# AdaptiveCity/deepdish

Hardware: AMD Instinct MI355X
Metric: end-to-end frames/sec (detect+encode+track) at 640x480 (higher is better)
Workload: dtype i8 (reference: uint8); encoder f16; 1 GPU; SSD-MobileNet-v1 uint8-quantised (300x300) + MARS-64x32x3 + deep_sort on synthetic 640x480 BGR frames, ~20 synthetic detections/frame (BASELINE.json configs[1]); streams_per_gpu=3072, worker_threads_per_gpu=2, parallelism=independent streams, 3072 per GPU in 2 worker groups, weights=seeded synthetic (seed 1234)

## Files before the change

deepdish_amd/csrc/mars_pair.hip:

```cpp
#include "mars_tail.h"

namespace {

typedef _Float16 h8 __attribute__((ext_vector_type(8)));
typedef float f4 __attribute__((ext_vector_type(4)));
typedef unsigned u4 __attribute__((ext_vector_type(4)));

__device__ __forceinline__ float elu(float v) {
    float e = __builtin_amdgcn_exp2f(v * 1.44269504088896340736f);
    e = __builtin_amdgcn_fmed3f(e, 0.f, 1.f);
    return __builtin_amdgcn_fmed3f(v, e - 1.f, 3.0e38f);
}

__device__ __forceinline__ void lds_fill16(const _Float16 *g, char *lds_wave_base) {
#if defined(__HIP_DEVICE_COMPILE__)
    __builtin_amdgcn_global_load_lds(g, lds_wave_base, 16, 0, 0);
#endif
}

__device__ __forceinline__ int frag_row(int a, int fr) { return (fr >> 2) * 8 + (a & 1) * 4 + (fr & 3); }

constexpr int PZ_B = 3072;
constexpr int PT64_B = 18 * 1024;
constexpr int PT32_B = 33 * 1024;
constexpr int PPLAIN_B = 16 * 1024;
constexpr int PRAW_B = 8 * 1024;
constexpr int pair_off_in(bool) { return PZ_B; }
constexpr int pair_off_h(bool first) { return PZ_B + 2 * (first ? PT32_B : PT64_B); }
constexpr int pair_off_res(bool first) { return pair_off_h(first) + 2 * PT64_B; }
constexpr int pair_off_raw(bool first) { return pair_off_res(first) + (first ? 2 : 3) * PPLAIN_B; }
constexpr int pair_off_const(bool first) { return pair_off_raw(first) + (first ? 2 * PRAW_B : 0); }
constexpr int pair_lds_bytes(bool first) { return pair_off_const(first) + 5 * 64 * 4; }

template <bool FIRST>
__global__ __launch_bounds__(512, 2) void mars_pair64_k(const MarsPairP P) {
    constexpr int OFF_IN = pair_off_in(FIRST), OFF_H = pair_off_h(FIRST), OFF_RES = pair_off_res(FIRST), OFF_RAW = pair_off_raw(FIRST),
                  OFF_C = pair_off_const(FIRST);
    constexpr int TIN_B = FIRST ? PT32_B : PT64_B, NRES = FIRST ? 2 : 3;
    extern __shared__ __attribute__((aligned(16))) char smem[];
    const int tid = threadIdx.x, lane = tid & 63;
    const int wave = __builtin_amdgcn_readfirstlane(tid >> 6);
    const int stage = wave >> 2, half = wave & 1, q = (wave >> 1) & 1;
    const int fr = lane & 15, fq = lane >> 4, j = fr >> 3, x = fr & 7;

    for (int i = tid * 16; i < OFF_C; i += 512 * 16) *reinterpret_cast<u4 *>(smem + i) = u4{0u, 0u, 0u, 0u};
    float *cst = reinterpret_cast<float *>(smem + OFF_C);
    if (tid < 64) {
        cst[tid] = P.bias_a[tid];
        cst[64 + tid] = P.bias_b[tid];
        cst[128 + tid] = P.aff2[tid];
        cst[192 + tid] = P.aff2[P.cout_pad + tid];
        cst[256 + tid] = (FIRST && P.bias_p) ? P.bias_p[tid] : 0.f;
    }
    __syncthreads();

    h8 wf[9][2][2];
    h8 wp[2];
    const bool a32 = FIRST && stage == 0;
    {
        const _Float16 *w = stage == 0 ? P.wa : P.wb;
        const int kpad = stage == 0 ? P.kpad_a : P.kpad_b;
#pragma unroll
        for (int t = 0; t < 9; ++t)
#pragma unroll
            for (int ks = 0; ks < 2; ++ks)
#pragma unroll
                for (int a = 0; a < 2; ++a) {
                    const size_t row = (size_t)(half * 32 + frag_row(a, fr)) * kpad;
                    wf[t][ks][a] = a32 ? *reinterpret_cast<const h8 *>(w + row + t * 32 + fq * 8)
                                       : *reinterpret_cast<const h8 *>(w + row + t * 64 + ks * 32 + fq * 8);
                }
#pragma unroll
        for (int a = 0; a < 2; ++a)
            wp[a] = FIRST ? *reinterpret_cast<const h8 *>(P.wp + (size_t)(half * 32 + frag_row(a, fr)) * P.kpad_p + fq * 8) : wf[0][0][a];
    }
#if defined(__HIP_DEVICE_COMPILE__)
#pragma unroll
    for (int t = 0; t < 9; ++t)
#pragma unroll
        for (int ks = 0; ks < 2; ++ks)
#pragma unroll
            for (int a = 0; a < 2; ++a) asm volatile("" ::"v"(wf[t][ks][a]));
    asm volatile("" ::"v"(wp[0]), "v"(wp[1]));
#endif

    const int n0 = blockIdx.x, nstep = gridDim.x;
    const int Kc = (P.n_img - n0 + nstep - 1) / nstep;

    const _Float16 *src[5];
    size_t stp[5];
    int n_dma;
    if constexpr (FIRST) {
        const int par = lane >> 5, pl = (lane >> 3) & 3, col = 2 * (lane & 7) + par;
#pragma unroll
        for (int h = 0; h < 4; ++h) {
            const int r = wave + 8 * h < 31 ? wave + 8 * h : 30;
            src[h] = col < 15 ? P.in + ((size_t)n0 * 31 + r) * 15 * P.cs_in + (size_t)col * P.cs_in + P.coff_in + pl * 8 : P.zero;
            stp[h] = col < 15 ? (size_t)nstep * 31 * 15 * P.cs_in : 0;
        }
        const int jr = lane >> 5, xx = lane & 7;
        src[4] = P.in2 + ((size_t)n0 * 31 + 2 * (2 * wave + jr)) * 15 * P.cs_in2 + (size_t)(2 * xx) * P.cs_in2 + P.coff_in2 + pl * 8;
        stp[4] = (size_t)nstep * 31 * 15 * P.cs_in2;
        n_dma = 5;
    } else {
        const int pl = lane >> 3, xx = lane & 7;
#pragma unroll
        for (int h = 0; h < 2; ++h) {
            src[h] = P.in + (((size_t)n0 * 16 + wave + 8 * h) * 8 + xx) * P.cs_in + P.coff_in + pl * 8;
            stp[h] = (size_t)nstep * 128 * P.cs_in;
            src[2 + h] = P.res + (((size_t)n0 * 16 + wave + 8 * h) * 8 + xx) * P.cs_res + P.coff_res + pl * 8;
            stp[2 + h] = (size_t)nstep * 128 * P.cs_res;
        }
        src[4] = P.zero; stp[4] = 0;
        n_dma = 4;
    }
    (void)n_dma;
    int dq = 0;
    auto issue = [&]() {
        char *T = smem + OFF_IN + (dq & 1) * TIN_B;
        if constexpr (FIRST) {
#pragma unroll
            for (int h = 0; h < 4; ++h) lds_fill16(src[h], T + ((wave + 8 * h < 31 ? wave + 8 * h : 30) + 1) * 1024);
            lds_fill16(src[4], smem + OFF_RAW + (dq & 1) * PRAW_B + wave * 1024);
        } else {
#pragma unroll
            for (int h = 0; h < 2; ++h) lds_fill16(src[h], T + (wave + 8 * h + 1) * 1024);
            const int rs = dq % 3;
#pragma unroll
            for (int h = 0; h < 2; ++h) lds_fill16(src[2 + h], smem + OFF_RES + rs * PPLAIN_B + (wave + 8 * h) * 1024);
        }
        ++dq;
        const bool more = dq < Kc;
#pragma unroll
        for (int h = 0; h < 5; ++h) src[h] += more ? stp[h] : 0;
    };

    const int co = half * 32 + fq * 8;
    const unsigned lo64 = (unsigned)((j * 64 + fq * 8 + x) * 16);
    const unsigned lo32 = (unsigned)((2 * j * 64 + fq * 8 + x) * 16);
    const f4 ba0 = *reinterpret_cast<const f4 *>(cst + (stage ? 64 : 0) + co), ba1 = *reinterpret_cast<const f4 *>(cst + (stage ? 64 : 0) + co + 4);

    issue();
    for (int c = 0; c <= Kc; ++c) {
#if defined(__HIP_DEVICE_COMPILE__)
        if (stage == 0 || c < 2) asm volatile("s_waitcnt vmcnt(0) lgkmcnt(0)" ::: "memory");
        else asm volatile("s_waitcnt vmcnt(8) lgkmcnt(0)" ::: "memory");
        __builtin_amdgcn_s_barrier();
        asm volatile("" ::: "memory");
#endif
        issue();
        const int cc = stage == 0 ? c : c - 1;
        if (cc < 0 || cc >= Kc) continue;
        const size_t n = (size_t)(n0 + cc * nstep);
#pragma unroll 1
        for (int f = 0; f < 4; ++f) {
            const int F = 4 * q + f;
            f4 acc[2] = {f4{0.f, 0.f, 0.f, 0.f}, f4{0.f, 0.f, 0.f, 0.f}};
            h8 X[4];
            if (a32) {
                const unsigned tb = (unsigned)(OFF_IN + (cc & 1) * PT32_B + 4 * F * 1024) + lo32;
                const unsigned bL = x == 0 ? ((tb + 512u - 16u) & 255u) : tb + 512u - 16u, bC = tb, bR = tb + 512u;
                const unsigned pb = (unsigned)(OFF_RAW + (cc & 1) * PRAW_B) + (unsigned)(((2 * F + j) * 32 + fq * 8 + x) * 16);
                f4 accp[2] = {f4{0.f, 0.f, 0.f, 0.f}, f4{0.f, 0.f, 0.f, 0.f}};
#if defined(__HIP_DEVICE_COMPILE__)
#define DD_RD(u_) do { if constexpr ((u_) < 9) { constexpr int dy_ = (u_) / 3, dx_ = (u_) - dy_ * 3;                                               \
                           asm volatile("ds_read_b128 %0, %1 offset:%2" : "=&v"(X[(u_) & 3]) : "v"(dx_ == 0 ? bL : dx_ == 1 ? bC : bR), "n"(dy_ * 1024) : "memory"); } \
                       else asm volatile("ds_read_b128 %0, %1" : "=&v"(X[(u_) & 3]) : "v"(pb) : "memory"); } while (0)
#define DD_UNIT(u_) do { if constexpr ((u_) + 3 < 10) DD_RD(((u_) + 3) % 10);                                                                      \
                         asm volatile("s_waitcnt lgkmcnt(%1)" : "+v"(X[(u_) & 3]) : "n"((u_) + 3 < 10 ? 3 : 9 - (u_)));                           \
                         if constexpr ((u_) < 9) { _Pragma("unroll") for (int a = 0; a < 2; ++a) acc[a] = __builtin_amdgcn_mfma_f32_16x16x32_f16(wf[(u_) % 9][0][a], X[(u_) & 3], acc[a], 0, 0, 0); } \
                         else { _Pragma("unroll") for (int a = 0; a < 2; ++a) accp[a] = __builtin_amdgcn_mfma_f32_16x16x32_f16(wp[a], X[(u_) & 3], accp[a], 0, 0, 0); } } while (0)
                DD_RD(0); DD_RD(1); DD_RD(2);
                DD_UNIT(0); DD_UNIT(1); DD_UNIT(2); DD_UNIT(3); DD_UNIT(4); DD_UNIT(5); DD_UNIT(6); DD_UNIT(7); DD_UNIT(8); DD_UNIT(9);
#undef DD_UNIT
#undef DD_RD
#endif
                const f4 c0 = *reinterpret_cast<const f4 *>(cst + 256 + co), c1 = *reinterpret_cast<const f4 *>(cst + 256 + co + 4);
                h8 sk;
#pragma unroll
                for (int i = 0; i < 4; ++i) { sk[i] = (_Float16)(accp[0][i] + c0[i]); sk[4 + i] = (_Float16)(accp[1][i] + c1[i]); }
                *reinterpret_cast<h8 *>(smem + OFF_RES + (cc & 1) * PPLAIN_B + ((2 * F + j) * 64 + (half * 4 + fq) * 8 + x) * 16) = sk;
            } else {
                const unsigned tb = (unsigned)((stage == 0 ? OFF_IN + (cc & 1) * PT64_B : OFF_H + (cc & 1) * PT64_B) + 2 * F * 1024) + lo64;
                const unsigned bL = x == 0 ? ((tb - 16u) & 255u) : tb - 16u, bC = tb, bR = x == 7 ? ((tb + 16u) & 255u) : tb + 16u;
#if defined(__HIP_DEVICE_COMPILE__)
#define DD_RD(u_) do { constexpr int t_ = (u_) >> 1, ks_ = (u_) & 1, dy_ = t_ / 3, dx_ = t_ - dy_ * 3;                                             \
                       asm volatile("ds_read_b128 %0, %1 offset:%2" : "=&v"(X[(u_) & 3]) : "v"(dx_ == 0 ? bL : dx_ == 1 ? bC : bR), "n"(dy_ * 1024 + ks_ * 512) : "memory"); } while (0)
#define DD_UNIT(u_) do { if constexpr ((u_) + 3 < 18) DD_RD(((u_) + 3) % 18);                                                                      \
                         asm volatile("s_waitcnt lgkmcnt(%1)" : "+v"(X[(u_) & 3]) : "n"((u_) + 3 < 18 ? 3 : 17 - (u_)));                          \
                         _Pragma("unroll") for (int a = 0; a < 2; ++a) acc[a] = __builtin_amdgcn_mfma_f32_16x16x32_f16(wf[(u_) >> 1][(u_) & 1][a], X[(u_) & 3], acc[a], 0, 0, 0); } while (0)
                DD_RD(0); DD_RD(1); DD_RD(2);
                DD_UNIT(0); DD_UNIT(1); DD_UNIT(2); DD_UNIT(3); DD_UNIT(4); DD_UNIT(5); DD_UNIT(6); DD_UNIT(7); DD_UNIT(8);
                DD_UNIT(9); DD_UNIT(10); DD_UNIT(11); DD_UNIT(12); DD_UNIT(13); DD_UNIT(14); DD_UNIT(15); DD_UNIT(16); DD_UNIT(17);
#undef DD_UNIT
#undef DD_RD
#endif
            }
            float v[8];
#pragma unroll
            for (int i = 0; i < 4; ++i) { v[i] = acc[0][i] + ba0[i]; v[4 + i] = acc[1][i] + ba1[i]; }
            if (stage == 0) {
                h8 o;
#pragma unroll
                for (int i = 0; i < 8; ++i) o[i] = (_Float16)elu(v[i]);
                *reinterpret_cast<h8 *>(smem + OFF_H + (cc & 1) * PT64_B + ((2 * F + j + 1) * 64 + (half * 4 + fq) * 8 + x) * 16) = o;
            } else {
                const int rs = FIRST ? (cc & 1) : cc % 3;
                const h8 rv = *reinterpret_cast<const h8 *>(smem + OFF_RES + rs * PPLAIN_B + ((2 * F + j) * 64 + (half * 4 + fq) * 8 + x) * 16);
#pragma unroll
                for (int i = 0; i < 8; ++i) v[i] += (float)rv[i];
                const size_t m = (n * 16 + 2 * F + j) * 8 + x;
                h8 o;
#pragma unroll
                for (int i = 0; i < 8; ++i) o[i] = (_Float16)v[i];
                *reinterpret_cast<h8 *>(P.out + m * P.cs_out + P.coff_out + co) = o;
                const f4 s0 = *reinterpret_cast<const f4 *>(cst + 128 + co), s1 = *reinterpret_cast<const f4 *>(cst + 128 + co + 4);
                const f4 t0 = *reinterpret_cast<const f4 *>(cst + 192 + co), t1 = *reinterpret_cast<const f4 *>(cst + 192 + co + 4);
                h8 o2;
#pragma unroll
                for (int i = 0; i < 4; ++i) { o2[i] = (_Float16)elu(s0[i] * v[i] + t0[i]); o2[4 + i] = (_Float16)elu(s1[i] * v[4 + i] + t1[i]); }
                *reinterpret_cast<h8 *>(P.out2 + m * P.cs_out2 + P.coff_out2 + co) = o2;
            }
        }
    }
#if defined(__HIP_DEVICE_COMPILE__)
    asm volatile("s_waitcnt vmcnt(0)" ::: "memory");
#endif
}

template <bool FIRST>
int launch_pair(hipStream_t s, int device, const MarsPairP &P) {
    constexpr int lds = pair_lds_bytes(FIRST);
    static_assert(lds <= 160 * 1024, "LDS budget");
    static DevOnce once;
    const int rc = once.run(device, [&]() -> int {
        DD_HIP(hipFuncSetAttribute(reinterpret_cast<const void *>(&mars_pair64_k<FIRST>), hipFuncAttributeMaxDynamicSharedMemorySize, lds));
        return DD_OK;
    });
    if (rc != DD_OK) return rc;
    const int n_cu = dd_cu_count(device);
    const int grid = P.n_img < n_cu ? P.n_img : n_cu;
    hipLaunchKernelGGL((mars_pair64_k<FIRST>), dim3(grid), dim3(512), lds, s, P);
    DD_LAUNCH_CHECK();
    return DD_OK;
}

}

int mars_pair64_launch(hipStream_t s, int device, const MarsPairP &P, bool first) {
    DD_REQUIRE(P.n_img > 0 && P.in && P.wa && P.wb && P.bias_a && P.bias_b && P.out && P.out2 && P.aff2 && P.zero && (first ? (P.in2 && P.wp) : P.res != nullptr), DD_E_ARG,
               "mars_pair64: bad argument");
    return first ? launch_pair<true>(s, device, P) : launch_pair<false>(s, device, P);
}
```

deepdish_amd/csrc/mars_tail.h:

```cpp
#pragma once
#include "common.h"

struct MarsWsP {
    const _Float16 *in;  int cs_in, coff_in;
    const _Float16 *in2; int cs_in2, coff_in2;
    const _Float16 *w;   int kpad;
    const _Float16 *w2;  int kpad2;
    const float *bias, *bias2;
    const _Float16 *res; int cs_res, coff_res;
    _Float16 *out;  int cs_out, coff_out;
    _Float16 *out2; int cs_out2, coff_out2;
    const float *aff2; int cout_pad;
    const _Float16 *zero;
    int n_img;
};

enum { MARS_WS_S1 = 0, MARS_WS_S1_RES = 1, MARS_WS_S2_PROJ = 2 };

int mars_ws128_launch(hipStream_t s, int device, const MarsWsP &P, int mode, int act, bool out2);

struct MarsPairP {
    const _Float16 *in;  int cs_in, coff_in;
    const _Float16 *in2; int cs_in2, coff_in2;
    const _Float16 *wa;  int kpad_a; const float *bias_a;
    const _Float16 *wp;  int kpad_p; const float *bias_p;
    const _Float16 *wb;  int kpad_b; const float *bias_b;
    const _Float16 *res; int cs_res, coff_res;
    _Float16 *out;  int cs_out, coff_out;
    _Float16 *out2; int cs_out2, coff_out2;
    const float *aff2; int cout_pad;
    const _Float16 *zero;
    int n_img;
};
int mars_pair64_launch(hipStream_t s, int device, const MarsPairP &P, bool first);
```

deepdish_amd/csrc/mars_tail.hip:

```cpp
#include "mars_tail.h"
#include <vector>

namespace {

typedef _Float16 h8 __attribute__((ext_vector_type(8)));
typedef float f4 __attribute__((ext_vector_type(4)));
typedef unsigned u4 __attribute__((ext_vector_type(4)));

enum { ACT_NONE = 0, ACT_ELU = 2 };

__device__ __forceinline__ float elu(float v) {
    float e = __builtin_amdgcn_exp2f(v * 1.44269504088896340736f);
    e = __builtin_amdgcn_fmed3f(e, 0.f, 1.f);
    return __builtin_amdgcn_fmed3f(v, e - 1.f, 3.0e38f);
}

__device__ __forceinline__ void lds_fill16(const _Float16 *g, char *lds_wave_base) {
#if defined(__HIP_DEVICE_COMPILE__)
    __builtin_amdgcn_global_load_lds(g, lds_wave_base, 16, 0, 0);
#endif
}

__device__ __forceinline__ int frag_row(int a, int fr) { return (fr >> 2) * 8 + (a & 1) * 4 + (fr & 3); }

#ifdef DD_MARS_STAMPS
__device__ unsigned long long dd_mars_stamps[256 * 8 * 8];
#define DD_STAMP(k) do { const unsigned long long t_ = __builtin_amdgcn_s_memtime(); st_acc[k] += t_ - st_last; st_last = t_; } while (0)
#else
#define DD_STAMP(k) do { } while (0)
#endif

constexpr int WS_LEAD = 2, WS_NB = WS_LEAD + 2, WS_NBR = WS_LEAD + 3;
constexpr int ws_tile_bytes(int mode) { return mode == MARS_WS_S2_PROJ ? 17 * 68 * 16 : 10 * 72 * 16; }
constexpr int ws_zero_bytes(int mode) { return mode == MARS_WS_S2_PROJ ? 0 : 7680; }
constexpr int WS_RES_BYTES = 8 * 72 * 16, WS_PRJ_BYTES = 4096;
constexpr int ws_xw_bytes(int mode) { return mode == MARS_WS_S2_PROJ ? 4096 : 2048; }
constexpr int ws_off_tiles(int mode) { return ws_zero_bytes(mode); }
constexpr int ws_off_aux(int mode) { return ws_off_tiles(mode) + WS_NB * ws_tile_bytes(mode); }
constexpr int ws_off_xchg(int mode) {
    return ws_off_aux(mode) + (mode == MARS_WS_S1_RES ? WS_NBR * WS_RES_BYTES : mode == MARS_WS_S2_PROJ ? WS_NB * WS_PRJ_BYTES : 0);
}
constexpr int ws_off_const(int mode) { return ws_off_xchg(mode) + 2 * 8 * ws_xw_bytes(mode); }
constexpr int ws_lds_bytes(int mode) { return ws_off_const(mode) + 3 * 128 * 4; }

template <int MODE, int ACT, bool OUT2>
__global__ __launch_bounds__(512, 2) void mars_ws128_k(const MarsWsP P) {
    constexpr bool S2 = MODE == MARS_WS_S2_PROJ, RES = MODE == MARS_WS_S1_RES;
    constexpr int LEAD = WS_LEAD, NB = WS_NB, NBR = WS_NBR;
    constexpr int TILE_B = ws_tile_bytes(MODE), XW_B = ws_xw_bytes(MODE);
    constexpr int OFF_T = ws_off_tiles(MODE), OFF_A = ws_off_aux(MODE), OFF_X = ws_off_xchg(MODE), OFF_C = ws_off_const(MODE);
    constexpr int KS = S2 ? 1 : 2, CIN = S2 ? 64 : 128;
    [[maybe_unused]] constexpr int N_DMA = S2 ? 3 : RES ? 2 : 1;
    [[maybe_unused]] constexpr int N_ST = S2 ? 2 : (RES && OUT2) ? 2 : 1;
    extern __shared__ __attribute__((aligned(16))) char smem[];
    const int tid = threadIdx.x, lane = tid & 63;
    const int wave = __builtin_amdgcn_readfirstlane(tid >> 6);
    const int cg = wave & 3, kh = wave >> 2;
    const int fr = lane & 15, fq = lane >> 4, yy = fr >> 2, x = fr & 3;

    for (int i = tid * 16; i < OFF_A; i += 512 * 16) *reinterpret_cast<u4 *>(smem + i) = u4{0u, 0u, 0u, 0u};
    float *cst = reinterpret_cast<float *>(smem + OFF_C);
    if (tid < 128) {
        cst[tid] = P.bias[tid];
        if constexpr (S2) cst[128 + tid] = P.bias2 ? P.bias2[tid] : 0.f;
        if constexpr (RES && OUT2) { cst[128 + tid] = P.aff2[tid]; cst[256 + tid] = P.aff2[P.cout_pad + tid]; }
    }
    __syncthreads();

    h8 wf[9][KS][2];
#pragma unroll
    for (int t = 0; t < 9; ++t)
#pragma unroll
        for (int ks = 0; ks < KS; ++ks)
#pragma unroll
            for (int a = 0; a < 2; ++a)
                wf[t][ks][a] = *reinterpret_cast<const h8 *>(P.w + (size_t)(cg * 32 + frag_row(a, fr)) * P.kpad + t * CIN + kh * (CIN / 2) + ks * 32 + fq * 8);
    h8 wp[2];
    if constexpr (S2) {
#pragma unroll
        for (int a = 0; a < 2; ++a) wp[a] = *reinterpret_cast<const h8 *>(P.w2 + (size_t)(cg * 32 + frag_row(a, fr)) * P.kpad2 + kh * 32 + fq * 8);
    }

#if defined(__HIP_DEVICE_COMPILE__)
#pragma unroll
    for (int t = 0; t < 9; ++t)
#pragma unroll
        for (int ks = 0; ks < KS; ++ks)
#pragma unroll
            for (int a = 0; a < 2; ++a) asm volatile("" ::"v"(wf[t][ks][a]));
    if constexpr (S2) asm volatile("" ::"v"(wp[0]), "v"(wp[1]));
#endif

    const int n0 = blockIdx.x, nstep = gridDim.x;
    const int Kc = (P.n_img - n0 + nstep - 1) / nstep;

    int dq = 0, dq_slot = 0, dq_rslot = 0;
    const _Float16 *src_a, *src_b, *src_c;
    size_t step_a, step_b, step_c;
    if constexpr (!S2) {
        src_a = P.in + (size_t)n0 * 32 * P.cs_in + ((wave * 4 + (lane & 3)) * P.cs_in + P.coff_in + (lane >> 2) * 8);
        src_b = RES ? P.res + (size_t)n0 * 32 * P.cs_res + ((wave * 4 + (lane & 3)) * P.cs_res + P.coff_res + (lane >> 2) * 8) : P.zero;
        src_c = P.zero;
        step_a = (size_t)nstep * 32 * P.cs_in; step_b = (size_t)nstep * 32 * P.cs_res; step_c = 0;
    } else {
        const int par = lane >> 5, pl = (lane >> 2) & 7, col = 2 * (lane & 3) + par;
        src_a = P.in + (size_t)n0 * 128 * P.cs_in + ((wave * 8 + col) * P.cs_in + P.coff_in + pl * 8);
        src_b = src_a + (size_t)64 * P.cs_in;
        const int ch = (wave & 3) * 64 + lane;
        src_c = P.in2 + (size_t)n0 * 128 * P.cs_in2 + ((2 * ((ch >> 2) & 7) * 8 + 2 * (ch & 3)) * P.cs_in2 + P.coff_in2 + (ch >> 5) * 8);
        step_a = step_b = (size_t)nstep * 128 * P.cs_in; step_c = (size_t)nstep * 128 * P.cs_in2;
    }
    auto issue = [&]() {
        char *T = smem + OFF_T + dq_slot * TILE_B;
        if constexpr (!S2) {
            lds_fill16(src_a, T + (wave + 1) * 72 * 16);
            if constexpr (RES) lds_fill16(src_b, smem + OFF_A + dq_rslot * WS_RES_BYTES + wave * 72 * 16);
        } else {
            lds_fill16(src_a, T + wave * 68 * 16);
            lds_fill16(src_b, T + (wave + 8) * 68 * 16);
            lds_fill16(src_c, smem + OFF_A + dq_slot * WS_PRJ_BYTES + (wave & 3) * 1024);
        }
        ++dq;
        const bool more = dq < Kc;
        src_a += more ? step_a : 0;
        if constexpr (RES || S2) src_b += more ? step_b : 0;
        if constexpr (S2) src_c += more ? step_c : 0;
        dq_slot = dq_slot + 1 == NB ? 0 : dq_slot + 1;
        dq_rslot = dq_rslot + 1 == NBR ? 0 : dq_rslot + 1;
    };

    const unsigned lo = S2 ? (unsigned)((2 * yy * 68 + (kh * 4 + fq) * 4 + x) * 16) : (unsigned)((yy * 72 + (kh * 8 + fq) * 4 + x) * 16);
    const unsigned lo_prj = (unsigned)(((kh * 4 + fq) * 32 + yy * 4 + x) * 16);
    const unsigned lo_res = (unsigned)(((4 * kh + yy) * 72 + (cg * 4 + fq) * 4 + x) * 16);
    const int co = cg * 32 + fq * 8;
    const f4 b0 = *reinterpret_cast<const f4 *>(cst + co), b1 = *reinterpret_cast<const f4 *>(cst + co + 4);

    f4 keep[S2 ? 4 : 2];
    int slot = 0, rslot_prev = 0, rslot = 0;

    auto epilogue = [&](int cprev) {
        const char *Xp = smem + OFF_X + ((cprev & 1) * 8 + (wave ^ 4)) * XW_B + lane * 16;
        const size_t n = (size_t)(n0 + cprev * nstep);
        const size_t m = (n * 8 + 4 * kh + yy) * 4 + x;
        float v[8];
        {
            const f4 o0 = *reinterpret_cast<const f4 *>(Xp), o1 = *reinterpret_cast<const f4 *>(Xp + 1024);
#pragma unroll
            for (int i = 0; i < 4; ++i) { v[i] = keep[0][i] + o0[i] + b0[i]; v[4 + i] = keep[1][i] + o1[i] + b1[i]; }
        }
        if constexpr (ACT == ACT_ELU) {
#pragma unroll
            for (int i = 0; i < 8; ++i) v[i] = elu(v[i]);
        }
        if constexpr (RES) {
            const h8 rv = *reinterpret_cast<const h8 *>(smem + OFF_A + rslot_prev * WS_RES_BYTES + lo_res);
#pragma unroll
            for (int i = 0; i < 8; ++i) v[i] += (float)rv[i];
        }
        h8 o;
#pragma unroll
        for (int i = 0; i < 8; ++i) o[i] = (_Float16)v[i];
        *reinterpret_cast<h8 *>(P.out + m * P.cs_out + P.coff_out + co) = o;
        if constexpr (RES && OUT2) {
            const f4 s0 = *reinterpret_cast<const f4 *>(cst + 128 + co), s1 = *reinterpret_cast<const f4 *>(cst + 128 + co + 4);
            const f4 t0 = *reinterpret_cast<const f4 *>(cst + 256 + co), t1 = *reinterpret_cast<const f4 *>(cst + 256 + co + 4);
            h8 o2;
#pragma unroll
            for (int i = 0; i < 4; ++i) { o2[i] = (_Float16)elu(s0[i] * v[i] + t0[i]); o2[4 + i] = (_Float16)elu(s1[i] * v[4 + i] + t1[i]); }
            *reinterpret_cast<h8 *>(P.out2 + m * P.cs_out2 + P.coff_out2 + co) = o2;
        }
        if constexpr (S2) {
            const f4 o0 = *reinterpret_cast<const f4 *>(Xp + 2048), o1 = *reinterpret_cast<const f4 *>(Xp + 3072);
            const f4 c0 = *reinterpret_cast<const f4 *>(cst + 128 + co), c1 = *reinterpret_cast<const f4 *>(cst + 128 + co + 4);
            h8 o2;
#pragma unroll
            for (int i = 0; i < 4; ++i) { o2[i] = (_Float16)(keep[2][i] + o0[i] + c0[i]); o2[4 + i] = (_Float16)(keep[3][i] + o1[i] + c1[i]); }
            *reinterpret_cast<h8 *>(P.out2 + m * P.cs_out2 + P.coff_out2 + co) = o2;
        }
    };

#ifdef DD_MARS_STAMPS
    unsigned long long st_acc[8] = {0, 0, 0, 0, 0, 0, 0, 0}, st_last = __builtin_amdgcn_s_memtime();
    const unsigned long long st_begin = st_last;
#endif
    static_assert(LEAD == 2, "the counted waits below are written for two crops of look-ahead");
    for (int ci = 0; ci < LEAD; ++ci) issue();
    DD_STAMP(0);
    for (int c = 0; c <= Kc; ++c) {
#if defined(__HIP_DEVICE_COMPILE__)
        if (kh == 0 || c == 0) {
            if (c <= 1) asm volatile("s_waitcnt vmcnt(%0) lgkmcnt(0)" ::"i"(N_DMA) : "memory");
            else if (c == 2) asm volatile("s_waitcnt vmcnt(%0) lgkmcnt(0)" ::"i"(N_DMA + N_ST) : "memory");
            else asm volatile("s_waitcnt vmcnt(%0) lgkmcnt(0)" ::"i"(N_DMA + 2 * N_ST) : "memory");
        } else asm volatile("s_waitcnt lgkmcnt(0)" ::: "memory");
        DD_STAMP(2);
        __builtin_amdgcn_s_barrier();
        asm volatile("" ::: "memory");
#endif
        DD_STAMP(3);
        auto compute = [&](f4 (&kp)[S2 ? 4 : 2]) {
            const unsigned tb = (unsigned)(OFF_T + slot * TILE_B) + lo;
            f4 acc[2][2] = {{f4{0.f, 0.f, 0.f, 0.f}, f4{0.f, 0.f, 0.f, 0.f}}, {f4{0.f, 0.f, 0.f, 0.f}, f4{0.f, 0.f, 0.f, 0.f}}};
            if constexpr (!S2) {
                const unsigned bs[3] = {x == 0 ? ((tb - 16u) & 255u) : tb - 16u, tb, x == 3 ? ((tb + 16u) & 255u) : tb + 16u};
                h8 X[4][2];
#if defined(__HIP_DEVICE_COMPILE__)
#define DD_RD(u_) do { constexpr int t_ = (u_) >> 1, p_ = (u_) & 1, dy_ = t_ / 3, dx_ = t_ - dy_ * 3;                                      \
                       asm volatile("ds_read_b128 %0, %2 offset:%3\n\tds_read_b128 %1, %2 offset:%4"                                       \
                                    : "=&v"(X[(u_) & 3][0]), "=&v"(X[(u_) & 3][1]) : "v"(bs[dx_]), "n"(((4 * p_ + dy_) * 72) * 16), "n"(((4 * p_ + dy_) * 72 + 16) * 16) : "memory"); } while (0)
#define DD_UNIT(u_) do { if constexpr ((u_) + 3 < 18) DD_RD(((u_) + 3) % 18);                                                            \
                         asm volatile("s_waitcnt lgkmcnt(%2)" : "+v"(X[(u_) & 3][0]), "+v"(X[(u_) & 3][1]) : "n"((u_) + 3 < 18 ? 6 : 2 * (17 - (u_))));          \
                         _Pragma("unroll") for (int ks = 0; ks < 2; ++ks) _Pragma("unroll") for (int a = 0; a < 2; ++a)                  \
                             acc[(u_) & 1][a] = __builtin_amdgcn_mfma_f32_16x16x32_f16(wf[(u_) >> 1][ks][a], X[(u_) & 3][ks], acc[(u_) & 1][a], 0, 0, 0); } while (0)
                DD_RD(0); DD_RD(1); DD_RD(2);
                DD_UNIT(0); DD_UNIT(1); DD_UNIT(2); DD_UNIT(3); DD_UNIT(4); DD_UNIT(5); DD_UNIT(6); DD_UNIT(7); DD_UNIT(8);
                DD_UNIT(9); DD_UNIT(10); DD_UNIT(11); DD_UNIT(12); DD_UNIT(13); DD_UNIT(14); DD_UNIT(15); DD_UNIT(16); DD_UNIT(17);
#undef DD_UNIT
#undef DD_RD
#endif
            } else {
                f4 accp[2][2] = {{f4{0.f, 0.f, 0.f, 0.f}, f4{0.f, 0.f, 0.f, 0.f}}, {f4{0.f, 0.f, 0.f, 0.f}, f4{0.f, 0.f, 0.f, 0.f}}};
                h8 X[4];
                const unsigned pb = (unsigned)(OFF_A + slot * WS_PRJ_BYTES) + lo_prj;
                const h8 hz = {(_Float16)0.f, (_Float16)0.f, (_Float16)0.f, (_Float16)0.f, (_Float16)0.f, (_Float16)0.f, (_Float16)0.f, (_Float16)0.f};
#if defined(__HIP_DEVICE_COMPILE__)
#define DD_RD(u_) do { if constexpr ((u_) < 18) { constexpr int t_ = (u_) >> 1, p_ = (u_) & 1, dy_ = t_ / 3, dx_ = t_ - dy_ * 3;                    \
                           asm volatile("ds_read_b128 %0, %1 offset:%2" : "=&v"(X[(u_) & 3]) : "v"(tb), "n"(((8 * p_ + dy_) * 68 + (dx_ == 1 ? 32 : 0) + (dx_ == 2 ? 1 : 0)) * 16) : "memory"); } \
                       else asm volatile("ds_read_b128 %0, %1 offset:%2" : "=&v"(X[(u_) & 3]) : "v"(pb), "n"(((u_) - 18) * 256) : "memory"); } while (0)
#define DD_UNIT(u_) do { if constexpr ((u_) + 3 < 20) DD_RD(((u_) + 3) % 20);                                                            \
                         asm volatile("s_waitcnt lgkmcnt(%1)" : "+v"(X[(u_) & 3]) : "n"((u_) + 3 < 20 ? 3 : 19 - (u_)));               \
                         if constexpr ((u_) < 18) { const h8 xv_ = (((u_) >> 1) % 3 == 2 && x == 3) ? hz : X[(u_) & 3];                    \
                             _Pragma("unroll") for (int a = 0; a < 2; ++a) acc[(u_) & 1][a] = __builtin_amdgcn_mfma_f32_16x16x32_f16(wf[(u_) >> 1][0][a], xv_, acc[(u_) & 1][a], 0, 0, 0); } \
                         else { _Pragma("unroll") for (int a = 0; a < 2; ++a) accp[(u_) - 18][a] = __builtin_amdgcn_mfma_f32_16x16x32_f16(wp[a], X[(u_) & 3], accp[(u_) - 18][a], 0, 0, 0); } } while (0)
                DD_RD(0); DD_RD(1); DD_RD(2);
                DD_UNIT(0); DD_UNIT(1); DD_UNIT(2); DD_UNIT(3); DD_UNIT(4); DD_UNIT(5); DD_UNIT(6); DD_UNIT(7); DD_UNIT(8); DD_UNIT(9);
                DD_UNIT(10); DD_UNIT(11); DD_UNIT(12); DD_UNIT(13); DD_UNIT(14); DD_UNIT(15); DD_UNIT(16); DD_UNIT(17); DD_UNIT(18); DD_UNIT(19);
#undef DD_UNIT
#undef DD_RD
#endif
                char *Xm = smem + OFF_X + ((c & 1) * 8 + wave) * XW_B + lane * 16;
                *reinterpret_cast<f4 *>(Xm + 2048) = kh ? accp[0][0] : accp[1][0];
                *reinterpret_cast<f4 *>(Xm + 3072) = kh ? accp[0][1] : accp[1][1];
                kp[2] = kh ? accp[1][0] : accp[0][0];
                kp[3] = kh ? accp[1][1] : accp[0][1];
            }
            char *Xm = smem + OFF_X + ((c & 1) * 8 + wave) * XW_B + lane * 16;
            *reinterpret_cast<f4 *>(Xm) = kh ? acc[0][0] : acc[1][0];
            *reinterpret_cast<f4 *>(Xm + 1024) = kh ? acc[0][1] : acc[1][1];
            kp[0] = kh ? acc[1][0] : acc[0][0];
            kp[1] = kh ? acc[1][1] : acc[0][1];
        };
        if (kh == 0) {
            f4 kn[S2 ? 4 : 2];
            if (c < Kc) compute(kn);
            DD_STAMP(5);
#if defined(__HIP_DEVICE_COMPILE__)
            asm volatile("s_waitcnt lgkmcnt(0)" ::: "memory");
            __builtin_amdgcn_s_barrier();
            asm volatile("" ::: "memory");
#endif
            DD_STAMP(3);
            issue();
            DD_STAMP(1);
            if (c > 0) epilogue(c - 1);
            DD_STAMP(4);
#pragma unroll
            for (int i = 0; i < (S2 ? 4 : 2); ++i) keep[i] = kn[i];
        } else {
            issue();
            DD_STAMP(1);
            if (c > 0) epilogue(c - 1);
            DD_STAMP(4);
#if defined(__HIP_DEVICE_COMPILE__)
            if (c == 0) asm volatile("s_waitcnt vmcnt(%0) lgkmcnt(0)" ::"i"(N_DMA) : "memory");
            else if (c == 1) asm volatile("s_waitcnt vmcnt(%0) lgkmcnt(0)" ::"i"(N_DMA + N_ST) : "memory");
            else asm volatile("s_waitcnt vmcnt(%0) lgkmcnt(0)" ::"i"(N_DMA + 2 * N_ST) : "memory");
            __builtin_amdgcn_s_barrier();
            asm volatile("" ::: "memory");
#endif
            DD_STAMP(3);
            if (c < Kc) compute(keep);
            DD_STAMP(5);
        }
        slot = slot + 1 == NB ? 0 : slot + 1;
        rslot_prev = rslot;
        rslot = rslot + 1 == NBR ? 0 : rslot + 1;
    }
#if defined(__HIP_DEVICE_COMPILE__)
    asm volatile("s_waitcnt vmcnt(0)" ::: "memory");
#endif
#ifdef DD_MARS_STAMPS
    if (lane == 0) {
        unsigned long long *d = dd_mars_stamps + ((size_t)blockIdx.x * 8 + wave) * 8;
        for (int k = 0; k < 6; ++k) d[k] = st_acc[k];
        d[6] = __builtin_amdgcn_s_memtime() - st_begin;
        d[7] = (unsigned long long)Kc;
    }
#endif
}

template <int MODE, int ACT, bool OUT2>
int launch_one(hipStream_t s, int device, const MarsWsP &P) {
    constexpr int lds = ws_lds_bytes(MODE);
    static_assert(lds <= 160 * 1024, "LDS budget");
    static DevOnce once;
    const int rc = once.run(device, [&]() -> int {
        DD_HIP(hipFuncSetAttribute(reinterpret_cast<const void *>(&mars_ws128_k<MODE, ACT, OUT2>), hipFuncAttributeMaxDynamicSharedMemorySize, lds));
        return DD_OK;
    });
    if (rc != DD_OK) return rc;
    const int n_cu = dd_cu_count(device);
    const int grid = P.n_img < n_cu ? P.n_img : n_cu;
    hipLaunchKernelGGL((mars_ws128_k<MODE, ACT, OUT2>), dim3(grid), dim3(512), lds, s, P);
    DD_LAUNCH_CHECK();
#ifdef DD_MARS_STAMPS
    {
        static std::vector<unsigned long long> h(256 * 8 * 8);
        DD_HIP(hipStreamSynchronize(s));
        DD_HIP(hipMemcpyFromSymbol(h.data(), HIP_SYMBOL(dd_mars_stamps), h.size() * 8));
        for (int half = 0; half < 2; ++half) {
            double a[7] = {0, 0, 0, 0, 0, 0, 0};
            int nw = 0;
            for (int b = 0; b < grid; ++b)
                for (int w = half * 4; w < half * 4 + 4; ++w, ++nw) {
                    const unsigned long long *d = h.data() + ((size_t)b * 8 + w) * 8;
                    for (int k = 0; k < 7; ++k) a[k] += (double)d[k] / (double)(k == 0 || k == 6 ? 1 : d[7] + 1);
                }
            fprintf(stderr, "mars_ws128_k<%d,%d,%d> K half %d: prologue DMAs %.0f | per step: issue %.0f, wait %.0f, barrier %.0f, epilogue %.0f, compute %.0f | loop total %.0f cycles, %d steps\n",
                    MODE, ACT, (int)OUT2, half, a[0] / nw, a[1] / nw, a[2] / nw, a[3] / nw, a[4] / nw, a[5] / nw, a[6] / nw, (int)h[7] + 1);
        }
    }
#endif
    return DD_OK;
}

}

int mars_ws128_launch(hipStream_t s, int device, const MarsWsP &P, int mode, int act, bool out2) {
    DD_REQUIRE(P.n_img > 0 && P.in && P.w && P.bias && P.out && P.zero, DD_E_ARG, "mars_ws128: bad argument");
    DD_REQUIRE((long long)P.n_img * 128 * (P.cs_in > P.cs_out ? P.cs_in : P.cs_out) < (1ll << 40), DD_E_CAPACITY, "mars_ws128: batch of %d", P.n_img);
    if (mode == MARS_WS_S2_PROJ) {
        DD_REQUIRE(P.in2 && P.w2 && P.out2 && act == ACT_ELU, DD_E_ARG, "mars_ws128: stride-2 form needs the projection operands and ELU");
        return launch_one<MARS_WS_S2_PROJ, ACT_ELU, false>(s, device, P);
    }
    if (mode == MARS_WS_S1) {
        DD_REQUIRE(!P.res && !P.out2, DD_E_ARG, "mars_ws128: plain form with a residual or a second output");
        return act == ACT_ELU ? launch_one<MARS_WS_S1, ACT_ELU, false>(s, device, P) : launch_one<MARS_WS_S1, ACT_NONE, false>(s, device, P);
    }
    DD_REQUIRE(mode == MARS_WS_S1_RES && P.res && act == ACT_NONE && (!out2 || (P.out2 && P.aff2)), DD_E_ARG, "mars_ws128: residual form");
    return out2 ? launch_one<MARS_WS_S1_RES, ACT_NONE, true>(s, device, P) : launch_one<MARS_WS_S1_RES, ACT_NONE, false>(s, device, P);
}
```

deepdish_amd/csrc/net_priv.h:

```cpp
#pragma once
#include <map>
#include <utility>
#include <vector>
#include "common.h"

struct TensorDesc { int buf, h, w, c, cs, coff, dtype, pad; };

struct dd_net {
    dd_ctx *ctx = nullptr;
    int max_batch = 0;
    std::vector<int32_t> prog;
    std::vector<TensorDesc> tensors;
    std::vector<int64_t> buf_elems;
    std::vector<void *> bufs;
    std::vector<int> buf_dtype;
    int n_ops = 0, ops_off = 0;
    void *arena = nullptr;
    int64_t arena_bytes = 0;
    char *d_weights = nullptr;
    int64_t weight_bytes = 0;
    int in_h = 0, in_w = 0, out_tensor = -1;
    bool profile = false;
    int last_batch = 0;
    DevBuf slab;
    bool ssd_dec = false, yolo_dec = false;
    int dec_anchors = 0; float dec_thr = 0.f;
    float *d_anchors = nullptr, *dec_boxes = nullptr, *dec_score = nullptr, *dec_keys = nullptr; int *dec_cls = nullptr;
    bool slab_moved = false;
    _Float16 *d_zero = nullptr;
    bool use_glds = true;
    bool use_rw = true;
    int tile_mode = 0;
    std::vector<hipEvent_t> events;
    std::vector<int32_t> op_launch;
    struct GraphEntry { int calls = 0; hipGraph_t graph = nullptr; hipGraphExec_t exec = nullptr; };
    bool use_graph = false;
    std::map<std::pair<const void *, int>, GraphEntry> graphs;
};

int netq_run_op(dd_net *net, int op_index, const int32_t *o, const uint8_t *input, int nimg, hipStream_t s, int *handled);
int netq_run_front(dd_net *net, const int32_t *o0, const int32_t *o1, const int32_t *o2, const uint8_t *input, int nimg, hipStream_t s, int *ran);
int netq_run_mid(dd_net *net, const int32_t *o3, const int32_t *o4, int nimg, hipStream_t s, int *ran);
int netq_prepare(dd_net *net);
```

deepdish_amd/csrc/nets.hip:

```cpp
#include <algorithm>
#include <cmath>
#include <cstdlib>
#include <map>
#include <string>
#include "common.h"
#include "ssd_dev.h"
#include "net_priv.h"
#include "mars_tail.h"

namespace {

typedef _Float16 h8 __attribute__((ext_vector_type(8)));
typedef _Float16 h4 __attribute__((ext_vector_type(4)));
typedef float f4 __attribute__((ext_vector_type(4)));

enum { OP_INPUT = 1, OP_CONV = 2, OP_DWCONV = 3, OP_MAXPOOL = 4, OP_UPSAMPLE = 5, OP_FC = 6, OP_L2NORM = 7, OP_STEM = 8, OP_DWPW = 9 };
enum { ACT_NONE = 0, ACT_RELU6 = 1, ACT_ELU = 2, ACT_SILU = 3, ACT_RELU = 4, ACT_SIGMOID = 5 };
enum { EPI_F16 = 0, EPI_F32 = 1, EPI_SSD_HEAD = 2, EPI_YOLO = 3 };
enum { OPK_DEFAULT = 0, OPK_FOLDED = 1, OPK_POOL_ROWS = 2, OPK_POOL_ROWS_STEM = 3, OPK_RES_UNIT = 4, OPK_SSD_FRONT = 5, OPK_C64_ROWS = 6, OPK_S2_ROWS = 7, OPK_CONV_WS = 8, OPK_WS_DW = 9, OPK_DWPW_ROWS = 10, OPK_SSD_HEAD_DEC = 11, OPK_RES_PAIR = 12, OPK_YOLO_HEAD_DEC = 13, OPK_MARS_WS = 14, OPK_FOLDED_PREV = 15, OPK_MARS_PAIR = 16, OPK_C64_STRIPS = 18, OPK_Q_FRONT = 19, OPK_Q_MID = 20, OPK_STEM_WIDE = 23 };
enum { DT_F16 = 0, DT_F32 = 1, DT_U8 = 2 };

constexpr int OP_WORDS = 48;
constexpr int TENSOR_WORDS = 8;

// ... 40 lines not shown
    const _Float16 *in; int H, W, cs_in, coff_in, cin;
    const _Float16 *w; const float *bias; int kpad;
    int kh, kw, stride, pad_t, pad_l;
    int ho, wo, cout, m;
    int act;
    void *out; int cs_out, coff_out, epi;
    const _Float16 *res; int cs_res, coff_res;
    _Float16 *out2; int cs_out2, coff_out2; const float *aff2; int cout_pad;
    int post_aff;
    int splitk; float *slab;
    const _Float16 *zero;
    int p[6]; float f[8];
    int th, tw, tiles_x, tiles_y;
    const uint8_t *src8; float in_mean, in_scale;
    const _Float16 *dw_w; const float *dw_bias; int dw_act; int total_quads;
    const float *anchors; float *dec_boxes, *dec_score, *dec_keys; int *dec_cls; float dec_thr;
};


__device__ __forceinline__ void conv_epilogue(const ConvP &P, int m, int co, float v[4], int hw) {
    const f4 bv = *reinterpret_cast<const f4 *>(P.bias + co);
#pragma unroll
    for (int r = 0; r < 4; ++r) v[r] += bv[r];
    if (P.epi == EPI_YOLO) {
        const int n = m / hw, p = m - n * hw;
        const int py = p / P.wo, px = p - py * P.wo;
#pragma unroll
        for (int r = 0; r < 4; ++r) {
            const int ch = co + r;
            if (ch >= P.cout) continue;
            const int no = P.p[0];
            const int an = ch / no, o = ch - an * no;
            const float s = fast_sigmoid(v[r]);
            float val = s;
            if (o < 4) val = yolo_box_col(o, s, (float)px, (float)py, P.f[6], P.f[2 * an], P.f[2 * an + 1], P.f[7], (float)P.p[4]);
            const size_t row = (size_t)n * P.p[1] + P.p[2] + (size_t)an * hw + p;
            static_cast<float *>(P.out)[row * no + o] = val;
        }
        return;
    }
#pragma unroll
    for (int r = 0; r < 4; ++r) v[r] = apply_act(v[r], P.act);
    if (P.epi == EPI_SSD_HEAD) {
        const int n = m / hw, p = m - n * hw;
        const int A = P.p[5];
        float *dst = static_cast<float *>(P.out) + ((size_t)n * P.p[1] + P.p[2] + (size_t)p * A) * P.p[3];
#pragma unroll
        for (int r = 0; r < 4; ++r)
            if (co + r < P.cout) dst[co + r] = v[r];
        return;
    }
    if (P.res) {
        const h4 rv = *reinterpret_cast<const h4 *>(P.res + (size_t)m * P.cs_res + P.coff_res + co);
#pragma unroll
        for (int r = 0; r < 4; ++r) v[r] += (float)rv[r];
    }
    if (P.epi == EPI_F32) {
        if (P.post_aff) {
            const f4 sc = *reinterpret_cast<const f4 *>(P.aff2 + co);
            const f4 sh = *reinterpret_cast<const f4 *>(P.aff2 + P.cout_pad + co);
#pragma unroll
            for (int r = 0; r < 4; ++r) v[r] = sc[r] * v[r] + sh[r];
        }
#pragma unroll
        for (int r = 0; r < 4; ++r)
            if (co + r >= P.cout) v[r] = 0.f;
        *reinterpret_cast<f4 *>(static_cast<float *>(P.out) + (size_t)m * P.cs_out + P.coff_out + co) = f4{v[0], v[1], v[2], v[3]};
        return;
    }
#pragma unroll
    for (int r = 0; r < 4; ++r)
        if (co + r >= P.cout) v[r] = 0.f;
    {
        h4 o;
#pragma unroll
        for (int r = 0; r < 4; ++r) o[r] = (_Float16)v[r];
        *reinterpret_cast<h4 *>(static_cast<_Float16 *>(P.out) + (size_t)m * P.cs_out + P.coff_out + co) = o;
    }
    if (P.out2) {
        const f4 sc = *reinterpret_cast<const f4 *>(P.aff2 + co);
        const f4 sh = *reinterpret_cast<const f4 *>(P.aff2 + P.cout_pad + co);
        h4 o;
#pragma unroll
        for (int r = 0; r < 4; ++r) {
            const float t = co + r < P.cout ? apply_act(sc[r] * v[r] + sh[r], ACT_ELU) : 0.f;
            o[r] = (_Float16)t;
        }
        *reinterpret_cast<h4 *>(P.out2 + (size_t)m * P.cs_out2 + P.coff_out2 + co) = o;
    }
}

typedef unsigned u4v_t __attribute__((ext_vector_type(4)));
template <int HI>
__device__ __forceinline__ float fma_mix_f16(unsigned x, unsigned w, float acc) {
#if defined(__HIP_DEVICE_COMPILE__)
    if (HI) asm("v_fma_mix_f32 %0, %1, %2, %0 op_sel:[1,1,0] op_sel_hi:[1,1,0]" : "+v"(acc) : "v"(x), "v"(w));
    else asm("v_fma_mix_f32 %0, %1, %2, %0 op_sel:[0,0,0] op_sel_hi:[1,1,0]" : "+v"(acc) : "v"(x), "v"(w));
#endif
    return acc;
}
__device__ __forceinline__ void dw_tap(float (&acc)[8], const h8 &x, const h8 &w) {
    const u4v_t xv = __builtin_bit_cast(u4v_t, x), wv = __builtin_bit_cast(u4v_t, w);
#pragma unroll
    for (int i = 0; i < 8; ++i)
        acc[i] = (i & 1) ? fma_mix_f16<1>(xv[i >> 1], wv[i >> 1], acc[i]) : fma_mix_f16<0>(xv[i >> 1], wv[i >> 1], acc[i]);
}

struct Epi8 { f4 b0, b1, s0, s1, t0, t1; };

__device__ __forceinline__ Epi8 epi8_load(const ConvP &P, int co) {
    Epi8 E;
    E.b0 = *reinterpret_cast<const f4 *>(P.bias + co);
    E.b1 = *reinterpret_cast<const f4 *>(P.bias + co + 4);
    E.s0 = E.s1 = E.t0 = E.t1 = f4{0.f, 0.f, 0.f, 0.f};
    if (P.out2) {
        E.s0 = *reinterpret_cast<const f4 *>(P.aff2 + co);
        E.s1 = *reinterpret_cast<const f4 *>(P.aff2 + co + 4);
        E.t0 = *reinterpret_cast<const f4 *>(P.aff2 + P.cout_pad + co);
        E.t1 = *reinterpret_cast<const f4 *>(P.aff2 + P.cout_pad + co + 4);
    }
    return E;
}

#ifndef DD_EPI_NT
#define DD_EPI_NT true
#endif
template <int ACT = -1, bool BIAS = true, int EF = -1, bool NT = DD_EPI_NT, bool TAIL = true>
__device__ __forceinline__ void conv_epilogue_f16x8(const ConvP &P, const Epi8 &E, int m, int co, float v[8], const h8 *res_pre = nullptr) {
    const int act = ACT < 0 ? P.act : ACT;
    const bool has_res = EF < 0 ? P.res != nullptr : EF >= 1, has_out2 = EF < 0 ? P.out2 != nullptr : EF == 1;
#pragma unroll
    for (int r = 0; r < 4; ++r) {
        v[r] = apply_act(BIAS ? v[r] + E.b0[r] : v[r], act);
        v[4 + r] = apply_act(BIAS ? v[4 + r] + E.b1[r] : v[4 + r], act);
    }
    if (has_res) {
        const h8 rv = res_pre ? *res_pre : *reinterpret_cast<const h8 *>(P.res + (size_t)m * P.cs_res + P.coff_res + co);
#pragma unroll
        for (int r = 0; r < 8; ++r) v[r] += (float)rv[r];
    }
    const bool tail = TAIL && co + 8 > P.cout;
    h8 o;
#pragma unroll
    for (int r = 0; r < 8; ++r) o[r] = (_Float16)v[r];
    if (tail) {
#pragma unroll
        for (int r = 0; r < 8; ++r)
            if (co + r >= P.cout) o[r] = (_Float16)0.f;
    }
    h8 *dst = reinterpret_cast<h8 *>(static_cast<_Float16 *>(P.out) + (size_t)m * P.cs_out + P.coff_out + co);
    if constexpr (NT) __builtin_nontemporal_store(o, dst);
    else *dst = o;
    if (has_out2) {
        h8 o2;
#pragma unroll
        for (int r = 0; r < 8; ++r) {
            const float sc = r < 4 ? E.s0[r] : E.s1[r - 4], sh = r < 4 ? E.t0[r] : E.t1[r - 4];
            o2[r] = (_Float16)apply_act(sc * v[r] + sh, ACT_ELU);
        }
        if (tail) {
#pragma unroll
            for (int r = 0; r < 8; ++r)
                if (co + r >= P.cout) o2[r] = (_Float16)0.f;
        }
        *reinterpret_cast<h8 *>(P.out2 + (size_t)m * P.cs_out2 + P.coff_out2 + co) = o2;
    }
}

template <int ACT = -1>
__device__ __forceinline__ void conv_epilogue_f16x8(const ConvP &P, int m, int co, float v[8]) {
    const Epi8 E = epi8_load(P, co);
    conv_epilogue_f16x8<ACT>(P, E, m, co, v);
}

template <int ACT, int BM, int BN, int T>
__device__ __forceinline__ void conv_finish_rows(const ConvP &P, const float *ot, int m0, int n0) {
    constexpr int OROW = BN + 4, G = BN / 8;
    static_assert(T % G == 0, "a thread keeps its channel group over the row loop");
    const int g = threadIdx.x % G, co = n0 + g * 8;
    if (co >= P.cout_pad) return;
    const Epi8 E = epi8_load(P, co);
    for (int pl = threadIdx.x / G; pl < BM; pl += T / G) {
        const int m = m0 + pl;
        if (m >= P.m) break;
        const f4 lo = *reinterpret_cast<const f4 *>(ot + pl * OROW + g * 8);
        const f4 hi = *reinterpret_cast<const f4 *>(ot + pl * OROW + g * 8 + 4);
        float v[8] = {lo[0], lo[1], lo[2], lo[3], hi[0], hi[1], hi[2], hi[3]};
        conv_epilogue_f16x8<ACT>(P, E, m, co, v);
    }
}

template <int WM, int WN, int MI, int NI>
__device__ __forceinline__ void conv_finish(const ConvP &P, f4 (&acc)[NI][MI], _Float16 *lds, int m0, int n0, int hw) {
    constexpr int T = WM * WN * 64;
    constexpr int BM = WM * MI * 16, BN = WN * NI * 16;
    const int tid = threadIdx.x, lane = tid & 63, wave = tid >> 6;
    const int wm = wave / WN, wn = wave % WN;
    const int fr = lane & 15, fq = lane >> 4;
    if (P.epi == EPI_F16 && P.splitk == 1) {
        constexpr int OROW = BN + 4;
        float *ot = reinterpret_cast<float *>(lds);
#pragma unroll
        for (int b = 0; b < MI; ++b)
#pragma unroll
            for (int a = 0; a < NI; ++a)
                *reinterpret_cast<f4 *>(ot + ((wm * MI + b) * 16 + fr) * OROW + (wn * NI + a) * 16 + fq * 4) = acc[a][b];
        __syncthreads();
        switch (P.act) {
            case ACT_NONE: conv_finish_rows<ACT_NONE, BM, BN, T>(P, ot, m0, n0); break;
            case ACT_RELU6: conv_finish_rows<ACT_RELU6, BM, BN, T>(P, ot, m0, n0); break;
            case ACT_ELU: conv_finish_rows<ACT_ELU, BM, BN, T>(P, ot, m0, n0); break;
            case ACT_SILU: conv_finish_rows<ACT_SILU, BM, BN, T>(P, ot, m0, n0); break;
            default: conv_finish_rows<-1, BM, BN, T>(P, ot, m0, n0);
        }
        return;
    }
    if (P.epi == EPI_SSD_HEAD && P.splitk == 1) {
        constexpr int OROW = BN + 4;
        float *ot = reinterpret_cast<float *>(lds);
#pragma unroll
        for (int b = 0; b < MI; ++b)
#pragma unroll
            for (int a = 0; a < NI; ++a)
                *reinterpret_cast<f4 *>(ot + ((wm * MI + b) * 16 + fr) * OROW + (wn * NI + a) * 16 + fq * 4) = acc[a][b];
        __syncthreads();
        const int A = P.p[5];
        typedef float f4u __attribute__((ext_vector_type(4), aligned(4)));
        constexpr int LPP = BN / 4, PPW = 64 / LPP;
        const int lc = (lane % LPP) * 4, lp = lane / LPP;
        const int ch = n0 + lc;
        const int nlive = min(4, max(0, P.cout - ch));
        f4 bias = f4{0.f, 0.f, 0.f, 0.f};
        for (int q = 0; q < nlive; ++q) bias[q] = P.bias[ch + q];
        for (int pl = wave * PPW + lp; pl < BM; pl += WM * WN * PPW) {
            const int m = m0 + pl;
            if (m >= P.m || nlive == 0) continue;
            const int n = m / hw, p = m - n * hw;
            float *__restrict__ dst = static_cast<float *>(P.out) + ((size_t)n * P.p[1] + P.p[2] + (size_t)p * A) * P.p[3] + ch;
            const f4 v = *reinterpret_cast<const f4 *>(ot + pl * OROW + lc) + bias;
            if (nlive == 4) *reinterpret_cast<f4u *>(dst) = v;
            else for (int q = 0; q < nlive; ++q) dst[q] = v[q];
// ... 1176 lines not shown
        for (int r = 0; r <= H / 2; ++r) {
            fill_pre(2 * r + 3); fill_pre(2 * r + 4);
            if constexpr (RAW_SEP) { fill_raw(2 * r + 1); fill_raw(2 * r + 2); }
            auto conv2 = [&](const _Float16 *ringp, int slot0, int mask, const h8 (&w)[9][2], f4 (&acc)[2][2]) {
                h8 X[2][3];
                auto rd = [&](int i, h8 (&x)[3]) {
                    const _Float16 *rs = ringp + ((slot0 + i) & mask) * RU_SLOT + offC;
                    x[0] = *reinterpret_cast<const h8 *>(rs - 8);
                    x[1] = *reinterpret_cast<const h8 *>(rs);
                    x[2] = *reinterpret_cast<const h8 *>(rs + 8);
                };
                rd(0, X[0]);
#pragma unroll
                for (int i = 0; i < 4; ++i) {
                    h8 (&x)[3] = X[i & 1];
#if defined(__HIP_DEVICE_COMPILE__)
                    asm volatile("" : "+v"(x[0]), "+v"(x[1]), "+v"(x[2]));
                    __builtin_amdgcn_sched_barrier(0);
#endif
                    if (i + 1 < 4) rd(i + 1, X[(i + 1) & 1]);
#if defined(__HIP_DEVICE_COMPILE__)
                    __builtin_amdgcn_sched_barrier(0);
#endif
#pragma unroll
                    for (int dx = 0; dx < 3; ++dx)
#pragma unroll
                        for (int cr = 0; cr < 2; ++cr) {
                            const int dy = i - cr;
                            if (dy < 0 || dy > 2) continue;
#pragma unroll
                            for (int a = 0; a < 2; ++a)
                                acc[cr][a] = __builtin_amdgcn_mfma_f32_16x16x32_f16(w[dy * 3 + dx][a], x[dx], acc[cr][a], 0, 0, 0);
                        }
#if defined(__HIP_DEVICE_COMPILE__)
                    __builtin_amdgcn_sched_barrier(0);
#endif
                }
            };
            {
                f4 acc[2][2] = {{bA0, bA1}, {bA0, bA1}};
                conv2(pre, 2 * r, RU_PRE_SLOTS - 1, wA, acc);
#pragma unroll
                for (int cr = 0; cr < 2; ++cr) {
                    const int y = 2 * r + cr;
                    const bool live = y < H && fr < W;
                    h8 o;
#pragma unroll
                    for (int q = 0; q < 4; ++q) {
                        o[q] = (_Float16)apply_act(acc[cr][0][q], actA);
                        o[4 + q] = (_Float16)apply_act(acc[cr][1][q], actA);
                    }
                    u4v_t ou = __builtin_bit_cast(u4v_t, o);
                    ou &= live ? 0xFFFFFFFFu : 0u;
                    *reinterpret_cast<u4v_t *>(h1 + (y & (RU_H1_SLOTS - 1)) * RU_SLOT + offC) = ou;
                }
            }
            {
                f4 acc[2][2] = {{EB.b0, EB.b1}, {EB.b0, EB.b1}};
                conv2(h1, 2 * r - 2, RU_H1_SLOTS - 1, wB, acc);
                h8 rv0 = RAW_SEP ? *reinterpret_cast<const h8 *>(rawr + ((2 * r - 1) & (RU_RAW_SLOTS - 1)) * RU_SLOT + offC)
                                 : *reinterpret_cast<const h8 *>(pre + ((2 * r) & (RU_PRE_SLOTS - 1)) * RU_SLOT + offC);
#if defined(__HIP_DEVICE_COMPILE__)
                asm volatile("s_waitcnt vmcnt(0)" ::: "memory");
#endif
#pragma unroll
                for (int cr = 0; cr < 2; ++cr) {
                    const int y = 2 * r - 1 + cr;
                    if (cr == 1) rv0 = RAW_SEP ? *reinterpret_cast<const h8 *>(rawr + (y & (RU_RAW_SLOTS - 1)) * RU_SLOT + offC)
                                               : *reinterpret_cast<const h8 *>(pre + ((y + 1) & (RU_PRE_SLOTS - 1)) * RU_SLOT + offC);
                    if ((unsigned)y >= (unsigned)H || fr >= W) continue;
                    float o[8];
#pragma unroll
                    for (int q = 0; q < 4; ++q) { o[q] = acc[cr][0][q]; o[4 + q] = acc[cr][1][q]; }
                    conv_epilogue_f16x8<ACT_NONE, false, 1, true, false>(PB, EB, (n * H + y) * W + fr, fq * 8, o, &rv0);
                }
            }
        }
    }
}

constexpr int RP_X_SLOTS = 8;
constexpr int rp_pair_halves() { return 6 * 8 + (RU_PRE_SLOTS + 2 * RU_H1_SLOTS + 2 * RP_X_SLOTS) * RU_SLOT; }

template <int ACT_A>
__global__ __launch_bounds__(512, 2) void res_pair_rows_k(const ConvP P1A, const ConvP P1B, const ConvP P2A, const ConvP P2B, const int n_img) {
    extern __shared__ __attribute__((aligned(16))) _Float16 lds[];
    const int tid = threadIdx.x, lane = tid & 63;
    const int wave = __builtin_amdgcn_readfirstlane(tid >> 6);
    const int pair = wave & 3, role = wave >> 2;
    const int fr = lane & 15, fq = lane >> 4;
    _Float16 *pbase = lds + (size_t)pair * rp_pair_halves();
    _Float16 *pre = pbase + 8;
    _Float16 *h1a = pre + RU_PRE_SLOTS * RU_SLOT + 8;
    _Float16 *xo = h1a + RU_H1_SLOTS * RU_SLOT + 8;
    _Float16 *xo2 = xo + RP_X_SLOTS * RU_SLOT + 8;
    _Float16 *h1b = xo2 + RP_X_SLOTS * RU_SLOT + 8;
    const h8 zero8 = {(_Float16)0.f, (_Float16)0.f, (_Float16)0.f, (_Float16)0.f, (_Float16)0.f, (_Float16)0.f, (_Float16)0.f, (_Float16)0.f};
    for (int i = (role * 64 + lane) * 8; i < rp_pair_halves(); i += 128 * 8) *reinterpret_cast<h8 *>(pbase + i) = zero8;

    const _Float16 *wa_p = role ? P2A.w : P1A.w, *wb_p = role ? P2B.w : P1B.w;
    const int kpa = role ? P2A.kpad : P1A.kpad, kpb = role ? P2B.kpad : P1B.kpad;
    h8 wA[9][2], wB[9][2];
#pragma unroll
    for (int t = 0; t < 9; ++t)
#pragma unroll
        for (int a = 0; a < 2; ++a) {
            wA[t][a] = *reinterpret_cast<const h8 *>(wa_p + (size_t)rw_weight_row(a, fr) * kpa + t * 32 + fq * 8);
            wB[t][a] = *reinterpret_cast<const h8 *>(wb_p + (size_t)rw_weight_row(a, fr) * kpb + t * 32 + fq * 8);
        }
    const float *ba_p = role ? P2A.bias : P1A.bias, *bb_p = role ? P2B.bias : P1B.bias, *af_p = role ? P2B.aff2 : P1B.aff2;
    const int cpad = role ? P2B.cout_pad : P1B.cout_pad;
    const f4 bA0 = *reinterpret_cast<const f4 *>(ba_p + fq * 8), bA1 = *reinterpret_cast<const f4 *>(ba_p + fq * 8 + 4);
    Epi8 EB;
    EB.b0 = *reinterpret_cast<const f4 *>(bb_p + fq * 8); EB.b1 = *reinterpret_cast<const f4 *>(bb_p + fq * 8 + 4);
    EB.s0 = *reinterpret_cast<const f4 *>(af_p + fq * 8); EB.s1 = *reinterpret_cast<const f4 *>(af_p + fq * 8 + 4);
    EB.t0 = *reinterpret_cast<const f4 *>(af_p + cpad + fq * 8); EB.t1 = *reinterpret_cast<const f4 *>(af_p + cpad + fq * 8 + 4);
    const int H = P1A.H, W = P1A.W;
    const int offC = (fq * 16 + fr) * 8;
    const int actA = ACT_A < 0 ? P1A.act : ACT_A;
    _Float16 *inr = role ? xo2 : pre, *h1r = role ? h1b : h1a, *resr = role ? xo : pre;

    const int n0 = blockIdx.x * 4 + pair, nstep = gridDim.x * 4;
    const int K = n0 < n_img ? (n_img - n0 + nstep - 1) / nstep : 0;
    const int base4 = blockIdx.x * 4;
    const int Kmax = base4 < n_img ? (n_img - base4 + nstep - 1) / nstep : 0;
    const int GA = 16 * K, Gall = 16 * Kmax + 2;
    auto fill_pre = [&](int s) {
        const int kk = (s + 1) >> 5, y = ((s + 1) & 31) - 1;
        const bool ok = kk < K && y >= 0 && fr < W;
        const _Float16 *src = P1A.in + ((size_t)(n0 + (ok ? kk : 0) * nstep) * H * W + (size_t)(ok ? y : 0) * W + fr) * P1A.cs_in + P1A.coff_in + fq * 8;
        lds_fill16(ok ? src : P1A.zero, pre + ((s + 1) & (RU_PRE_SLOTS - 1)) * RU_SLOT);
    };
#if defined(__HIP_DEVICE_COMPILE__)
    asm volatile("s_waitcnt lgkmcnt(0)" ::: "memory");
    __builtin_amdgcn_s_barrier();
    asm volatile("" ::: "memory");
#endif
    if (role == 0 && K > 0) { fill_pre(-1); fill_pre(0); fill_pre(1); fill_pre(2); fill_pre(3); fill_pre(4); }
#if defined(__HIP_DEVICE_COMPILE__)
    asm volatile("s_waitcnt vmcnt(0)" ::: "memory");
#endif
    auto conv2 = [&](const _Float16 *ringp, int slot0, int mask, const h8 (&w)[9][2], f4 (&acc)[2][2]) {
        h8 X[2][3];
        auto rd = [&](int i, h8 (&x)[3]) {
            const _Float16 *rs = ringp + ((slot0 + i) & mask) * RU_SLOT + offC;
            x[0] = *reinterpret_cast<const h8 *>(rs - 8);
            x[1] = *reinterpret_cast<const h8 *>(rs);
            x[2] = *reinterpret_cast<const h8 *>(rs + 8);
        };
        rd(0, X[0]);
#pragma unroll
        for (int i = 0; i < 4; ++i) {
            h8 (&x)[3] = X[i & 1];
#if defined(__HIP_DEVICE_COMPILE__)
            asm volatile("" : "+v"(x[0]), "+v"(x[1]), "+v"(x[2]));
            __builtin_amdgcn_sched_barrier(0);
#endif
            if (i + 1 < 4) rd(i + 1, X[(i + 1) & 1]);
#if defined(__HIP_DEVICE_COMPILE__)
            __builtin_amdgcn_sched_barrier(0);
#endif
#pragma unroll
            for (int dx = 0; dx < 3; ++dx)
#pragma unroll
                for (int cr = 0; cr < 2; ++cr) {
                    const int dy = i - cr;
                    if (dy < 0 || dy > 2) continue;
#pragma unroll
                    for (int a = 0; a < 2; ++a)
                        acc[cr][a] = __builtin_amdgcn_mfma_f32_16x16x32_f16(w[dy * 3 + dx][a], x[dx], acc[cr][a], 0, 0, 0);
                }
#if defined(__HIP_DEVICE_COMPILE__)
            __builtin_amdgcn_sched_barrier(0);
#endif
        }
    };
    f4 accC[2][2];
    int grC = -1;
    auto b_store = [&]() {
#pragma unroll
        for (int cr = 0; cr < 2; ++cr) {
            const int s = 2 * grC - 1 + cr;
            const int kk = (s + 1) >> 5, y = ((s + 1) & 31) - 1;
            if (y < 0 || fr >= W) continue;
            float o[8];
#pragma unroll
            for (int q = 0; q < 4; ++q) { o[q] = accC[cr][0][q]; o[4 + q] = accC[cr][1][q]; }
            const h8 rv = *reinterpret_cast<const h8 *>(resr + ((s + 1) & (RU_PRE_SLOTS - 1)) * RU_SLOT + offC);
            conv_epilogue_f16x8<ACT_NONE, false, 1, true, false>(P2B, EB, ((n0 + kk * nstep) * H + y) * W + fr, fq * 8, o, &rv);
        }
    };
    for (int g = 0; g < Gall; ++g) {
        const int gr = role ? g - 2 : g;
        const bool active = role ? (gr >= 0 && gr < GA) : (K > 0 && gr <= GA);
        if (grC >= 0) { b_store(); grC = -1; }
        if (active) {
            if (role == 0) { fill_pre(2 * gr + 5); fill_pre(2 * gr + 6); }
            {
                f4 acc[2][2] = {{bA0, bA1}, {bA0, bA1}};
                conv2(inr, 2 * gr, RU_PRE_SLOTS - 1, wA, acc);
#pragma unroll
                for (int cr = 0; cr < 2; ++cr) {
                    const int s = 2 * gr + cr;
                    const bool live = ((s + 1) & 31) != 0 && fr < W;
                    h8 o;
#pragma unroll
                    for (int q = 0; q < 4; ++q) {
                        o[q] = (_Float16)apply_act(acc[cr][0][q], actA);
                        o[4 + q] = (_Float16)apply_act(acc[cr][1][q], actA);
                    }
                    u4v_t ou = __builtin_bit_cast(u4v_t, o);
                    ou &= live ? 0xFFFFFFFFu : 0u;
                    *reinterpret_cast<u4v_t *>(h1r + (s & (RU_H1_SLOTS - 1)) * RU_SLOT + offC) = ou;
                }
            }
            {
                f4 acc[2][2] = {{EB.b0, EB.b1}, {EB.b0, EB.b1}};
                conv2(h1r, 2 * gr - 2, RU_H1_SLOTS - 1, wB, acc);
                h8 rv[2];
#pragma unroll
                for (int cr = 0; cr < 2; ++cr) rv[cr] = *reinterpret_cast<const h8 *>(resr + ((2 * gr + cr) & (RU_PRE_SLOTS - 1)) * RU_SLOT + offC);
                if (role == 0) {
#pragma unroll
                    for (int cr = 0; cr < 2; ++cr) {
                        const int s = 2 * gr - 1 + cr;
                        const bool live = ((s + 1) & 31) != 0 && fr < W;
                        float v[8];
#pragma unroll
                        for (int q = 0; q < 4; ++q) { v[q] = acc[cr][0][q]; v[4 + q] = acc[cr][1][q]; }
#pragma unroll
                        for (int q = 0; q < 8; ++q) v[q] += (float)rv[cr][q];
                        h8 o, o2;
#pragma unroll
                        for (int q = 0; q < 8; ++q) o[q] = (_Float16)v[q];
#pragma unroll
                        for (int q = 0; q < 8; ++q) {
                            const float sc = q < 4 ? EB.s0[q] : EB.s1[q - 4], sh = q < 4 ? EB.t0[q] : EB.t1[q - 4];
                            o2[q] = (_Float16)apply_act(sc * v[q] + sh, ACT_ELU);
                        }
                        u4v_t ou = __builtin_bit_cast(u4v_t, o), ou2 = __builtin_bit_cast(u4v_t, o2);
                        ou &= live ? 0xFFFFFFFFu : 0u;
                        ou2 &= live ? 0xFFFFFFFFu : 0u;
                        *reinterpret_cast<u4v_t *>(xo + ((s + 1) & (RP_X_SLOTS - 1)) * RU_SLOT + offC) = ou;
                        *reinterpret_cast<u4v_t *>(xo2 + ((s + 1) & (RP_X_SLOTS - 1)) * RU_SLOT + offC) = ou2;
                    }
#if defined(__HIP_DEVICE_COMPILE__)
                    asm volatile("s_waitcnt vmcnt(2)" ::: "memory");
#endif
                } else {
#pragma unroll
                    for (int cr = 0; cr < 2; ++cr) { accC[cr][0] = acc[cr][0]; accC[cr][1] = acc[cr][1]; }
                    grC = gr;
                }
            }
        }
#if defined(__HIP_DEVICE_COMPILE__)
        asm volatile("s_waitcnt lgkmcnt(0)" ::: "memory");
        __builtin_amdgcn_s_barrier();
        asm volatile("" ::: "memory");
#endif
    }
    if (grC >= 0) b_store();
#if defined(__HIP_DEVICE_COMPILE__)
    asm volatile("s_waitcnt vmcnt(0)" ::: "memory");
#endif
}

constexpr int C64_PITCH = 704, C64_SLOTS = 11, C64_RES_SLOTS = 4, C64_LEAD = 3;
constexpr int c64_wave_halves() { return C64_SLOTS * C64_PITCH + C64_RES_SLOTS * 512; }

template <int ACT, int EF, bool STRIP = false>
__global__ __launch_bounds__(256, 2) void conv3x3_c64_rows_k(const ConvP P, const int n_img) {
    extern __shared__ __attribute__((aligned(16))) _Float16 lds[];
    const int tid = threadIdx.x, lane = tid & 63;
    const int wave = __builtin_amdgcn_readfirstlane(tid >> 6);
    const int fr = lane & 15, fq = lane >> 4;
    const int j = fr >> 3, x = fr & 7;
    _Float16 *ring = lds + (size_t)wave * c64_wave_halves(), *resr = ring + C64_SLOTS * C64_PITCH;
    const int H = P.H, S = H + 1, RPI = H / 2;
    constexpr int NRES = EF ? 1 : 0;
    (void)NRES;
    const int NSX = STRIP ? P.W >> 3 : 1;

    const int half = wave & 1;
    h8 wf[9][2][2];
#pragma unroll
    for (int t = 0; t < 9; ++t)
#pragma unroll
        for (int ks = 0; ks < 2; ++ks)
#pragma unroll
            for (int a = 0; a < 2; ++a)
                wf[t][ks][a] = *reinterpret_cast<const h8 *>(P.w + (size_t)(half * 32 + rw_weight_row(a, fr)) * P.kpad + t * 64 + ks * 32 + fq * 8);
    const Epi8 E = epi8_load(P, half * 32 + fq * 8);
    const int lane_off = (fq * 10 + x) * 8;
    const int n0 = blockIdx.x * 2 + (wave >> 1), nstep = gridDim.x * 2;
    const int K = n0 < n_img ? (n_img - n0 + nstep - 1) / nstep : 0;
    const int T = K * S + 1, Q = K * RPI;

    int dma_off[2];
    bool dma_px[2], dma_l[2], dma_r[2];
#pragma unroll
    for (int c2 = 0; c2 < 2; ++c2) {
        const int c = 16 * c2 + lane, pl = c / 10, sl = c - pl * 10;
        dma_px[c2] = sl >= 1 && sl <= 8;
        dma_l[c2] = sl == 0; dma_r[c2] = sl == 9;
        dma_off[c2] = (sl - 1) * P.cs_in + pl * 8;
    }
    int dq = 0, dq_slot = 0, dq_k = 0, dq_y = -1;
    int dq_f = n0 / NSX, dq_sx = n0 - dq_f * NSX;
    auto issue_row = [&]() {
        const bool rok = dq < T && dq_y >= 0;
        const _Float16 *row = STRIP ? P.in + (((size_t)dq_f * H + (rok ? dq_y : 0)) * P.W + dq_sx * 8) * P.cs_in + P.coff_in
                                    : P.in + ((size_t)(n0 + dq_k * nstep) * H + (rok ? dq_y : 0)) * 8 * P.cs_in + P.coff_in;
        _Float16 *dst = ring + dq_slot * C64_PITCH;
#pragma unroll
        for (int c2 = 0; c2 < 2; ++c2) {
            const bool ok = rok && (dma_px[c2] || (STRIP && ((dma_l[c2] && dq_sx > 0) || (dma_r[c2] && dq_sx + 1 < NSX))));
            lds_fill16(ok ? row + dma_off[c2] : P.zero, dst + 128 * c2);
        }
        ++dq;
        dq_slot = dq_slot + 1 == C64_SLOTS ? 0 : dq_slot + 1;
// ... 1676 lines not shown
            const int split = force_split > 0 ? force_split : nimg >= 1536 ? 1 : nimg >= 768 ? 2 : 4;
            const int n_units = nimg * split;
            const int grid = std::min(dd_ceil_div(n_units, 4), 2 * 256);
            if (stem) hipLaunchKernelGGL((conv3x3_pool_rows_k<ACT_ELU, true>), dim3((unsigned)grid), dim3(256), ring_bytes, s, P, n_units, split | (dbg << 8));
            else hipLaunchKernelGGL((conv3x3_pool_rows_k<ACT_ELU, false>), dim3((unsigned)grid), dim3(256), ring_bytes, s, P, n_units, split | (dbg << 8));
            DD_LAUNCH_CHECK();
            return DD_OK;
        }
    } else {
        spatial_tile(P.ho, P.wo, 1, RW_MAX_PATCH, P);
    }
    const int npix = (P.th + 2) * (P.tw + 2);
    DD_REQUIRE(npix <= RW_MAX_PATCH, DD_E_ARG, "conv3x3_rw: patch of %d pixels", npix);
    DD_REQUIRE(pool || !P.src8 || (P.tw == 32 && P.act == ACT_SILU && !P.res && !P.out2), DD_E_ARG, "conv3x3_rw: an input op was folded into a launch that cannot take it");
    const size_t lds_bytes = (size_t)4 * ((npix * 16 + 255) & ~255) + (pool ? (size_t)P.th * P.tw * 32 * sizeof(_Float16) : 0);
    const int total = nimg * P.tiles_x * P.tiles_y;
    const int grid = std::min(total, 2 * 256);
    if (pool) {
        static DevOnce once;
        const int rc = once.run(device, [&]() -> int {
            DD_HIP(hipFuncSetAttribute(reinterpret_cast<const void *>(&conv3x3_rw_k<2, 32, ACT_ELU, true>),
                                       hipFuncAttributeMaxDynamicSharedMemorySize, (int)lds_bytes));
            return DD_OK;
        });
        if (rc != DD_OK) return rc;
    }
    if (pool) {
        hipLaunchKernelGGL((conv3x3_rw_k<2, 32, ACT_ELU, true>), dim3((unsigned)grid), dim3(256), lds_bytes, s, P, total);
        DD_LAUNCH_CHECK();
        return DD_OK;
    }
#define DD_RW(TW_, ACT_, EF_) hipLaunchKernelGGL((conv3x3_rw_k<2, TW_, ACT_, false, EF_>), dim3((unsigned)grid), dim3(256), lds_bytes, s, P, total)
    const int ef = (!P.res && !P.out2) ? 0 : (P.res && P.out2) ? 1 : -1;
    if (P.tw == 32 && P.act == ACT_ELU && ef == 0) DD_RW(32, ACT_ELU, 0);
    else if (P.tw == 32 && P.act == ACT_SILU && P.src8 && ef == 0)
        hipLaunchKernelGGL((conv3x3_rw_k<2, 32, ACT_SILU, false, 0, true>), dim3((unsigned)grid), dim3(256), lds_bytes, s, P, total);
    else if (P.tw == 32 && P.act == ACT_SILU) DD_RW(32, ACT_SILU, -1);
    else if (P.tw == 15 && P.act == ACT_ELU && ef == 0) DD_RW(15, ACT_ELU, 0);
    else if (P.tw == 15 && P.act == ACT_NONE && ef == 1) DD_RW(15, ACT_NONE, 1);
    else DD_RW(0, -1, -1);
#undef DD_RW
    DD_LAUNCH_CHECK();
    return DD_OK;
}

bool res_unit_fusable(const ConvP &A, const ConvP &B, int nimg) {
    static const bool off = getenv("DD_RES_UNIT_UNFUSED") && atoi(getenv("DD_RES_UNIT_UNFUSED")) != 0;
    static const int min_img = getenv("DD_RES_UNIT_MIN") ? atoi(getenv("DD_RES_UNIT_MIN")) : 512;
    auto plain = [](const ConvP &P) {
        return P.kh == 3 && P.kw == 3 && P.stride == 1 && P.pad_t == 1 && P.pad_l == 1 && P.cin == 32 && P.cout == 32 && P.cout_pad == 32 &&
               P.epi == EPI_F16 && P.W == 15 && P.wo == 15 && P.H == P.ho && P.splitk <= 1;
    };
    return !off && nimg >= min_img && plain(A) && plain(B) && A.act == ACT_ELU && !A.res && !A.out2 && !A.coff_out &&
           B.act == ACT_NONE && B.res && B.out2 && B.in == static_cast<const _Float16 *>(A.out) && !B.coff_in && B.cs_in == A.cs_out && B.H == A.H;
}

int launch_res_unit(hipStream_t s, const ConvP &A, const ConvP &B, int nimg, int device) {
    const bool raw_sep = !(B.res == A.in && B.cs_res == A.cs_in && B.coff_res == A.coff_in);
    const size_t lds_bytes = (size_t)4 * ru_wave_halves(raw_sep) * sizeof(_Float16);
    static DevOnce once;
    const int rc = once.run(device, [&]() -> int {
        DD_HIP(hipFuncSetAttribute(reinterpret_cast<const void *>(&res_unit_rows_k<ACT_ELU, true>),
                                   hipFuncAttributeMaxDynamicSharedMemorySize, (int)(4 * ru_wave_halves(true) * sizeof(_Float16))));
        return DD_OK;
    });
    if (rc != DD_OK) return rc;
    const int grid = std::min(dd_ceil_div(nimg, 4), 2 * 256);
    if (raw_sep) hipLaunchKernelGGL((res_unit_rows_k<ACT_ELU, true>), dim3((unsigned)grid), dim3(256), lds_bytes, s, A, B, nimg);
    else hipLaunchKernelGGL((res_unit_rows_k<ACT_ELU, false>), dim3((unsigned)grid), dim3(256), lds_bytes, s, A, B, nimg);
    DD_LAUNCH_CHECK();
    return DD_OK;
}

bool res_pair_fusable(const ConvP &A1, const ConvP &B1, const ConvP &A2, const ConvP &B2, int nimg) {
    static const bool off = getenv("DD_RES_PAIR_OFF") && atoi(getenv("DD_RES_PAIR_OFF")) != 0;
    static const int min_img = getenv("DD_RES_PAIR_MIN") ? atoi(getenv("DD_RES_PAIR_MIN")) : 1024;
    return !off && nimg >= min_img && A1.H == 31 && A1.W == 15 &&
           B1.res == A1.in && B1.cs_res == A1.cs_in && B1.coff_res == A1.coff_in &&
           A2.in == static_cast<const _Float16 *>(B1.out2) && A2.cs_in == B1.cs_out2 && !A2.coff_in && !B1.coff_out2 &&
           B2.res == static_cast<const _Float16 *>(B1.out) && B2.cs_res == B1.cs_out && B2.coff_res == B1.coff_out &&
           A2.H == A1.H && A2.W == A1.W && A1.act == ACT_ELU && A2.act == ACT_ELU;
}

int launch_res_pair(hipStream_t s, const ConvP &A1, const ConvP &B1, const ConvP &A2, const ConvP &B2, int nimg, int device) {
    constexpr size_t lds_bytes = (size_t)4 * rp_pair_halves() * sizeof(_Float16);
    static DevOnce once;
    const int rc = once.run(device, [&]() -> int {
        DD_HIP(hipFuncSetAttribute(reinterpret_cast<const void *>(&res_pair_rows_k<ACT_ELU>), hipFuncAttributeMaxDynamicSharedMemorySize, (int)lds_bytes));
        return DD_OK;
    });
    if (rc != DD_OK) return rc;
    const int grid = std::min(dd_ceil_div(nimg, 4), 256);
    hipLaunchKernelGGL((res_pair_rows_k<ACT_ELU>), dim3((unsigned)grid), dim3(512), lds_bytes, s, A1, B1, A2, B2, nimg);
    DD_LAUNCH_CHECK();
    return DD_OK;
}

bool s2_rows_eligible(const ConvP &P, int nimg, int max_batch) {
    static const bool off = getenv("DD_S2_ROWS_OFF") && atoi(getenv("DD_S2_ROWS_OFF")) != 0;
    static const int min_img = getenv("DD_S2_ROWS_MIN") ? atoi(getenv("DD_S2_ROWS_MIN")) : 512;
    return !off && nimg >= min_img && P.kh == 3 && P.kw == 3 && P.stride == 2 && P.pad_t == 1 && P.pad_l == 1 && P.cin == 32 && P.cout == 64 &&
           P.cout_pad == 64 && P.kpad >= 288 && P.epi == EPI_F16 && P.W == 15 && P.H == 31 && P.ho == 16 && P.wo == 8 && P.splitk <= 1 &&
           P.act == ACT_ELU && !P.res && !P.out2 && (long long)dd_ceil_div(max_batch * P.ho * P.wo, 64) >= 256;
}

int launch_conv3x3_s2_rows(hipStream_t s, const ConvP &P, int nimg, int device) {
    constexpr size_t lds_bytes = (size_t)4 * S2_SLOTS * S2_PITCH * sizeof(_Float16);
    static DevOnce once;
    const int rc = once.run(device, [&]() -> int {
        DD_HIP(hipFuncSetAttribute(reinterpret_cast<const void *>(&conv3x3_s2_rows_k<ACT_ELU>), hipFuncAttributeMaxDynamicSharedMemorySize, (int)lds_bytes));
        return DD_OK;
    });
    if (rc != DD_OK) return rc;
    const int grid = std::min(dd_ceil_div(nimg, 4), 2 * 256);
    hipLaunchKernelGGL((conv3x3_s2_rows_k<ACT_ELU>), dim3((unsigned)grid), dim3(256), lds_bytes, s, P, nimg);
    DD_LAUNCH_CHECK();
    return DD_OK;
}

bool c64_strips_eligible(const ConvP &P, int nimg, int max_batch) {
    static const bool off = getenv("DD_C64_STRIPS_OFF") && atoi(getenv("DD_C64_STRIPS_OFF")) != 0;
    static const int min_items = getenv("DD_C64_STRIPS_MIN") ? atoi(getenv("DD_C64_STRIPS_MIN")) : 1024;
    return !off && P.kh == 3 && P.kw == 3 && P.stride == 1 && P.pad_t == 1 && P.pad_l == 1 && P.cin == 64 && P.cout == 64 &&
           P.cout_pad == 64 && P.kpad == 576 && P.epi == EPI_F16 && P.W > 8 && P.W % 8 == 0 && P.wo == P.W && P.H == P.ho && P.H % 2 == 0 &&
           P.splitk <= 1 && P.act == ACT_SILU && !P.out2 && (!P.res || (P.cs_res % 8 == 0 && P.coff_res % 8 == 0)) &&
           P.cs_in % 8 == 0 && P.coff_in % 8 == 0 && (long long)nimg * (P.W >> 3) >= min_items &&
           (long long)dd_ceil_div(max_batch * P.ho * P.wo, 64) >= 256;
}

int launch_conv3x3_c64_strips(hipStream_t s, const ConvP &P, int nimg, int device) {
    constexpr size_t lds_bytes = (size_t)4 * c64_wave_halves() * sizeof(_Float16);
    static DevOnce once;
    const int rc = once.run(device, [&]() -> int {
        DD_HIP(hipFuncSetAttribute(reinterpret_cast<const void *>(&conv3x3_c64_rows_k<ACT_SILU, 0, true>), hipFuncAttributeMaxDynamicSharedMemorySize, (int)lds_bytes));
        DD_HIP(hipFuncSetAttribute(reinterpret_cast<const void *>(&conv3x3_c64_rows_k<ACT_SILU, 2, true>), hipFuncAttributeMaxDynamicSharedMemorySize, (int)lds_bytes));
        return DD_OK;
    });
    if (rc != DD_OK) return rc;
    const long long items = (long long)nimg * (P.W >> 3);
    DD_REQUIRE(items * P.H * 8 < (1LL << 31), DD_E_CAPACITY, "conv3x3_c64 strips: %lld items exceed 32-bit pixel indexing", items);
    const int grid = (int)std::min<long long>((items + 1) / 2, 2 * 256);
    if (P.res) hipLaunchKernelGGL((conv3x3_c64_rows_k<ACT_SILU, 2, true>), dim3((unsigned)grid), dim3(256), lds_bytes, s, P, (int)items);
    else hipLaunchKernelGGL((conv3x3_c64_rows_k<ACT_SILU, 0, true>), dim3((unsigned)grid), dim3(256), lds_bytes, s, P, (int)items);
    DD_LAUNCH_CHECK();
    return DD_OK;
}

bool c64_rows_eligible(const ConvP &P, int nimg, int max_batch) {
    static const bool off = getenv("DD_C64_ROWS_OFF") && atoi(getenv("DD_C64_ROWS_OFF")) != 0;
    static const int min_img = getenv("DD_C64_ROWS_MIN") ? atoi(getenv("DD_C64_ROWS_MIN")) : 512;
    return !off && nimg >= min_img && P.kh == 3 && P.kw == 3 && P.stride == 1 && P.pad_t == 1 && P.pad_l == 1 && P.cin == 64 && P.cout == 64 &&
           P.cout_pad == 64 && P.kpad == 576 && P.epi == EPI_F16 && P.W == 8 && P.wo == 8 && P.H == P.ho && P.H % 2 == 0 && P.splitk <= 1 &&
           ((P.act == ACT_ELU && !P.res && !P.out2) || (P.act == ACT_NONE && P.res && P.out2 && P.cs_res % 8 == 0 && P.coff_res % 8 == 0)) &&
           (long long)dd_ceil_div(max_batch * P.ho * P.wo, 64) >= 256;
}

int launch_conv3x3_c64_rows(hipStream_t s, const ConvP &P, int nimg, int device) {
    constexpr size_t lds_bytes = (size_t)4 * c64_wave_halves() * sizeof(_Float16);
    static DevOnce once;
    const int rc = once.run(device, [&]() -> int {
        DD_HIP(hipFuncSetAttribute(reinterpret_cast<const void *>(&conv3x3_c64_rows_k<ACT_ELU, 0>), hipFuncAttributeMaxDynamicSharedMemorySize, (int)lds_bytes));
        DD_HIP(hipFuncSetAttribute(reinterpret_cast<const void *>(&conv3x3_c64_rows_k<ACT_NONE, 1>), hipFuncAttributeMaxDynamicSharedMemorySize, (int)lds_bytes));
        return DD_OK;
    });
    if (rc != DD_OK) return rc;
    const int grid = std::min(dd_ceil_div(nimg, 2), 2 * 256);
    if (P.res) hipLaunchKernelGGL((conv3x3_c64_rows_k<ACT_NONE, 1>), dim3((unsigned)grid), dim3(256), lds_bytes, s, P, nimg);
    else hipLaunchKernelGGL((conv3x3_c64_rows_k<ACT_ELU, 0>), dim3((unsigned)grid), dim3(256), lds_bytes, s, P, nimg);
    DD_LAUNCH_CHECK();
    return DD_OK;
}

bool ssd_front_fusable(const ConvP &S, const ConvP &P, int nimg) {
    static const bool off = getenv("DD_SSD_FRONT_UNFUSED") && atoi(getenv("DD_SSD_FRONT_UNFUSED")) != 0;
    static const int min_img = getenv("DD_SSD_FRONT_MIN") ? atoi(getenv("DD_SSD_FRONT_MIN")) : 16;
    return !off && nimg >= min_img && S.stride == 2 && S.cout == 32 && S.cout_pad == 32 && S.act == ACT_RELU6 && (S.W * 3) % 4 == 0 &&
// ... 173 lines not shown
    DD_LAUNCH_CHECK();
    return DD_OK;
}

bool ws_dw_fusable(const ConvP &P, const DwP &Q, int nimg) {
    static const bool off = getenv("DD_WS_DW_OFF") && atoi(getenv("DD_WS_DW_OFF")) != 0;
    if (off || !ws_eligible(P) || P.act != ACT_RELU6 || Q.act != ACT_RELU6 || Q.stride != 1 || Q.pad_t != 1 || Q.pad_l != 1) return false;
    if (Q.in != static_cast<const _Float16 *>(P.out) || Q.coff_in || Q.cs_in != P.cs_out || P.coff_out || Q.H != P.ho || Q.W != P.wo ||
        Q.ho != Q.H || Q.wo != Q.W || Q.c != P.cout || P.cout != P.cout_pad || (Q.W != 19 && Q.W != 10) || (long long)nimg * Q.H * Q.W >= (1 << 23))
        return false;
    const int n_slices = P.cout_pad / 128, n_workers = (512 / 8 / n_slices) * 8;
    if (n_slices < 1 || (512 / 8) % n_slices) return false;
    const int per = dd_ceil_div(nimg, n_workers);
    return (double)nimg / ((double)per * n_workers) >= 0.85;
}

template <int KS, int WMAP>
int launch_conv_ws_dw(hipStream_t s, ConvP &P, const DwP &Q, int nimg, int device) {
    constexpr int NW = 4, D = 4;
    const int n_slices = P.cout_pad / (32 * NW);
    P.splitk = 1;
    constexpr size_t lds_bytes = ((size_t)D * WS_BM * 64 + NW * 4 * WSD_SLOTS * 8 + 8 + 9 * 128) * sizeof(_Float16);
    static DevOnce once;
    const int rc = once.run(device, [&]() -> int {
        DD_HIP(hipFuncSetAttribute(reinterpret_cast<const void *>(&conv_ws_dw_k<KS, WMAP, ACT_RELU6, ACT_RELU6>), hipFuncAttributeMaxDynamicSharedMemorySize, (int)lds_bytes));
        return DD_OK;
    });
    if (rc != DD_OK) return rc;
    static const int dbg_mode = getenv("DD_WS_MODE") ? atoi(getenv("DD_WS_MODE")) : 0;
    P.p[5] = dbg_mode;
    hipLaunchKernelGGL((conv_ws_dw_k<KS, WMAP, ACT_RELU6, ACT_RELU6>), dim3(512), dim3(NW * 64), lds_bytes, s, P, Q, n_slices, nimg);
    DD_LAUNCH_CHECK();
    return DD_OK;
}


template <int STRIDE>
int launch_dwpw_big(hipStream_t s, ConvP &P, int device, int nimg) {
    const size_t in_bytes = (size_t)nimg * P.H * P.W * P.cs_in * sizeof(_Float16);
    DD_REQUIRE(in_bytes < (1ull << 31), DD_E_CAPACITY, "dwpw_big: input of %zu bytes exceeds the 2 GiB buffer-resource window", in_bytes);
    P.p[0] = (int)in_bytes;
    P.total_quads = nimg * P.ho * ((P.wo + 1) / 2);
    const size_t lds_bytes = (size_t)(2 * DWB_BM + 2 * DWB_BN) * 64 * sizeof(_Float16) + (size_t)P.cin * (18 + 4) + DWB_BM * sizeof(int);
    const bool relu6 = P.act == ACT_RELU6 && P.dw_act == ACT_RELU6;
    static DevOnce once;
    const int rc = once.run(device, [&]() -> int {
        DD_HIP(hipFuncSetAttribute(reinterpret_cast<const void *>(&dwpw_big_k<STRIDE, ACT_RELU6, ACT_RELU6>),
                                   hipFuncAttributeMaxDynamicSharedMemorySize, 160 * 1024));
        DD_HIP(hipFuncSetAttribute(reinterpret_cast<const void *>(&dwpw_big_k<STRIDE, -1, -1>),
                                   hipFuncAttributeMaxDynamicSharedMemorySize, 160 * 1024));
        return DD_OK;
    });
    if (rc != DD_OK) return rc;
    const dim3 grid((unsigned)(dd_ceil_div(P.total_quads, DWB_BM / 2) * (P.cout_pad / DWB_BN)));
    if (relu6) hipLaunchKernelGGL((dwpw_big_k<STRIDE, ACT_RELU6, ACT_RELU6>), grid, dim3(512), lds_bytes, s, P);
    else hipLaunchKernelGGL((dwpw_big_k<STRIDE, -1, -1>), grid, dim3(512), lds_bytes, s, P);
    DD_LAUNCH_CHECK();
    return DD_OK;
}


bool mars_ws_on() {
    static const bool on = !(getenv("DD_MARS_WS") && atoi(getenv("DD_MARS_WS")) == 0);
    return on;
}
bool mars_ws_s1_eligible(const ConvP &P) {
    return mars_ws_on() && P.kh == 3 && P.kw == 3 && P.stride == 1 && P.pad_t == 1 && P.pad_l == 1 && P.H == 8 && P.W == 4 && P.ho == 8 && P.wo == 4 &&
           P.cin == 128 && P.cout == 128 && P.cout_pad == 128 && P.kpad >= 1152 && P.epi == EPI_F16 && P.cs_in % 8 == 0 && P.coff_in % 8 == 0 &&
           P.cs_out % 8 == 0 && P.coff_out % 8 == 0 &&
           ((P.act == ACT_ELU && !P.res && !P.out2) || (P.act == ACT_NONE && P.res && P.cs_res % 8 == 0 && P.coff_res % 8 == 0 && (!P.out2 || (P.cs_out2 % 8 == 0 && P.coff_out2 % 8 == 0))));
}
bool mars_ws_s2_eligible(const ConvP &P) {
    return mars_ws_on() && P.kh == 3 && P.kw == 3 && P.stride == 2 && P.pad_t == 0 && P.pad_l == 0 && P.H == 16 && P.W == 8 && P.ho == 8 && P.wo == 4 &&
           P.cin == 64 && P.cout == 128 && P.cout_pad == 128 && P.kpad >= 576 && P.epi == EPI_F16 && P.act == ACT_ELU && !P.res && !P.out2 &&
           P.cs_in % 8 == 0 && P.coff_in % 8 == 0 && P.cs_out % 8 == 0 && P.coff_out % 8 == 0;
}
bool mars_proj_follows(const dd_net *net, int i, const ConvP &P) {
    const int32_t *q = net->prog.data() + net->ops_off + (size_t)(i + 1) * OP_WORDS;
    if (q[0] != OP_CONV || q[5] != 1 || q[6] != 1 || q[7] != 2 || q[8] != 0 || q[9] != 0 || q[10] != 64 || q[11] != 128 || q[12] != 128 ||
        q[14] != ACT_NONE || q[15] != EPI_F16 || q[3] >= 0 || q[4] >= 0 || q[13] < 64 || q[1] < 0 || q[2] < 0) return false;
    const TensorDesc &qs = net->tensors[q[1]], &qd = net->tensors[q[2]];
    return qs.h == 16 && qs.w == 8 && qd.h == 8 && qd.w == 4 && qs.cs % 8 == 0 && qs.coff % 8 == 0 && qd.cs % 8 == 0 && qd.coff % 8 == 0 && qd.dtype == DT_F16;
}
int mars_pair_match(const dd_net *net, int i, int nimg, MarsPairP &Q, bool &first) {
    void *const *bufs = net->bufs.data();
    static const bool off = getenv("DD_MARS_PAIR") && atoi(getenv("DD_MARS_PAIR")) == 0;
    static const int min_crops = getenv("DD_MARS_PAIR_MIN") ? atoi(getenv("DD_MARS_PAIR_MIN")) : 256;
    if (off || nimg < min_crops) return 0;
    auto op = [&](int k) { return net->prog.data() + net->ops_off + (size_t)k * OP_WORDS; };
    auto W = [&](const int32_t *o, int word) { return net->d_weights + (size_t)(uint32_t)o[word]; };
    auto conv3 = [&](const int32_t *o, int stride, int cin, int act) {
        return o[0] == OP_CONV && o[5] == 3 && o[6] == 3 && o[7] == stride && o[10] == cin && o[11] == 64 && o[12] == 64 && o[14] == act && o[15] == EPI_F16 &&
               o[8] == 1 && o[9] == 1 && o[13] >= 9 * cin && o[1] >= 0 && o[2] >= 0 && !o[29];
    };
    auto t16x8 = [&](int t, int c) { const TensorDesc &d = net->tensors[t]; return d.h == 16 && d.w == 8 && d.c == c && d.cs % 8 == 0 && d.coff % 8 == 0 && d.dtype == DT_F16; };
    auto t31x15 = [&](int t) { const TensorDesc &d = net->tensors[t]; return d.h == 31 && d.w == 15 && d.c == 32 && d.cs % 8 == 0 && d.coff % 8 == 0 && d.dtype == DT_F16; };
    memset(&Q, 0, sizeof(Q));
    const int32_t *a = op(i);
    int nb;
    if (i + 2 < net->n_ops && a[30] == 3 && conv3(a, 2, 32, ACT_ELU) && a[3] < 0 && a[4] < 0 && t31x15(a[1]) && t16x8(a[2], 64)) {
        const int32_t *p = op(i + 1);
        if (!(p[30] == 4 && p[0] == OP_CONV && p[5] == 1 && p[6] == 1 && p[7] == 2 && p[8] == 0 && p[9] == 0 && p[10] == 32 && p[11] == 64 && p[12] == 64 &&
              p[14] == ACT_NONE && p[15] == EPI_F16 && p[3] < 0 && p[4] < 0 && p[13] >= 32 && p[1] >= 0 && p[2] >= 0 && t31x15(p[1]) && t16x8(p[2], 64))) return 0;
        first = true; nb = i + 2;
        const TensorDesc &ti = net->tensors[a[1]], &tr = net->tensors[p[1]];
        Q.in = reinterpret_cast<const _Float16 *>(bufs[ti.buf]); Q.cs_in = ti.cs; Q.coff_in = ti.coff;
        Q.in2 = reinterpret_cast<const _Float16 *>(bufs[tr.buf]); Q.cs_in2 = tr.cs; Q.coff_in2 = tr.coff;
        Q.wp = reinterpret_cast<const _Float16 *>(W(p, 16)); Q.kpad_p = p[13]; Q.bias_p = reinterpret_cast<const float *>(W(p, 17));
        const int32_t *b = op(nb);
        if (b[3] != p[2]) return 0;
    } else if (i + 1 < net->n_ops && a[30] == 4 && conv3(a, 1, 64, ACT_ELU) && a[3] < 0 && a[4] < 0 && t16x8(a[1], 64) && t16x8(a[2], 64)) {
        first = false; nb = i + 1;
        const TensorDesc &ti = net->tensors[a[1]];
        Q.in = reinterpret_cast<const _Float16 *>(bufs[ti.buf]); Q.cs_in = ti.cs; Q.coff_in = ti.coff;
        const int32_t *b = op(nb);
        if (b[3] < 0 || !t16x8(b[3], 64)) return 0;
        const TensorDesc &tr = net->tensors[b[3]];
        Q.res = reinterpret_cast<const _Float16 *>(bufs[tr.buf]); Q.cs_res = tr.cs; Q.coff_res = tr.coff;
    } else return 0;
    const int32_t *b = op(nb);
    if (!(conv3(b, 1, 64, ACT_NONE) && b[1] == a[2] && b[3] >= 0 && b[4] >= 0 && b[19] && t16x8(b[2], 64) && t16x8(b[4], 64))) return 0;
    Q.wa = reinterpret_cast<const _Float16 *>(W(a, 16)); Q.kpad_a = a[13]; Q.bias_a = reinterpret_cast<const float *>(W(a, 17));
    Q.wb = reinterpret_cast<const _Float16 *>(W(b, 16)); Q.kpad_b = b[13]; Q.bias_b = reinterpret_cast<const float *>(W(b, 17));
    const TensorDesc &to = net->tensors[b[2]], &t2 = net->tensors[b[4]];
    Q.out = reinterpret_cast<_Float16 *>(bufs[to.buf]); Q.cs_out = to.cs; Q.coff_out = to.coff;
    Q.out2 = reinterpret_cast<_Float16 *>(bufs[t2.buf]); Q.cs_out2 = t2.cs; Q.coff_out2 = t2.coff;
    Q.aff2 = reinterpret_cast<const float *>(W(b, 18)); Q.cout_pad = b[12];
    Q.zero = net->d_zero; Q.n_img = nimg;
    return nb - i + 1;
}

MarsWsP mars_ws_params(const ConvP &P, int nimg) {
    MarsWsP Q;
    memset(&Q, 0, sizeof(Q));
    Q.in = P.in; Q.cs_in = P.cs_in; Q.coff_in = P.coff_in;
    Q.w = P.w; Q.kpad = P.kpad; Q.bias = P.bias;
    Q.res = P.res; Q.cs_res = P.cs_res; Q.coff_res = P.coff_res;
    Q.out = static_cast<_Float16 *>(P.out); Q.cs_out = P.cs_out; Q.coff_out = P.coff_out;
    Q.out2 = P.out2; Q.cs_out2 = P.cs_out2; Q.coff_out2 = P.coff_out2; Q.aff2 = P.aff2; Q.cout_pad = P.cout_pad;
    Q.zero = P.zero; Q.n_img = nimg;
    return Q;
}

}

extern "C" {

static int net_create(dd_ctx *ctx, const int32_t *program_host, int n_words, const void *weights_host,
                      int64_t n_weight_bytes, int max_batch, dd_net **out, bool share);
int dd_net_destroy(dd_net *n);

int dd_net_create(dd_ctx *ctx, const int32_t *program_host, int n_words, const void *weights_host,
                  int64_t n_weight_bytes, int max_batch, dd_net **out) {
    return net_create(ctx, program_host, n_words, weights_host, n_weight_bytes, max_batch, out, false);
}

int dd_net_create_shared(dd_ctx *ctx, const int32_t *program_host, int n_words, const void *weights_host,
                         int64_t n_weight_bytes, int max_batch, dd_net **out) {
    return net_create(ctx, program_host, n_words, weights_host, n_weight_bytes, max_batch, out, true);
}

static int net_create(dd_ctx *ctx, const int32_t *program_host, int n_words, const void *weights_host,
                      int64_t n_weight_bytes, int max_batch, dd_net **out, bool share) {
    DD_REQUIRE(ctx && program_host && weights_host && out && max_batch > 0 && n_words >= 8, DD_E_ARG,
               "dd_net_create: bad argument");
    DD_REQUIRE(program_host[0] == 0x314E4444, DD_E_ARG, "dd_net_create: bad program magic");
    const int nt = program_host[1], nb = program_host[2], no = program_host[3];
    DD_REQUIRE(n_words == 8 + nt * TENSOR_WORDS + nb * 2 + no * OP_WORDS, DD_E_ARG, "dd_net_create: program size mismatch");
    dd_net *n = new dd_net();
    struct Guard { dd_net *n; ~Guard() { if (n) (void)dd_net_destroy(n); } } guard{n};
    n->ctx = ctx;
    n->max_batch = max_batch;
    n->prog.assign(program_host, program_host + n_words);
    n->in_h = program_host[4];
    n->in_w = program_host[5];
    n->out_tensor = program_host[6];
    const int32_t *p = program_host + 8;
    for (int i = 0; i < nt; ++i, p += TENSOR_WORDS) n->tensors.push_back(TensorDesc{p[0], p[1], p[2], p[3], p[4], p[5], p[6], p[7]});
    DD_HIP(hipSetDevice(ctx->device));
    if (share) {
        const int32_t *ops = p + (size_t)nb * 2;
        std::vector<int> first(nb, -1), last(nb, -1);
        for (int t = 0; t < nt; ++t) DD_REQUIRE(n->tensors[t].buf >= 0 && n->tensors[t].buf < nb, DD_E_ARG, "dd_net_create_shared: tensor %d names buffer %d of %d", t, n->tensors[t].buf, nb);
        for (int i = 0; i < no; ++i)
            DD_REQUIRE((ops + (size_t)i * OP_WORDS)[0] < 16, DD_E_ARG, "dd_net_create_shared: uint8 programs keep one buffer per tensor (their borders are set once)");
        std::vector<int> gs(no), ge(no);
        for (int i = 0; i < no;) {
            int j = i;
            while (j + 1 < no && (ops + (size_t)j * OP_WORDS)[30] != 0) ++j;
            for (int k = i; k <= j; ++k) { gs[k] = i; ge[k] = j; }
            i = j + 1;
        }
        auto touch2 = [&](int t, int i) {
            if (t < 0 || t >= nt) return;
            const int b = n->tensors[t].buf;
            first[b] = first[b] < 0 ? gs[i] : std::min(first[b], gs[i]);
            last[b] = std::max(last[b], ge[i]);
        };
        for (int i = 0; i < no; ++i) {
            const int32_t *o = ops + (size_t)i * OP_WORDS;
            touch2(o[1], i); touch2(o[2], i); touch2(o[3], i); touch2(o[4], i);
        }
        if (n->out_tensor >= 0) last[n->tensors[n->out_tensor].buf] = no;
        std::vector<size_t> bytes(nb), off(nb, 0);
        size_t arena = 0;
        std::vector<int> order(nb);
        for (int b = 0; b < nb; ++b) { order[b] = b; bytes[b] = ((size_t)p[2 * b] * max_batch * dtype_size(p[2 * b + 1] & 0xff) + 256 + 255) & ~(size_t)255; }
        std::stable_sort(order.begin(), order.end(), [&](int a, int b) { return first[a] < first[b]; });
        std::vector<int> placed;
        for (int b : order) {
            if (first[b] < 0) { first[b] = 0; last[b] = no; }
            size_t at = 0;
            for (bool moved = true; moved;) {
                moved = false;
                for (int q : placed)
                    if (!(last[q] < first[b] || last[b] < first[q]) && at < off[q] + bytes[q] && off[q] < at + bytes[b]) { at = off[q] + bytes[q]; moved = true; }
            }
            off[b] = at;
            arena = std::max(arena, at + bytes[b]);
            placed.push_back(b);
        }
        DD_HIP(hipMalloc(&n->arena, arena));
        DD_HIP(hipMemset(n->arena, 0, arena));
        n->arena_bytes = (int64_t)arena;
// ... 42 lines not shown
    if (n->arena) (void)hipFree(n->arena);
    else for (void *b : n->bufs) (void)hipFree(b);
    for (hipEvent_t e : n->events) (void)hipEventDestroy(e);
    net_drop_graphs(n);
    n->slab.release();
    (void)hipFree(n->d_zero);
    (void)hipFree(n->d_weights);
    for (void *q : {(void *)n->d_anchors, (void *)n->dec_boxes, (void *)n->dec_score, (void *)n->dec_keys, (void *)n->dec_cls}) (void)hipFree(q);
    delete n;
    return DD_OK;
}

int dd_net_activation_bytes(dd_net *n, int64_t *out_host) {
    DD_REQUIRE(n && out_host, DD_E_ARG, "dd_net_activation_bytes: NULL argument");
    if (n->arena) { *out_host = n->arena_bytes; return DD_OK; }
    int64_t tot = 0;
    for (size_t i = 0; i < n->bufs.size(); ++i) tot += n->buf_elems[i] * n->max_batch * (int64_t)dtype_size(n->buf_dtype[i]) + 256;
    *out_host = tot;
    return DD_OK;
}

int dd_net_last_batch(dd_net *n, int *out_host) {
    DD_REQUIRE(n && out_host, DD_E_ARG, "dd_net_last_batch: NULL argument");
    *out_host = n->last_batch;
    return DD_OK;
}

int dd_net_input_size(dd_net *n, int *h_host, int *w_host) {
    DD_REQUIRE(n && h_host && w_host, DD_E_ARG, "dd_net_input_size: NULL argument");
    *h_host = n->in_h; *w_host = n->in_w;
    return DD_OK;
}

int dd_net_max_batch(dd_net *n, int *out_host) {
    DD_REQUIRE(n && out_host, DD_E_ARG, "dd_net_max_batch: NULL argument");
    *out_host = n->max_batch;
    return DD_OK;
}

int dd_net_output(dd_net *n, int tensor, void **dev_ptr, int *h, int *w, int *c, int *cs, int *dtype) {
    DD_REQUIRE(n, DD_E_ARG, "dd_net_output: NULL net");
    const int t = tensor < 0 ? n->out_tensor : tensor;
    DD_REQUIRE(t >= 0 && t < (int)n->tensors.size(), DD_E_ARG, "dd_net_output: tensor %d out of range", t);
    const TensorDesc &d = n->tensors[t];
    if (dev_ptr) *dev_ptr = static_cast<char *>(n->bufs[d.buf]) + (size_t)d.coff * dtype_size(d.dtype);
    if (h) *h = d.h;
    if (w) *w = d.w;
    if (c) *c = d.c;
    if (cs) *cs = d.cs;
    if (dtype) *dtype = d.dtype;
    return DD_OK;
}

int dd_net_profile(dd_net *n, int enable) {
    DD_REQUIRE(n, DD_E_ARG, "dd_net_profile: NULL net");
    DD_DEVICE(n->ctx);
    if (enable && n->events.empty()) {
        n->events.resize(n->n_ops + 2);
        for (auto &e : n->events) DD_HIP(hipEventCreate(&e));
    }
    n->profile = enable != 0;
    return DD_OK;
}

int dd_net_profile_read(dd_net *n, float *ms_host, int cap, int *n_ops_host) {
    DD_REQUIRE(n && ms_host && n_ops_host, DD_E_ARG, "dd_net_profile_read: NULL argument");
    DD_DEVICE(n->ctx);
    DD_REQUIRE(n->profile && !n->events.empty(), DD_E_STATE, "dd_net_profile_read: profiling is off");
    DD_REQUIRE(cap >= n->n_ops, DD_E_ARG, "dd_net_profile_read: cap %d < %d ops", cap, n->n_ops);
    DD_HIP(hipEventSynchronize(n->events[n->n_ops + 1]));
    float empty = 0.f;
    DD_HIP(hipEventElapsedTime(&empty, n->events[n->n_ops], n->events[n->n_ops + 1]));
    for (int i = 0; i < n->n_ops; ++i) {
        DD_HIP(hipEventElapsedTime(&ms_host[i], n->events[i], n->events[i + 1]));
        ms_host[i] = ms_host[i] > empty ? ms_host[i] - empty : 0.f;
    }
    *n_ops_host = n->n_ops;
    return DD_OK;
}

int dd_net_op_launches(dd_net *n, int32_t *codes_host, int cap, int *n_ops_host) {
    DD_REQUIRE(n && codes_host && n_ops_host, DD_E_ARG, "dd_net_op_launches: NULL argument");
    DD_REQUIRE(cap >= n->n_ops, DD_E_ARG, "dd_net_op_launches: cap %d < %d ops", cap, n->n_ops);
    for (int i = 0; i < n->n_ops; ++i) codes_host[i] = i < (int)n->op_launch.size() ? n->op_launch[i] : OPK_DEFAULT;
    *n_ops_host = n->n_ops;
    return DD_OK;
}

int dd_net_read(dd_net *n, int tensor, int n_img, void *dst, int dst_on_device, void *stream) {
    DD_REQUIRE(n && dst && n_img >= 0 && n_img <= n->max_batch, DD_E_ARG, "dd_net_read: bad argument");
    DD_DEVICE(n->ctx);
    const int t = tensor < 0 ? n->out_tensor : tensor;
    DD_REQUIRE(t >= 0 && t < (int)n->tensors.size(), DD_E_ARG, "dd_net_read: tensor %d out of range", t);
    const TensorDesc &d = n->tensors[t];
    DD_REQUIRE(!n->arena || t == n->out_tensor, DD_E_STATE, "dd_net_read: tensor %d of an engine whose buffers share memory by lifetime "
               "(dd_net_create_shared): only the output tensor outlives the forward", t);
    DD_REQUIRE(d.coff == 0, DD_E_ARG, "dd_net_read: tensor %d is a channel slice", t);
    for (int i = 0; i < n->n_ops && i < (int)n->op_launch.size(); ++i) {
        const int32_t *o = n->prog.data() + n->ops_off + (size_t)i * OP_WORDS;
        DD_REQUIRE(!(o[2] == t && n->op_launch[i] == OPK_SSD_HEAD_DEC), DD_E_STATE,
                   "dd_net_read: tensor %d (the SSD head matrix) was not written: the head layers decoded in their epilogue "
                   "(dd_net_ssd_decode); read dd_net_ssd_decoded instead", t);
        DD_REQUIRE(!(o[2] == t && n->op_launch[i] == OPK_YOLO_HEAD_DEC), DD_E_STATE,
                   "dd_net_read: tensor %d (the Detect matrix) was not written: the head layers reduced their rows in their epilogue "
                   "(dd_net_yolo_decode); read dd_net_yolo_decoded instead", t);
        DD_REQUIRE(!((o[2] == t || o[4] == t) && n->op_launch[i] == OPK_FOLDED), DD_E_STATE,
                   "dd_net_read: tensor %d was not written by the last forward (op %d ran inside the next op's launch at this batch "
                   "size and its output stayed on chip); run a smaller batch or a program compiled without the fusion flags", t, i);
    }
    hipStream_t s = dd_pick_stream(n->ctx, stream);
    const size_t bytes = d.pad ? (size_t)n_img * (d.h + 2) * (d.w + 2) * d.cs
                               : (size_t)n_img * d.h * d.w * d.cs * dtype_size(d.dtype);
    if (!bytes) return DD_OK;
    DD_HIP(hipMemcpyAsync(dst, n->bufs[d.buf], bytes, dst_on_device ? hipMemcpyDeviceToDevice : hipMemcpyDeviceToHost, s));
    if (!dst_on_device) DD_HIP(hipStreamSynchronize(s));
    return DD_OK;
}

static int net_run_ops(dd_net *net, const uint8_t *input, int nimg, hipStream_t s);

int dd_net_use_graph(dd_net *net, int enable) {
    DD_REQUIRE(net, DD_E_ARG, "dd_net_use_graph: NULL net");
    DD_DEVICE(net->ctx);
    net->use_graph = enable != 0;
    if (!net->use_graph) net_drop_graphs(net);
    return DD_OK;
}

int dd_net_ssd_decode(dd_net *net, const float *anchors_host, int n_anchors, float score_thr, int enable) {
    DD_REQUIRE(net, DD_E_ARG, "dd_net_ssd_decode: NULL net");
    DD_DEVICE(net->ctx);
    net_drop_graphs(net);
    if (!enable) { net->ssd_dec = false; return DD_OK; }
    DD_REQUIRE(anchors_host && n_anchors > 0, DD_E_ARG, "dd_net_ssd_decode: anchors missing");
    int heads = 0;
    for (int i = 0; i < net->n_ops; ++i) {
        const int32_t *o = net->prog.data() + net->ops_off + (size_t)i * OP_WORDS;
        if (o[0] == OP_CONV && o[15] == EPI_SSD_HEAD) {
            DD_REQUIRE(o[18] && o[21] == n_anchors && 4 + o[20] <= 96, DD_E_ARG,
                       "dd_net_ssd_decode: head op %d has no per-anchor weight copy, or %d anchors / %d classes do not fit", i, o[21], o[20]);
            ++heads;
        }
        if (o[0] == 20) {
            DD_REQUIRE(o[21] == n_anchors, DD_E_ARG, "dd_net_ssd_decode: the program decodes %d anchors, %d given", o[21], n_anchors);
            ++heads;
        }
    }
    DD_REQUIRE(heads > 0, DD_E_ARG, "dd_net_ssd_decode: the program has no SSD head");
    if (net->dec_anchors != n_anchors) {
        for (void *q : {(void *)net->d_anchors, (void *)net->dec_boxes, (void *)net->dec_score, (void *)net->dec_keys, (void *)net->dec_cls}) (void)hipFree(q);
        net->d_anchors = net->dec_boxes = net->dec_score = net->dec_keys = nullptr; net->dec_cls = nullptr; net->dec_anchors = 0;
        const size_t per = (size_t)net->max_batch * n_anchors;
        DD_HIP(hipMalloc(&net->d_anchors, (size_t)n_anchors * 4 * sizeof(float)));
        DD_HIP(hipMalloc(&net->dec_boxes, per * 4 * sizeof(float)));
        DD_HIP(hipMalloc(&net->dec_score, per * sizeof(float)));
        DD_HIP(hipMalloc(&net->dec_keys, per * sizeof(float)));
        DD_HIP(hipMalloc(&net->dec_cls, per * sizeof(int)));
        net->dec_anchors = n_anchors;
    }
    DD_HIP(hipMemcpy(net->d_anchors, anchors_host, (size_t)n_anchors * 4 * sizeof(float), hipMemcpyHostToDevice));
    net->dec_thr = score_thr;
    net->ssd_dec = true;
    return DD_OK;
}

int dd_net_yolo_decode(dd_net *net, int enable) {
    DD_REQUIRE(net, DD_E_ARG, "dd_net_yolo_decode: NULL net");
    DD_DEVICE(net->ctx);
    net_drop_graphs(net);
    if (!enable) { net->yolo_dec = false; return DD_OK; }
    DD_REQUIRE(!net->ssd_dec, DD_E_STATE, "dd_net_yolo_decode: the SSD decode is on for this network");
    int heads = 0, rows = 0;
    for (int i = 0; i < net->n_ops; ++i) {
        const int32_t *o = net->prog.data() + net->ops_off + (size_t)i * OP_WORDS;
        if (o[0] == OP_CONV && o[15] == EPI_YOLO) {
            DD_REQUIRE(o[18] && !o[19] && o[20] >= 6 && o[20] <= 96, DD_E_ARG,
                       "dd_net_yolo_decode: head op %d has no per-anchor weight copy, or %d columns per row do not fit", i, o[20]);
            DD_REQUIRE(rows == 0 || rows == o[21], DD_E_ARG, "dd_net_yolo_decode: heads disagree on the rows per image");
            rows = o[21];
            ++heads;
        }
    }
    DD_REQUIRE(heads > 0 && rows > 0, DD_E_ARG, "dd_net_yolo_decode: the program has no YOLOv5 Detect head");
    if (net->dec_anchors != rows || !net->dec_boxes) {
        for (void *q : {(void *)net->d_anchors, (void *)net->dec_boxes, (void *)net->dec_score, (void *)net->dec_keys, (void *)net->dec_cls}) (void)hipFree(q);
        net->d_anchors = net->dec_boxes = net->dec_score = net->dec_keys = nullptr; net->dec_cls = nullptr; net->dec_anchors = 0;
        const size_t per = (size_t)net->max_batch * rows;
        DD_HIP(hipMalloc(&net->dec_boxes, per * 4 * sizeof(float)));
// ... 26 lines not shown
}


int dd_net_ssd_decoded(dd_net *net, float **boxes, float **scores, int **classes, float **keys) {
    DD_REQUIRE(net && net->ssd_dec, DD_E_STATE, "dd_net_ssd_decoded: dd_net_ssd_decode is off");
    if (boxes) *boxes = net->dec_boxes;
    if (scores) *scores = net->dec_score;
    if (classes) *classes = net->dec_cls;
    if (keys) *keys = net->dec_keys;
    return DD_OK;
}

int dd_net_ssd_heads_u8(dd_net *net, const uint8_t **box_q, const uint8_t **cls_q, int *cls_stride, const uint8_t **lut, float *quant4_host,
                        int *n_anchors, int *n_classes) {
    DD_REQUIRE(net && box_q && cls_q && cls_stride && lut && quant4_host && n_anchors && n_classes, DD_E_ARG, "dd_net_ssd_heads_u8: NULL argument");
    DD_REQUIRE(!net->arena, DD_E_STATE, "dd_net_ssd_heads_u8: the engine's buffers share memory by lifetime (dd_net_create_shared): the head "
               "tensors do not outlive the forward");
    for (int i = 0; i < net->n_ops; ++i) {
        const int32_t *o = net->prog.data() + net->ops_off + (size_t)i * OP_WORDS;
        if (o[0] != 20) continue;
        DD_REQUIRE(o[1] >= 0 && o[1] < (int)net->tensors.size() && o[3] >= 0 && o[3] < (int)net->tensors.size(), DD_E_ARG, "dd_net_ssd_heads_u8: head tensors out of range");
        const TensorDesc &tb = net->tensors[o[1]], &tc = net->tensors[o[3]];
        DD_REQUIRE(tb.cs == 4 && tb.h == o[21] && tc.h == o[21] && tb.w == 1 && tc.w == 1 && o[20] <= tc.cs && !tb.pad && !tc.pad && !tb.coff && !tc.coff, DD_E_ARG,
                   "dd_net_ssd_heads_u8: head tensors of %d anchors are not [anchors][4] / [anchors][>= %d] bytes", o[21], o[20]);
        *box_q = static_cast<const uint8_t *>(net->bufs[tb.buf]); *cls_q = static_cast<const uint8_t *>(net->bufs[tc.buf]);
        *cls_stride = tc.cs; *n_anchors = o[21]; *n_classes = o[20];
        *lut = reinterpret_cast<const uint8_t *>(net->d_weights + (size_t)(uint32_t)o[16]);
        const float *of = reinterpret_cast<const float *>(o);
        for (int q = 0; q < 4; ++q) quant4_host[q] = of[32 + q];
        return DD_OK;
    }
    DD_REQUIRE(false, DD_E_ARG, "dd_net_ssd_heads_u8: the program has no uint8 SSD head");
}

int dd_net_ssd_decoded_read(dd_net *net, int n, float *boxes_host, float *scores_host, int *classes_host, float *keys_host) {
    DD_REQUIRE(net && net->ssd_dec && n >= 0 && n <= net->max_batch, DD_E_STATE, "dd_net_ssd_decoded_read: decode is off or n out of range");
    DD_DEVICE(net->ctx);
    hipStream_t s = net->ctx->stream;
    DD_HIP(hipStreamSynchronize(s));
    const size_t per = (size_t)n * net->dec_anchors;
    if (!per) return DD_OK;
    if (boxes_host) DD_HIP(hipMemcpy(boxes_host, net->dec_boxes, per * 4 * sizeof(float), hipMemcpyDeviceToHost));
    if (scores_host) DD_HIP(hipMemcpy(scores_host, net->dec_score, per * sizeof(float), hipMemcpyDeviceToHost));
    if (classes_host) DD_HIP(hipMemcpy(classes_host, net->dec_cls, per * sizeof(int), hipMemcpyDeviceToHost));
    if (keys_host) DD_HIP(hipMemcpy(keys_host, net->dec_keys, per * sizeof(float), hipMemcpyDeviceToHost));
    return DD_OK;
}

int dd_net_forward(dd_net *net, const uint8_t *input, int nimg, void *stream) {
    DD_REQUIRE(net && input && nimg >= 0, DD_E_ARG, "dd_net_forward: bad argument");
    DD_DEVICE(net->ctx);
    DD_REQUIRE(nimg <= net->max_batch, DD_E_CAPACITY, "dd_net_forward: batch %d > max_batch %d", nimg, net->max_batch);
    if (nimg == 0) return DD_OK;
    net->last_batch = nimg;
    hipStream_t s = dd_pick_stream(net->ctx, stream);
    auto eager = [&]() -> int {
        const int rc = net_run_ops(net, input, nimg, s);
        if (net->slab_moved) { net->slab_moved = false; net_drop_graphs(net); }
        return rc;
    };
    if (!net->use_graph || net->profile) return eager();
    if (net->graphs.size() > 256) net_drop_graphs(net);
    dd_net::GraphEntry &g = net->graphs[std::make_pair(static_cast<const void *>(input), nimg)];
    if (g.exec) { DD_HIP(hipGraphLaunch(g.exec, s)); return DD_OK; }
    if (g.calls++ == 0) return eager();
    DD_HIP(hipStreamBeginCapture(s, hipStreamCaptureModeThreadLocal));
    const int rc = net_run_ops(net, input, nimg, s);
    hipGraph_t graph = nullptr;
    const hipError_t e = hipStreamEndCapture(s, &graph);
    if (rc != DD_OK) { if (graph) (void)hipGraphDestroy(graph); return rc; }
    DD_HIP(e);
    g.graph = graph;
    DD_HIP(hipGraphInstantiate(&g.exec, graph, nullptr, nullptr, 0));
    DD_HIP(hipGraphLaunch(g.exec, s));
    return DD_OK;
}

static int net_run_ops(dd_net *net, const uint8_t *input, int nimg, hipStream_t s) {
    auto base = [&](int t) -> char * {
        const TensorDesc &d = net->tensors[t];
        return static_cast<char *>(net->bufs[d.buf]);
    };
    net->op_launch.assign((size_t)net->n_ops, OPK_DEFAULT);
    ConvP stem_p;
    bool stem_pending = false;
    bool wide_pending = false, wide_ready = false;
    bool input_pending = false;
    float input_mean = 0.f, input_scale = 1.f;
    int input_op = -1;
    ConvP unit_a;
    bool unit_pending = false;
    ConvP pw_p;
    bool pw_pending = false;
    bool proj_done = false;
    MarsPairP pair64;
    bool pair64_first = false;
    int pair_left = 0;
    ConvP pair_a, pair_b;
    bool pair_pending = false;
    int pair_op = -1;
    auto flush_pair = [&]() -> int {
        pair_pending = false;
        net->op_launch[pair_op] = OPK_RES_UNIT;
        return launch_res_unit(s, pair_a, pair_b, nimg, net->ctx->device);
    };
    auto run_ws = [&](ConvP &P) { return P.cin == 256 ? launch_conv_ws<4>(s, P, net->ctx->device) : launch_conv_ws<8>(s, P, net->ctx->device); };
    int first_op = 0;
    bool mid_on = false;
    {
        static const int chunk_env = getenv("DD_Q_FRONT_CHUNK") ? atoi(getenv("DD_Q_FRONT_CHUNK")) : 0;
        auto opw = [&](int k) { return net->prog.data() + net->ops_off + (size_t)k * OP_WORDS; };
        const char *front_env = getenv("DD_Q_FRONT"), *front_min_env = getenv("DD_Q_FRONT_MIN");
        const int front_min = front_min_env ? atoi(front_min_env) : 24;
        {
            const char *mid_env = getenv("DD_Q_MID");
            mid_on = !(mid_env && atoi(mid_env) == 0) && nimg >= front_min;
        }
        if (!(front_env && atoi(front_env) == 0) && chunk_env <= 0 && nimg >= front_min && net->n_ops > 3 && opw(0)[0] == 16 && opw(1)[0] == 19 && opw(2)[0] == 19) {
            if (net->profile) for (int k = 0; k < 3; ++k) DD_HIP(hipEventRecord(net->events[k], s));
            int ran = 0;
            const int rc = netq_run_front(net, opw(0), opw(1), opw(2), input, nimg, s, &ran);
            if (rc != DD_OK) return rc;
            if (ran) { first_op = 3; net->op_launch[0] = OPK_FOLDED; net->op_launch[1] = OPK_FOLDED; net->op_launch[2] = OPK_Q_FRONT; }
        }
        if (first_op == 0 && chunk_env > 0 && nimg > chunk_env && net->n_ops > 3 && opw(0)[0] == 16 && opw(1)[0] == 19 && opw(2)[0] == 19 && opw(1)[1] == opw(0)[2] && opw(2)[1] == opw(1)[2]) {
            const TensorDesc &t2 = net->tensors[opw(2)[2]];
            const size_t img_out = (size_t)(t2.h + 2) * (t2.w + 2) * t2.cs;
            void *&out_buf = net->bufs[t2.buf];
            void *const out_base = out_buf;
            if (net->profile) for (int k = 0; k < 3; ++k) DD_HIP(hipEventRecord(net->events[k], s));
            for (int c0 = 0; c0 < nimg; c0 += chunk_env) {
                const int nc = std::min(chunk_env, nimg - c0);
                out_buf = static_cast<char *>(out_base) + (size_t)c0 * img_out;
                for (int k = 0; k < 3; ++k) {
                    int handled = 0;
                    const int rc = netq_run_op(net, k, opw(k), input + (size_t)c0 * net->in_h * net->in_w * 3, nc, s, &handled);
                    if (rc != DD_OK || !handled) { out_buf = out_base; return rc != DD_OK ? rc : DD_E_ARG; }
                }
            }
            out_buf = out_base;
            first_op = 3;
        }
    }
    for (int i = first_op; i < net->n_ops; ++i) {
        if (net->profile) DD_HIP(hipEventRecord(net->events[i], s));
        const int32_t *o = net->prog.data() + net->ops_off + (size_t)i * OP_WORDS;
        const float *of = reinterpret_cast<const float *>(o);
        const int kind = o[0], src = o[1], dst = o[2], res = o[3], dst2 = o[4];
        const TensorDesc *ts = src >= 0 ? &net->tensors[src] : nullptr;
        const TensorDesc *td = dst >= 0 ? &net->tensors[dst] : nullptr;
        DD_REQUIRE(!input_pending || (kind == OP_CONV && i == input_op + 1), DD_E_STATE, "dd_net_forward: input op %d was folded into an op that did not take it", input_op);
        if (mid_on && kind == 19 && i + 1 < net->n_ops && net->prog[net->ops_off + (size_t)(i + 1) * OP_WORDS] == 19) {
            const int32_t *o4 = net->prog.data() + net->ops_off + (size_t)(i + 1) * OP_WORDS;
            if (net->profile) DD_HIP(hipEventRecord(net->events[i + 1], s));
            int ran = 0;
            const int rc = netq_run_mid(net, o, o4, nimg, s, &ran);
            if (rc != DD_OK) return rc;
            if (ran) { net->op_launch[i] = OPK_FOLDED; net->op_launch[i + 1] = OPK_Q_MID; ++i; continue; }
        }
        DD_REQUIRE((!wide_pending || kind == OP_CONV) && (!wide_ready || kind == OP_MAXPOOL), DD_E_STATE, "dd_net_forward: op %d does not take the first layer folded into it", i);
        if (pair_pending && kind != OP_CONV) { const int rc = flush_pair(); if (rc != DD_OK) return rc; }
        if (pw_pending && kind != OP_DWCONV) {
            pw_pending = false; net->op_launch[i - 1] = OPK_CONV_WS;
            const int rc = run_ws(pw_p);
            if (rc != DD_OK) return rc;
        }
        if (unit_pending && kind != OP_CONV) {
            unit_pending = false; net->op_launch[i - 1] = OPK_DEFAULT;
            const int rc = launch_conv3x3_rw(s, unit_a, nimg, false, net->ctx->device);
            if (rc != DD_OK) return rc;
        }
        if (stem_pending && !(kind == OP_CONV && o[29]) && kind != OP_DWPW) {
            stem_pending = false; net->op_launch[i - 1] = OPK_DEFAULT;
            const int rc = launch_stem(s, stem_p, nimg);
            if (rc != DD_OK) return rc;
        }
        switch (kind) {
            case OP_INPUT: {
                const int s2d = o[5];
                const int m = nimg * td->h * td->w;
                if (s2d && o[30] && !o[6] && td->cs == 32 && !td->coff && i + 1 < net->n_ops && net->use_rw) {
                    const int32_t *q = net->prog.data() + net->ops_off + (size_t)(i + 1) * OP_WORDS;
                    static const bool off = getenv("DD_FOCUS_UNFUSED") && atoi(getenv("DD_FOCUS_UNFUSED")) != 0;
                    if (!off && q[0] == OP_CONV && q[1] == dst && q[5] == 3 && q[6] == 3 && q[7] == 1 && q[8] == 1 && q[9] == 1 && q[10] == 32 &&
                        q[12] == 32 && q[14] == ACT_SILU && q[15] == EPI_F16 && q[3] < 0 && q[4] < 0 && !q[29] && td->w % 32 == 0) {
                        input_pending = true; input_mean = of[32]; input_scale = of[33]; input_op = i;
                        net->op_launch[i] = OPK_FOLDED;
                        break;
                    }
                }
                if (s2d && td->cs >= 16 && td->cs % 8 == 0) {
                    const int cpp = td->cs / 8;
                    DD_REQUIRE((long long)m * cpp < (1ll << 31), DD_E_CAPACITY, "dd_net_forward: %d x %d input chunks", m, cpp);
                    hipLaunchKernelGGL(input_s2d_chunks_k, dim3(dd_ceil_div(m * cpp, 256)), dim3(256), 0, s, input, net->in_h, net->in_w, o[6],
                                       of[32], of[33], m * cpp, cpp, reinterpret_cast<_Float16 *>(base(dst)) + td->coff, td->cs);
                } else
                hipLaunchKernelGGL(input_k, dim3(dd_ceil_div(m, 256)), dim3(256), 0, s, input, net->in_h, net->in_w, o[6],
                                   of[32], of[33], s2d, m, reinterpret_cast<_Float16 *>(base(dst)) + td->coff, td->cs);
                DD_LAUNCH_CHECK();
                break;
            }
            case OP_CONV: {
#define DD_NO_PENDING() DD_REQUIRE(!unit_pending && !pair_pending && !stem_pending && !pw_pending && !input_pending, DD_E_STATE, \
                                   "dd_net_forward: op %d is folded into a neighbouring launch while an earlier op's launch is still held back", i)
                if (proj_done) { DD_NO_PENDING(); proj_done = false; net->op_launch[i] = OPK_FOLDED_PREV; break; }
                if (pair_left > 0) {
                    DD_NO_PENDING();
                    if (--pair_left > 0) { net->op_launch[i] = OPK_FOLDED; break; }
                    const int rc = mars_pair64_launch(s, net->ctx->device, pair64, pair64_first);
                    if (rc != DD_OK) return rc;
                    net->op_launch[i] = OPK_MARS_PAIR;
                    break;
                }
                if (o[30] == 3 || o[30] == 4) {
                    const int n_ops = mars_pair_match(net, i, nimg, pair64, pair64_first);
                    if (n_ops) { DD_NO_PENDING(); pair_left = n_ops - 1; net->op_launch[i] = OPK_FOLDED; break; }
                }
#undef DD_NO_PENDING
                ConvP P;
                memset(&P, 0, sizeof(P));
                P.in = reinterpret_cast<const _Float16 *>(base(src)); P.H = ts->h; P.W = ts->w; P.cs_in = ts->cs;
                P.coff_in = ts->coff; P.cin = o[10];
                P.kh = o[5]; P.kw = o[6]; P.stride = o[7]; P.pad_t = o[8]; P.pad_l = o[9];
                P.cout = o[11]; P.cout_pad = o[12]; P.kpad = o[13]; P.act = o[14]; P.epi = o[15];
                P.w = reinterpret_cast<const _Float16 *>(net->d_weights + (size_t)(uint32_t)o[16]);
                P.bias = reinterpret_cast<const float *>(net->d_weights + (size_t)(uint32_t)o[17]);
                P.ho = o[26]; P.wo = o[27]; P.m = nimg * P.ho * P.wo;
                P.out = base(dst); P.cs_out = td->cs; P.coff_out = td->coff;
                if (res >= 0) {
                    const TensorDesc &tr = net->tensors[res];
                    P.res = reinterpret_cast<const _Float16 *>(base(res)); P.cs_res = tr.cs; P.coff_res = tr.coff;
                }
                if (dst2 >= 0) {
                    const TensorDesc &t2 = net->tensors[dst2];
                    P.out2 = reinterpret_cast<_Float16 *>(base(dst2)); P.cs_out2 = t2.cs; P.coff_out2 = t2.coff;
                    P.aff2 = reinterpret_cast<const float *>(net->d_weights + (size_t)(uint32_t)o[18]);
                }
                if (dst2 < 0 && o[19]) {
                    P.aff2 = reinterpret_cast<const float *>(net->d_weights + (size_t)(uint32_t)o[18]);
                    P.post_aff = 1;
                }
                for (int q = 0; q < 6; ++q) P.p[q] = o[20 + q];
                for (int q = 0; q < 8; ++q) P.f[q] = of[32 + q];
                int rc;
                DD_REQUIRE(!o[29] || (net->use_rw && P.kh == 3 && P.stride == 1 && P.cin == 32 && P.cout_pad == 32), DD_E_ARG,
                           "dd_net_forward: fused pooling is only built for the 3x3 32->32 kernel");
                if (unit_pending) {
                    unit_pending = false;
                    if (res_unit_fusable(unit_a, P, nimg)) {
                        P.zero = net->d_zero;
                        if (pair_pending) {
                            if (res_pair_fusable(pair_a, pair_b, unit_a, P, nimg)) {
                                pair_pending = false;
                                rc = launch_res_pair(s, pair_a, pair_b, unit_a, P, nimg, net->ctx->device);
                                if (rc != DD_OK) return rc;
                                net->op_launch[i] = OPK_RES_PAIR;
                                break;
                            }
                            if ((rc = flush_pair()) != DD_OK) return rc;
                        }
                        if (o[30] == 2 && i + 2 < net->n_ops) {
                            pair_a = unit_a; pair_b = P; pair_pending = true; pair_op = i;
                            net->op_launch[i] = OPK_FOLDED;
                            break;
                        }
                        rc = launch_res_unit(s, unit_a, P, nimg, net->ctx->device);
                        if (rc != DD_OK) return rc;
                        net->op_launch[i] = OPK_RES_UNIT;
                        break;
                    }
                    if (pair_pending && (rc = flush_pair()) != DD_OK) return rc;
                    net->op_launch[i - 1] = OPK_DEFAULT;
                    rc = launch_conv3x3_rw(s, unit_a, nimg, false, net->ctx->device);
                    if (rc != DD_OK) return rc;
                }
                if (pair_pending) {
                    const bool next_a = net->use_rw && P.kh == 3 && P.kw == 3 && P.stride == 1 && P.cin == 32 && P.cout_pad == 32 && P.epi == EPI_F16 &&
                                        P.pad_t == 1 && P.pad_l == 1 && o[30] && !o[29] && i + 1 < net->n_ops && nimg >= 160 && !P.res && !P.out2 &&
                                        P.in == static_cast<const _Float16 *>(pair_b.out2);
                    if (!next_a && (rc = flush_pair()) != DD_OK) return rc;
                }
                if (P.epi == EPI_YOLO && net->yolo_dec && o[18] && !o[19]) {
                    DD_REQUIRE(P.p[1] == net->dec_anchors, DD_E_ARG, "dd_net_forward: head of %d rows, decode set up for %d", P.p[1], net->dec_anchors);
                    P.w = reinterpret_cast<const _Float16 *>(net->d_weights + (size_t)(uint32_t)o[18]);
                    P.bias = reinterpret_cast<const float *>(net->d_weights + (size_t)(uint32_t)o[31]);
                    P.zero = net->d_zero;
                    P.dec_boxes = net->dec_boxes; P.dec_score = net->dec_score; P.dec_cls = net->dec_cls;
                    rc = launch_yolo_head_dec(s, P);
                    if (rc != DD_OK) return rc;
                    net->op_launch[i] = OPK_YOLO_HEAD_DEC;
                    break;
                }
                if (P.epi == EPI_SSD_HEAD && net->ssd_dec && o[18] && !o[19]) {
                    DD_REQUIRE(P.p[1] == net->dec_anchors, DD_E_ARG, "dd_net_forward: head of %d anchors, decode set up for %d", P.p[1], net->dec_anchors);
                    P.w = reinterpret_cast<const _Float16 *>(net->d_weights + (size_t)(uint32_t)o[18]);
                    P.bias = reinterpret_cast<const float *>(net->d_weights + (size_t)(uint32_t)o[31]);
                    P.zero = net->d_zero;
                    P.anchors = net->d_anchors; P.dec_boxes = net->dec_boxes; P.dec_score = net->dec_score; P.dec_keys = net->dec_keys;
                    P.dec_cls = net->dec_cls; P.dec_thr = net->dec_thr;
                    rc = launch_ssd_head_dec(s, P);
                    if (rc != DD_OK) return rc;
                    net->op_launch[i] = OPK_SSD_HEAD_DEC;
                    break;
                }
                const bool bk32 = o[28] == 32;
                const bool glds = !bk32 && net->use_glds;
                P.zero = net->d_zero;
                if (net->use_rw && P.kh == 3 && P.kw == 3 && P.stride == 1 && P.cin == 32 && P.cout_pad == 32 &&
                    P.epi == EPI_F16 && P.pad_t == 1 && P.pad_l == 1) {
                    if (input_pending) { input_pending = false; P.src8 = input; P.in_mean = input_mean; P.in_scale = input_scale; }
                    if (o[29]) { P.p[0] = td->h; P.p[1] = td->w; }
                    if (wide_pending) {
                        wide_pending = false;
                        const int32_t *r = o + OP_WORDS;
                        const TensorDesc &tp = net->tensors[r[2]];
                        P.src8 = stem_p.src8; P.in_mean = stem_p.in_mean; P.in_scale = stem_p.in_scale;
                        P.dw_w = stem_p.w; P.dw_bias = stem_p.bias; P.dw_act = stem_p.act;
                        P.out = base(r[2]); P.cs_out = tp.cs; P.coff_out = tp.coff; P.p[0] = tp.h; P.p[1] = tp.w;
                        stem_p = P; wide_ready = true; net->op_launch[i] = OPK_FOLDED;
                        break;
                    }
                    if (stem_pending) {
                        stem_pending = false;
                        if (o[29] && pool_rows_fusable(P, nimg) && stem_p.out == static_cast<const void *>(P.in) && !P.coff_in) {
                            P.src8 = stem_p.src8; P.in_mean = stem_p.in_mean; P.in_scale = stem_p.in_scale;
                            P.dw_w = stem_p.w; P.dw_bias = stem_p.bias; P.dw_act = stem_p.act;
                        } else {
                            net->op_launch[i - 1] = OPK_DEFAULT;
                            rc = launch_stem(s, stem_p, nimg);
                            if (rc != DD_OK) return rc;
                        }
                    }
                    if (o[30] && !o[29] && i + 1 < net->n_ops && nimg >= 160 && !P.res && !P.out2) {
                        if (pair_pending && P.in != static_cast<const _Float16 *>(pair_b.out2) && (rc = flush_pair()) != DD_OK) return rc;
                        unit_a = P; unit_pending = true;
                        net->op_launch[i] = OPK_FOLDED;
                        break;
                    }
                    if (o[29] && pool_rows_fusable(P, nimg)) net->op_launch[i] = P.src8 ? OPK_POOL_ROWS_STEM : OPK_POOL_ROWS;
                    rc = launch_conv3x3_rw(s, P, nimg, o[29] != 0, net->ctx->device);
                } else if (mars_ws_s1_eligible(P)) {
                    const MarsWsP Q = mars_ws_params(P, nimg);
                    net->op_launch[i] = OPK_MARS_WS;
                    rc = mars_ws128_launch(s, net->ctx->device, Q, P.res ? MARS_WS_S1_RES : MARS_WS_S1, P.act, P.out2 != nullptr);
                } else if (o[30] == 3 && i + 1 < net->n_ops && mars_ws_s2_eligible(P) && mars_proj_follows(net, i, P)) {
                    const int32_t *q = net->prog.data() + net->ops_off + (size_t)(i + 1) * OP_WORDS;
                    const TensorDesc &qs = net->tensors[q[1]], &qd = net->tensors[q[2]];
                    MarsWsP Q = mars_ws_params(P, nimg);
                    Q.in2 = reinterpret_cast<const _Float16 *>(base(q[1])); Q.cs_in2 = qs.cs; Q.coff_in2 = qs.coff;
                    Q.w2 = reinterpret_cast<const _Float16 *>(net->d_weights + (size_t)(uint32_t)q[16]); Q.kpad2 = q[13];
                    Q.bias2 = reinterpret_cast<const float *>(net->d_weights + (size_t)(uint32_t)q[17]);
                    Q.out2 = reinterpret_cast<_Float16 *>(base(q[2])); Q.cs_out2 = qd.cs; Q.coff_out2 = qd.coff;
                    net->op_launch[i] = OPK_MARS_WS;
                    rc = mars_ws128_launch(s, net->ctx->device, Q, MARS_WS_S2_PROJ, P.act, false);
                    proj_done = true;
                } else if (s2_rows_eligible(P, nimg, net->max_batch)) {
                    net->op_launch[i] = OPK_S2_ROWS;
                    rc = launch_conv3x3_s2_rows(s, P, nimg, net->ctx->device);
                } else if (c64_rows_eligible(P, nimg, net->max_batch)) {
                    net->op_launch[i] = OPK_C64_ROWS;
                    rc = launch_conv3x3_c64_rows(s, P, nimg, net->ctx->device);
                } else if (c64_strips_eligible(P, nimg, net->max_batch)) {
                    net->op_launch[i] = OPK_C64_STRIPS;
                    rc = launch_conv3x3_c64_strips(s, P, nimg, net->ctx->device);
                } else if (ws_eligible(P) && o[30] && i + 1 < net->n_ops && P.act == ACT_RELU6) {
                    pw_p = P; pw_pending = true; net->op_launch[i] = OPK_FOLDED;
                    break;
                } else if (ws_eligible(P)) {
                    net->op_launch[i] = OPK_CONV_WS;
                    rc = P.cin == 256 ? launch_conv_ws<4>(s, P, net->ctx->device) : launch_conv_ws<8>(s, P, net->ctx->device);
                } else if (P.cout_pad <= 32) {
                    rc = bk32 ? launch_conv<4, 1, 1, 2, 32, false>(s, P, net->slab, net->max_batch, net->ctx->device, &net->slab_moved)
                       : (glds && P.m >= 16384) ? launch_conv<4, 1, 2, 2, 64, true>(s, P, net->slab, net->max_batch, net->ctx->device, &net->slab_moved)
                       : glds ? launch_conv<4, 1, 1, 2, 64, true>(s, P, net->slab, net->max_batch, net->ctx->device, &net->slab_moved)
                              : launch_conv<4, 1, 1, 2, 64, false>(s, P, net->slab, net->max_batch, net->ctx->device, &net->slab_moved);
                } else if (glds && net->tile_mode != 1 && P.m >= 16384 && P.cout_pad >= 128) {
                    const int gy128 = dd_ceil_div(P.cout_pad, 128);
                    const int c128 = dd_ceil_div(dd_ceil_div(P.m, 128) * gy128, 512) * 128;
                    const int c192 = dd_ceil_div(dd_ceil_div(P.m, 192) * gy128, 512) * 192;
                    if (P.epi == EPI_F16 && c192 <= c128 && net->tile_mode != 2)
                        rc = launch_conv<4, 2, 3, 4, 64, true>(s, P, net->slab, net->max_batch, net->ctx->device, &net->slab_moved);
                    else
                        rc = launch_conv<4, 2, 2, 4, 64, true>(s, P, net->slab, net->max_batch, net->ctx->device, &net->slab_moved);
                } else if (glds && net->tile_mode != 1 && P.m >= 16384 && P.cout_pad == 64) {
                    rc = launch_conv<4, 2, 2, 2, 64, true>(s, P, net->slab, net->max_batch, net->ctx->device, &net->slab_moved);
                } else if (glds && net->tile_mode != 1 && P.m >= 4096 && P.cout_pad >= 128) {
                    rc = launch_conv<2, 2, 2, 4, 64, true>(s, P, net->slab, net->max_batch, net->ctx->device, &net->slab_moved);
                } else {
                    rc = bk32 ? launch_conv<2, 2, 2, 2, 32, false>(s, P, net->slab, net->max_batch, net->ctx->device, &net->slab_moved)
                       : glds ? launch_conv<2, 2, 2, 2, 64, true>(s, P, net->slab, net->max_batch, net->ctx->device, &net->slab_moved)
                              : launch_conv<2, 2, 2, 2, 64, false>(s, P, net->slab, net->max_batch, net->ctx->device, &net->slab_moved);
                }
                if (rc != DD_OK) return rc;
                break;
            }
            case OP_STEM: {
                ConvP P;
                memset(&P, 0, sizeof(P));
                P.src8 = input; P.H = net->in_h; P.W = net->in_w; P.in_mean = of[32]; P.in_scale = of[33];
                P.zero = net->d_zero;
                P.kh = P.kw = 3; P.stride = o[7]; P.pad_t = o[8]; P.pad_l = o[9];
                P.cout = o[11]; P.cout_pad = o[12]; P.act = o[14]; P.epi = EPI_F16; P.splitk = 1;
                DD_REQUIRE(P.cout_pad == 32 && (P.stride == 1 || P.stride == 2), DD_E_ARG, "dd_net_forward: stem needs 32 output channels, stride 1 or 2");
                P.w = reinterpret_cast<const _Float16 *>(net->d_weights + (size_t)(uint32_t)o[16]);
                P.bias = reinterpret_cast<const float *>(net->d_weights + (size_t)(uint32_t)o[17]);
                P.ho = td->h; P.wo = td->w; P.m = nimg * P.ho * P.wo;
                P.out = base(dst); P.cs_out = td->cs; P.coff_out = td->coff;
                static const bool unfused = getenv("DD_STEM_UNFUSED") && atoi(getenv("DD_STEM_UNFUSED")) != 0;
                if (o[30] && !unfused && i + 1 < net->n_ops && P.stride == 1 && P.pad_t == 1 && P.pad_l == 1 && P.cout == 32 && P.act == ACT_ELU &&
                    P.W == 32 && (reinterpret_cast<uintptr_t>(input) & 3) == 0) {
                    stem_p = P; stem_pending = true; net->op_launch[i] = OPK_FOLDED;
                    break;
                }
                auto sole_reader = [&](int t, int reader) {
                    if (t < 0 || t == net->out_tensor) return false;
                    for (int k = 0; k < net->n_ops; ++k) {
                        const int32_t *w = net->prog.data() + net->ops_off + (size_t)k * OP_WORDS;
                        for (int a : {w[1], w[3]})
                            if (k != reader && a >= 0 && net->tensors[a].buf == net->tensors[t].buf) return false;
                    }
                    return true;
                };
                const char *wide_env = getenv("DD_STEM_WIDE"), *wide_min_env = getenv("DD_STEM_WIDE_MIN");
                const bool wide_off = wide_env ? atoi(wide_env) == 0 : !STEM_WIDE_DEFAULT;
                const int wide_min = wide_min_env ? atoi(wide_min_env) : STEM_WIDE_MIN_CROPS;
                if (o[30] && !wide_off && nimg >= wide_min && i + 2 < net->n_ops && net->use_rw && stem_wide_geometry(P.H, P.W) && P.stride == 1 &&
                    P.pad_t == 1 && P.pad_l == 1 && P.cout == 32 && P.act == ACT_ELU && !td->coff && (reinterpret_cast<uintptr_t>(input) & 3) == 0) {
                    const int32_t *q = o + OP_WORDS, *r = o + 2 * OP_WORDS;
                    if (q[0] == OP_CONV && q[1] == dst && q[5] == 3 && q[6] == 3 && q[7] == 1 && q[8] == 1 && q[9] == 1 && q[10] == 32 && q[11] == 32 && q[12] == 32 &&
                        q[14] == ACT_ELU && q[15] == EPI_F16 && q[3] < 0 && q[4] < 0 && !q[29] && !q[30] &&
                        r[0] == OP_MAXPOOL && r[1] == q[2] && r[5] == 3 && r[6] <= 1 && r[7] == 2 && r[8] == 0 && r[2] >= 0 && sole_reader(q[2], i + 2) &&
                        net->tensors[r[2]].h == P.H / 2 - 1 && net->tensors[r[2]].w == P.W / 2 - 1 && net->tensors[r[2]].c == 32) {
                        stem_p = P; wide_pending = true; net->op_launch[i] = OPK_FOLDED;
                        break;
                    }
// ... 149 lines not shown
```

deepdish_amd/profile.py:

```python
import ctypes
import numpy as np

from ._lib import lib, check
from .runtime import ptr

PEAK_F16_TFLOPS = 2500.0
PEAK_HBM_GBS = 8000.0
PEAK_I8_TOPS = 5000.0


def last_batch(net):
    n = ctypes.c_int()
    check(lib().dd_net_last_batch(net._h, ctypes.byref(n)), 'dd_net_last_batch')
    return n.value


def net_op_times(net):
    n = len(net.program.ops)
    ms = np.zeros(n, dtype=np.float32)
    cnt = ctypes.c_int()
    check(lib().dd_net_profile_read(net._h, ptr(ms), n, ctypes.byref(cnt)), 'dd_net_profile_read')
    return ms


OPK_FOLDED = 1
OPK_NAMES = {2: 'conv3x3_pool_rows_k', 3: 'conv3x3_pool_rows_k<STEM>', 4: 'res_unit_rows_k', 5: 'ssd_front_k', 6: 'conv3x3_c64_rows_k', 7: 'conv3x3_s2_rows_k', 8: 'conv_ws_k', 9: 'conv_ws_dw_k', 10: 'dwpw_rows_k', 11: 'conv_glds_k<ssd_head_decode>', 12: 'res_pair_rows_k', 13: 'conv_glds_k<yolo_head_decode>', 14: 'mars_ws128_k', 16: 'mars_pair64_k', 17: 'q_dwm_k', 18: 'conv3x3_c64_rows_k<strips>', 19: 'q_front_k', 20: 'q_mid_k', 21: 'q_conv_k<add>', 22: 'q_add_k', 23: 'stem_conv_pool_wide_k'}
OPK_FOLDED_PREV = 15


def net_op_launches(net):
    n = len(net.program.ops)
    codes = np.zeros(n, dtype=np.int32)
    cnt = ctypes.c_int(0)
    check(lib().dd_net_op_launches(net._h, ptr(codes), n, ctypes.byref(cnt)), 'dd_net_op_launches')
    return codes


def launches_of(net, ms, batch):
    out, pend = [], None
    for t, info, code in zip(ms, net.program.info, net_op_launches(net)):
        fl, by = info['flops'] * batch, info['bytes'] * batch + info.get('wbytes', 0)
        if code == OPK_FOLDED:
            if pend is None:
                pend = [float(t), fl, info.get('src_bytes', 0) * batch + info.get('wbytes', 0)]
            else:
                pend[0] += float(t); pend[1] += fl; pend[2] += info.get('wbytes', 0)
            continue
        if code == OPK_FOLDED_PREV and out:
            k0, t0, f0, b0 = out[-1]
            out[-1] = (k0, t0 + float(t), f0 + fl, b0 + by)
            continue
        if pend is not None:
            t, fl, by = float(t) + pend[0], fl + pend[1], by - info.get('src_bytes', 0) * batch + pend[2]
            pend = None
        out.append((OPK_NAMES.get(int(code), info['kernel']), float(t), fl, by))
    return out


def profile_nets(run_once, nets_with_batch, reps=20):
    for _, net, _ in nets_with_batch:
        check(lib().dd_net_profile(net._h, 1), 'dd_net_profile')
    acc = {}
    try:
        for _ in range(reps):
            run_once()
            for name, net, batch in nets_with_batch:
                ms = net_op_times(net)
                b = batch() if callable(batch) else batch
                for kname, t, fl, by in launches_of(net, ms, b):
                    k = acc.setdefault(kname, dict(ms=0.0, flops=0.0, bytes=0.0, launches=0))
                    k['ms'] += t; k['flops'] += fl; k['bytes'] += by; k['launches'] += 1
    finally:
        for _, net, _ in nets_with_batch:
            check(lib().dd_net_profile(net._h, 0), 'dd_net_profile')
    for k in acc.values():
        for f in ('ms', 'flops', 'bytes'):
            k[f] /= reps
        k['launches'] /= reps
    return acc


def pmc_traffic(kernel, streams):
    import json, os
    root = os.path.join(os.path.dirname(os.path.dirname(os.path.abspath(__file__))), 'profiles')
    path = next((p for p in (os.path.join(root, 'r%02d_pmc_traffic_s%d.json' % (r, streams)) for r in (6, 5, 4, 3, 2, 1)) if os.path.exists(p)), None)
    if path is None:
        return None, None
    keys = [part.replace(',', ', ') for part in kernel.split('+')]
    tot_b = tot_n = 0.0
    for k, v in json.load(open(path)).items():
        if any(key in k for key in keys):
            tot_b += (v['hbm_read_bytes_corrected'] + v['hbm_write_bytes']) * v['launches']
            tot_n += v['launches']
    src = 'profiles/%s (rocprofv3 --pmc FETCH_SIZE and WRITE_SIZE passes of `bench.py --groups 1 --streams %d`, committed; not measured in this run)' % (os.path.basename(path), streams)
    return (tot_b / tot_n, src) if tot_n else (None, None)


def dominant_kernel_roofline(pipes, step_group, args, reps=20):
    f0 = args.warmup
    p = pipes[0]
    nets = [('mars', p.enc, lambda: last_batch(p.enc))]
    if p.det is not None:
        nets.append(('ssd', p.det, p.S))
    state = dict(f=f0)

    def run_once():
        step_group(0, state['f'])
        state['f'] = f0 + (state['f'] + 1 - f0) % max(1, args.steps)

    acc = profile_nets(run_once, nets, reps)
    per_kernel = {n: round(v['ms'], 5) for n, v in sorted(acc.items(), key=lambda kv: -kv[1]['ms'])}
    fam = [n for n in ('conv_glds_k', 'conv_ws_k', 'conv_ws_dw_k', 'conv_glds_k<ssd_head_decode>') if n in acc]
    if len(fam) > 1:
        parts = [acc.pop(n) for n in fam]
        acc['+'.join(fam)] = {f: sum(p[f] for p in parts) for f in ('ms', 'flops', 'bytes', 'launches')}
    name, k = max(acc.items(), key=lambda kv: kv[1]['ms'])
    sec = k['ms'] * 1e-3
    avg_us = 1e3 * k['ms'] / max(k['launches'], 1e-9)
# ... 18 lines not shown
```

include/deepdish_hip.h:

```cpp
#ifndef DEEPDISH_HIP_H
#define DEEPDISH_HIP_H

#include <stdint.h>

#ifdef __cplusplus
extern "C" {
#endif

#define DD_OK            0
#define DD_E_ARG        -1
#define DD_E_HIP        -2
#define DD_E_STATE      -3
#define DD_E_CAPACITY   -4

#define DD_FEATURE_DIM 128

typedef struct dd_ctx dd_ctx;
typedef struct dd_tracker dd_tracker;
typedef struct dd_net dd_net;
typedef struct dd_pipeline dd_pipeline;

const char *dd_last_error(void);
int dd_version(void);

// ... 27 lines not shown
           int *out_idx, int *out_n, void *stream);

int dd_nms_ssd(dd_ctx *ctx, const double *xyxy, const double *scores, int k, double iou_thr,
               int *out_idx, int *out_n, void *stream);

int dd_lsap_host(const double *cost_host, int nr, int nc, int *row_ind_host, int *col_ind_host);

int dd_pyset_difference_order_host(const int *a_host, int na, const int *b_host, int nb, int *out_host,
                                   int *out_n_host);

int dd_tracker_create(dd_ctx *ctx, double max_cosine_distance, double max_iou_distance,
                      int max_age, int n_init, int nn_budget ,
                      int track_capacity, int gallery_capacity, dd_tracker **out);
int dd_tracker_create_metric(dd_ctx *ctx, int metric, double matching_threshold, double max_iou_distance,
                             int max_age, int n_init, int nn_budget ,
                             int track_capacity, int gallery_capacity, dd_tracker **out);
int dd_tracker_destroy(dd_tracker *trk);
int dd_tracker_predict(dd_tracker *trk);
int dd_tracker_update(dd_tracker *trk, const double *tlwh_host, const float *feats,
                      int feats_on_device, int n);
int dd_tracker_count(dd_tracker *trk, int which, int *out_n_host);
int dd_tracker_read(dd_tracker *trk, int which, int64_t *ints6_host, double *means_host,
                    double *covs_host);
int dd_tracker_track_update(dd_tracker *t, int64_t track_id, const double *tlwh_host, const float *feat, int feat_on_device);
int dd_tracker_track_predict(dd_tracker *t, int64_t track_id);
int dd_tracker_track_set(dd_tracker *t, int64_t track_id, int state, int time_since_update);
int dd_tracker_remove(dd_tracker *t, const int64_t *track_ids_host, int n);
int dd_tracker_next_id(dd_tracker *trk, int64_t *out_host);

int dd_tracker_last_cost(dd_tracker *trk, double *app_host, double *iou_host, int cap, int *rows_host, int *cols_host);
int dd_tracker_last_matches(dd_tracker *trk, int *pairs_host, int cap, int *out_m_host);

int dd_crop_resize(dd_ctx *ctx, const uint8_t *frame, int H, int W, const int64_t *boxes_host,
                   int n, int ph, int pw, uint8_t *out, int *valid_host, void *stream);
int dd_crop_resize_f64(dd_ctx *ctx, const uint8_t *frame, int H, int W, const double *boxes_host, int n, int ph,
                       int pw, uint8_t *out, int *valid_host, void *stream);

int dd_fake_encode(dd_ctx *ctx, const uint8_t *patches, int n, int mode, float *out, void *stream);

int dd_resize_lanczos(dd_ctx *ctx, const uint8_t *src, int H, int W, int src_c, int swap_rb,
                      uint8_t *dst, int h, int w, void *stream);
int dd_resize_lanczos_batch(dd_ctx *ctx, const uint8_t *src, int batch, int H, int W, int src_c, int swap_rb,
                            uint8_t *dst, int h, int w, void *stream);
int dd_resize_bilinear(dd_ctx *ctx, const uint8_t *src, int H, int W, int c,
                       uint8_t *dst, int h, int w, void *stream);

typedef struct dd_ingest dd_ingest;
int dd_ingest_create(dd_ctx *ctx, int slots, int n_streams, int src_h, int src_w, int dst_h, int dst_w, int flip,
                     dd_ingest **out);
int dd_ingest_destroy(dd_ingest *g);
int dd_ingest_host_slot(dd_ingest *g, int slot, uint8_t **host_ptr, int64_t *n_bytes);
int dd_ingest_wait_uploaded(dd_ingest *g, int slot);
int dd_ingest_submit(dd_ingest *g, int slot);
int dd_ingest_acquire(dd_ingest *g, int slot, void *consumer_stream, const uint8_t **frames_dev);
int dd_ingest_release(dd_ingest *g, int slot, void *consumer_stream);

typedef struct dd_mog2 dd_mog2;
int dd_mog2_create(dd_ctx *ctx, int n_streams, int height, int width, int history, double var_threshold, int detect_shadows,
                   dd_mog2 **out);
int dd_mog2_destroy(dd_mog2 *m);
int dd_mog2_apply(dd_mog2 *m, const uint8_t *frames, double learning_rate, uint8_t *mask, uint8_t *masked_frames, void *stream);
int dd_mog2_state(dd_mog2 *m, int stream_index, float *weight_host, float *variance_host, float *mean_host, uint8_t *nmodes_host);
int dd_mask_box_count(dd_ctx *ctx, const uint8_t *mask, int n_streams, int height, int width, const int *boxes_xywh_host,
                      const int *box_stream_host, int n_boxes, int *counts_host, void *stream);

int dd_net_create(dd_ctx *ctx, const int32_t *program_host, int n_words, const void *weights_host,
                  int64_t n_weight_bytes, int max_batch, dd_net **out);
int dd_net_create_shared(dd_ctx *ctx, const int32_t *program_host, int n_words, const void *weights_host,
                         int64_t n_weight_bytes, int max_batch, dd_net **out);
int dd_net_activation_bytes(dd_net *net, int64_t *out_host);
int dd_net_destroy(dd_net *net);
int dd_net_forward(dd_net *net, const uint8_t *input, int n, void *stream);
int dd_net_output(dd_net *net, int tensor, void **dev_ptr_host, int *h_host, int *w_host, int *c_host,
                  int *cs_host, int *dtype_host);

int dd_net_use_graph(dd_net *net, int enable);
int dd_net_input_size(dd_net *net, int *h_host, int *w_host);
int dd_net_max_batch(dd_net *net, int *out_host);
int dd_net_last_batch(dd_net *net, int *out_host);
int dd_net_read(dd_net *net, int tensor, int n, void *dst, int dst_on_device, void *stream);

int dd_net_profile(dd_net *net, int enable);
int dd_net_profile_read(dd_net *net, float *ms_host, int cap, int *n_ops_host);
int dd_net_op_launches(dd_net *net, int32_t *codes_host, int cap, int *n_ops_host);

int dd_ssd_postprocess(dd_ctx *ctx, const float *raw, const float *anchors, int n_anchors,
                       int n_classes, int max_det, float score_thr, float iou_thr,
                       float *boxes, float *classes, float *scores, int *count, void *stream);

int dd_ssd_decode(dd_ctx *ctx, const float *raw, const float *anchors, int n_anchors, int n_classes, float score_thr,
                  float *boxes, float *scores, int *classes, float *keys, int batch, void *stream);
int dd_ssd_postprocess_decoded(dd_ctx *ctx, const float *dec_boxes, const float *dec_scores, const int *dec_classes,
                               const float *dec_keys, int n_anchors, int max_det, float score_thr, float iou_thr,
                               float *boxes, float *classes, float *scores, int *count, int batch, void *stream);
int dd_net_ssd_decode(dd_net *net, const float *anchors_host, int n_anchors, float score_thr, int enable);
int dd_net_ssd_decoded(dd_net *net, float **boxes_dev, float **scores_dev, int **classes_dev, float **keys_dev);
int dd_net_ssd_decoded_read(dd_net *net, int n, float *boxes_host, float *scores_host, int *classes_host, float *keys_host);

int dd_ssd_regular_nms_decoded(dd_ctx *ctx, const float *dec_boxes, const float *scores_in, int score_ld, int first_class_col,
                               int n_anchors, int n_classes, int max_det, int detections_per_class, float score_thr, float iou_thr,
                               float *boxes, float *classes, float *scores, int *count, int batch, void *stream);
int dd_ssd_postprocess_regular(dd_ctx *ctx, const float *raw, const float *anchors, int n_anchors, int n_classes, int max_det,
                               int detections_per_class, float score_thr, float iou_thr, float *boxes, float *classes, float *scores,
                               int *count, int batch, void *stream);
int dd_ssd_postprocess_regular_u8(dd_ctx *ctx, const uint8_t *box_q, const uint8_t *cls_q, int cls_stride, const uint8_t *logistic_table,
                                  const float *quant4_host, const float *anchors, int n_anchors, int n_classes, int max_det,
                                  int detections_per_class, float score_thr, float iou_thr, float *boxes, float *classes, float *scores,
                                  int *count, int batch, void *stream);
int dd_net_ssd_heads_u8(dd_net *net, const uint8_t **box_q_dev, const uint8_t **cls_q_dev, int *cls_stride_host,
                        const uint8_t **logistic_table_dev, float *quant4_host, int *n_anchors_host, int *n_classes_host);

int dd_net_yolo_decode(dd_net *net, int enable);
int dd_net_yolo_decoded(dd_net *net, float **boxes, float **conf, int **classes, int *rows);
int dd_net_yolo_decoded_read(dd_net *net, int n, float *boxes_host, float *conf_host, int *classes_host);

int dd_ssd_detections(dd_ctx *ctx, const float *boxes, const float *classes, const float *scores, int batch,
                      int max_det, double confidence, double iou_thr, double img_w, double img_h, double *out_boxes,
                      int *out_cls, double *out_scores, int *out_n, void *stream);

int dd_yolov5_decode(dd_ctx *ctx, const float *raw, int n_rows, int n_cls, float thr,
                     float img_w, float img_h, float *out_boxes, float *out_scores,
                     int *out_cls, int cap, int *out_n, void *stream);

int dd_pipeline_create(dd_ctx *ctx, int n_streams, int frame_h, int frame_w, dd_net *detector,
                       const float *anchors_host, int n_anchors, int n_classes, dd_net *encoder,
                       const char *labels_nl, const char *wanted_nl, double max_cosine_distance,
                       double nms_max_overlap, double max_iou_distance, int max_age, int n_init,
                       const double *line_host, int track_capacity, int gallery_capacity, dd_pipeline **out);
int dd_pipeline_destroy(dd_pipeline *p);
int dd_pipeline_detector_adaptor(dd_pipeline *p, int adaptor);
int dd_pipeline_ssd_options(dd_pipeline *p, int max_detections, float nms_score_threshold, float nms_iou_threshold);
int dd_pipeline_ssd_regular_nms(dd_pipeline *p, int detections_per_class);
int dd_pipeline_detector_skip_frames(dd_pipeline *p, int n);
int dd_pipeline_metric(dd_pipeline *p, int metric);
int dd_pipeline_step(dd_pipeline *p, const uint8_t *frames, const double *inj_boxes_host,
                     const double *inj_scores_host, const int *inj_cls_host, const int *inj_offsets_host);
int dd_pipeline_step2(dd_pipeline *p, const uint8_t *frames, const uint8_t *frames_next, const double *inj_boxes_host,
                      const double *inj_scores_host, const int *inj_cls_host, const int *inj_offsets_host);
int dd_pipeline_detector_stream(dd_pipeline *p, void **stream_out);
int dd_pipeline_background_subtraction(dd_pipeline *p, double ratio, int masking);
int dd_pipeline_motion_mask(dd_pipeline *p, uint8_t *dst, int dst_on_device, long long *rejected_host);
int dd_pipeline_counts(dd_pipeline *p, int64_t *counts_host);
int dd_pipeline_tracker(dd_pipeline *p, int stream, dd_tracker **out);
int dd_pipeline_stage_seconds(dd_pipeline *p, double *out4_host, long long *steps_host);
int dd_pipeline_stage_gpu_ms(dd_pipeline *p, double *out6_host, long long *steps_host);
int dd_pipeline_detections(dd_pipeline *p, int stream, double *boxes_host, double *scores_host, int *classes_host, int cap, int *n_host);

int dd_counts_accumulate(dd_ctx *ctx, int64_t *acc, const int64_t *counts_host, int n, void *stream);

#ifdef __cplusplus
}
#endif
#endif
```

Measured before the change: 146,300 frames/s.

## Derive pre-activated MARS inputs in consumer kernels instead of writing second tensor

Producer kernels of the MARS encoder no longer write the separate affine+ELU output tensor (out2) when the next kernel can rebuild it. Consumer kernels now apply the scale/shift+ELU to the raw residual tile in LDS right after the DMA lands. This cuts one activation write and one activation read per residual block. The cost is extra ALU and LDS work plus an extra wait in the consumer's pipeline loop, and the wait counts change depending on whether out2 is present.

```diff
diff --git a/deepdish_amd/csrc/mars_pair.hip b/deepdish_amd/csrc/mars_pair.hip
--- a/deepdish_amd/csrc/mars_pair.hip
+++ b/deepdish_amd/csrc/mars_pair.hip
@@ -6,11 +6,7 @@
 typedef float f4 __attribute__((ext_vector_type(4)));
 typedef unsigned u4 __attribute__((ext_vector_type(4)));
 
-__device__ __forceinline__ float elu(float v) {
-    float e = __builtin_amdgcn_exp2f(v * 1.44269504088896340736f);
-    e = __builtin_amdgcn_fmed3f(e, 0.f, 1.f);
-    return __builtin_amdgcn_fmed3f(v, e - 1.f, 3.0e38f);
-}
+__device__ __forceinline__ float elu(float v) { return dd_mars_elu(v); }
 
 __device__ __forceinline__ void lds_fill16(const _Float16 *g, char *lds_wave_base) {
 #if defined(__HIP_DEVICE_COMPILE__)
@@ -30,9 +26,9 @@
 constexpr int pair_off_res(bool first) { return pair_off_h(first) + 2 * PT64_B; }
 constexpr int pair_off_raw(bool first) { return pair_off_res(first) + (first ? 2 : 3) * PPLAIN_B; }
 constexpr int pair_off_const(bool first) { return pair_off_raw(first) + (first ? 2 * PRAW_B : 0); }
-constexpr int pair_lds_bytes(bool first) { return pair_off_const(first) + 5 * 64 * 4; }
-
-template <bool FIRST>
+constexpr int pair_lds_bytes(bool first) { return pair_off_const(first) + 7 * 64 * 4; }
+
+template <bool FIRST, bool DERIVE>
 __global__ __launch_bounds__(512, 2) void mars_pair64_k(const MarsPairP P) {
     constexpr int OFF_IN = pair_off_in(FIRST), OFF_H = pair_off_h(FIRST), OFF_RES = pair_off_res(FIRST), OFF_RAW = pair_off_raw(FIRST),
                   OFF_C = pair_off_const(FIRST);
@@ -51,6 +47,9 @@
         cst[128 + tid] = P.aff2[tid];
         cst[192 + tid] = P.aff2[P.cout_pad + tid];
         cst[256 + tid] = (FIRST && P.bias_p) ? P.bias_p[tid] : 0.f;
+        constexpr int CIN = FIRST ? 32 : 64;
+        cst[320 + tid] = (DERIVE && tid < CIN) ? P.derive[tid] : 0.f;
+        cst[384 + tid] = (DERIVE && tid < CIN) ? P.derive[P.derive_pad + tid] : 0.f;
     }
     __syncthreads();
 
@@ -92,11 +91,14 @@
     int n_dma;
     if constexpr (FIRST) {
         const int par = lane >> 5, pl = (lane >> 3) & 3, col = 2 * (lane & 7) + par;
+        const _Float16 *tin = DERIVE ? P.in2 : P.in;
+        const int cs_t = DERIVE ? P.cs_in2 : P.cs_in, coff_t = DERIVE ? P.coff_in2 : P.coff_in;
 #pragma unroll
         for (int h = 0; h < 4; ++h) {
             const int r = wave + 8 * h < 31 ? wave + 8 * h : 30;
-            src[h] = col < 15 ? P.in + ((size_t)n0 * 31 + r) * 15 * P.cs_in + (size_t)col * P.cs_in + P.coff_in + pl * 8 : P.zero;
-            stp[h] = col < 15 ? (size_t)nstep * 31 * 15 * P.cs_in : 0;
+            const bool live = col < 15 && !(DERIVE && wave + 8 * h >= 31);
+            src[h] = live ? tin + ((size_t)n0 * 31 + r) * 15 * cs_t + (size_t)col * cs_t + coff_t + pl * 8 : P.zero;
+            stp[h] = live ? (size_t)nstep * 31 * 15 * cs_t : 0;
         }
         const int jr = lane >> 5, xx = lane & 7;
         src[4] = P.in2 + ((size_t)n0 * 31 + 2 * (2 * wave + jr)) * 15 * P.cs_in2 + (size_t)(2 * xx) * P.cs_in2 + P.coff_in2 + pl * 8;
@@ -106,8 +108,8 @@
         const int pl = lane >> 3, xx = lane & 7;
 #pragma unroll
         for (int h = 0; h < 2; ++h) {
-            src[h] = P.in + (((size_t)n0 * 16 + wave + 8 * h) * 8 + xx) * P.cs_in + P.coff_in + pl * 8;
-            stp[h] = (size_t)nstep * 128 * P.cs_in;
+            src[h] = DERIVE ? P.zero : P.in + (((size_t)n0 * 16 + wave + 8 * h) * 8 + xx) * P.cs_in + P.coff_in + pl * 8;
+            stp[h] = DERIVE ? 0 : (size_t)nstep * 128 * P.cs_in;
             src[2 + h] = P.res + (((size_t)n0 * 16 + wave + 8 * h) * 8 + xx) * P.cs_res + P.coff_res + pl * 8;
             stp[2 + h] = (size_t)nstep * 128 * P.cs_res;
         }
@@ -120,11 +122,13 @@
         char *T = smem + OFF_IN + (dq & 1) * TIN_B;
         if constexpr (FIRST) {
 #pragma unroll
-            for (int h = 0; h < 4; ++h) lds_fill16(src[h], T + ((wave + 8 * h < 31 ? wave + 8 * h : 30) + 1) * 1024);
+            for (int h = 0; h < 4; ++h) lds_fill16(src[h], T + ((wave + 8 * h < 31 ? wave + 8 * h : DERIVE ? 31 : 30) + 1) * 1024);
             lds_fill16(src[4], smem + OFF_RAW + (dq & 1) * PRAW_B + wave * 1024);
         } else {
-#pragma unroll
-            for (int h = 0; h < 2; ++h) lds_fill16(src[h], T + (wave + 8 * h + 1) * 1024);
+            if constexpr (!DERIVE) {
+#pragma unroll
+                for (int h = 0; h < 2; ++h) lds_fill16(src[h], T + (wave + 8 * h + 1) * 1024);
+            }
             const int rs = dq % 3;
 #pragma unroll
             for (int h = 0; h < 2; ++h) lds_fill16(src[2 + h], smem + OFF_RES + rs * PPLAIN_B + (wave + 8 * h) * 1024);
@@ -144,7 +148,43 @@
     for (int c = 0; c <= Kc; ++c) {
 #if defined(__HIP_DEVICE_COMPILE__)
         if (stage == 0 || c < 2) asm volatile("s_waitcnt vmcnt(0) lgkmcnt(0)" ::: "memory");
-        else asm volatile("s_waitcnt vmcnt(8) lgkmcnt(0)" ::: "memory");
+        else if (P.out2) asm volatile("s_waitcnt vmcnt(8) lgkmcnt(0)" ::: "memory");
+        else asm volatile("s_waitcnt vmcnt(4) lgkmcnt(0)" ::: "memory");
+        if constexpr (DERIVE) {
+            if (c < Kc) {
+                char *T = smem + OFF_IN + (c & 1) * TIN_B;
+                if constexpr (FIRST) {
+                    const int pl = (lane >> 3) & 3;
+                    const bool col15 = (lane >> 5) == 1 && (lane & 7) == 7;
+                    const f4 s0 = *reinterpret_cast<const f4 *>(cst + 320 + pl * 8), s1 = *reinterpret_cast<const f4 *>(cst + 320 + pl * 8 + 4);
+                    const f4 t0 = *reinterpret_cast<const f4 *>(cst + 384 + pl * 8), t1 = *reinterpret_cast<const f4 *>(cst + 384 + pl * 8 + 4);
+#pragma unroll
+                    for (int h = 0; h < 4; ++h) {
+                        if (wave + 8 * h >= 31) continue;
+                        h8 *pc = reinterpret_cast<h8 *>(T + (wave + 8 * h + 1) * 1024 + lane * 16);
+                        const h8 r = *pc;
+                        h8 o;
+#pragma unroll
+                        for (int i = 0; i < 4; ++i) { o[i] = dd_mars_pre(r[i], s0[i], t0[i]); o[4 + i] = dd_mars_pre(r[4 + i], s1[i], t1[i]); }
+                        if (!col15) *pc = o;
+                    }
+                } else {
+                    const int pl = lane >> 3;
+                    const f4 s0 = *reinterpret_cast<const f4 *>(cst + 320 + pl * 8), s1 = *reinterpret_cast<const f4 *>(cst + 320 + pl * 8 + 4);
+                    const f4 t0 = *reinterpret_cast<const f4 *>(cst + 384 + pl * 8), t1 = *reinterpret_cast<const f4 *>(cst + 384 + pl * 8 + 4);
+                    const char *R = smem + OFF_RES + (c % 3) * PPLAIN_B;
+#pragma unroll
+                    for (int h = 0; h < 2; ++h) {
+                        const h8 r = *reinterpret_cast<const h8 *>(R + (wave + 8 * h) * 1024 + lane * 16);
+                        h8 o;
+#pragma unroll
+                        for (int i = 0; i < 4; ++i) { o[i] = dd_mars_pre(r[i], s0[i], t0[i]); o[4 + i] = dd_mars_pre(r[4 + i], s1[i], t1[i]); }
+                        *reinterpret_cast<h8 *>(T + (wave + 8 * h + 1) * 1024 + lane * 16) = o;
+                    }
+                }
+            }
+            asm volatile("s_waitcnt lgkmcnt(0)" ::: "memory");
+        }
         __builtin_amdgcn_s_barrier();
         asm volatile("" ::: "memory");
 #endif
@@ -214,12 +254,14 @@
 #pragma unroll
                 for (int i = 0; i < 8; ++i) o[i] = (_Float16)v[i];
                 *reinterpret_cast<h8 *>(P.out + m * P.cs_out + P.coff_out + co) = o;
-                const f4 s0 = *reinterpret_cast<const f4 *>(cst + 128 + co), s1 = *reinterpret_cast<const f4 *>(cst + 128 + co + 4);
-                const f4 t0 = *reinterpret_cast<const f4 *>(cst + 192 + co), t1 = *reinterpret_cast<const f4 *>(cst + 192 + co + 4);
-                h8 o2;
-#pragma unroll
-                for (int i = 0; i < 4; ++i) { o2[i] = (_Float16)elu(s0[i] * v[i] + t0[i]); o2[4 + i] = (_Float16)elu(s1[i] * v[4 + i] + t1[i]); }
-                *reinterpret_cast<h8 *>(P.out2 + m * P.cs_out2 + P.coff_out2 + co) = o2;
+                if (P.out2) {
+                    const f4 s0 = *reinterpret_cast<const f4 *>(cst + 128 + co), s1 = *reinterpret_cast<const f4 *>(cst + 128 + co + 4);
+                    const f4 t0 = *reinterpret_cast<const f4 *>(cst + 192 + co), t1 = *reinterpret_cast<const f4 *>(cst + 192 + co + 4);
+                    h8 o2;
+#pragma unroll
+                    for (int i = 0; i < 4; ++i) { o2[i] = dd_mars_pre(o[i], s0[i], t0[i]); o2[4 + i] = dd_mars_pre(o[4 + i], s1[i], t1[i]); }
+                    *reinterpret_cast<h8 *>(P.out2 + m * P.cs_out2 + P.coff_out2 + co) = o2;
+                }
             }
         }
     }
@@ -228,19 +270,19 @@
 #endif
 }
 
-template <bool FIRST>
+template <bool FIRST, bool DERIVE>
 int launch_pair(hipStream_t s, int device, const MarsPairP &P) {
     constexpr int lds = pair_lds_bytes(FIRST);
     static_assert(lds <= 160 * 1024, "LDS budget");
     static DevOnce once;
     const int rc = once.run(device, [&]() -> int {
-        DD_HIP(hipFuncSetAttribute(reinterpret_cast<const void *>(&mars_pair64_k<FIRST>), hipFuncAttributeMaxDynamicSharedMemorySize, lds));
+        DD_HIP(hipFuncSetAttribute(reinterpret_cast<const void *>(&mars_pair64_k<FIRST, DERIVE>), hipFuncAttributeMaxDynamicSharedMemorySize, lds));
         return DD_OK;
     });
     if (rc != DD_OK) return rc;
     const int n_cu = dd_cu_count(device);
     const int grid = P.n_img < n_cu ? P.n_img : n_cu;
-    hipLaunchKernelGGL((mars_pair64_k<FIRST>), dim3(grid), dim3(512), lds, s, P);
+    hipLaunchKernelGGL((mars_pair64_k<FIRST, DERIVE>), dim3(grid), dim3(512), lds, s, P);
     DD_LAUNCH_CHECK();
     return DD_OK;
 }
@@ -248,7 +290,9 @@
 }
 
 int mars_pair64_launch(hipStream_t s, int device, const MarsPairP &P, bool first) {
-    DD_REQUIRE(P.n_img > 0 && P.in && P.wa && P.wb && P.bias_a && P.bias_b && P.out && P.out2 && P.aff2 && P.zero && (first ? (P.in2 && P.wp) : P.res != nullptr), DD_E_ARG,
+    DD_REQUIRE(P.n_img > 0 && (P.in || P.derive) && P.wa && P.wb && P.bias_a && P.bias_b && P.out && (!P.out2 || P.aff2) && P.zero && (first ? (P.in2 && P.wp) : P.res != nullptr), DD_E_ARG,
                "mars_pair64: bad argument");
-    return first ? launch_pair<true>(s, device, P) : launch_pair<false>(s, device, P);
-}
+    DD_REQUIRE(!P.derive || P.derive_pad >= (first ? 32 : 64), DD_E_ARG, "mars_pair64: derive_pad %d", P.derive_pad);
+    if (P.derive) return first ? launch_pair<true, true>(s, device, P) : launch_pair<false, true>(s, device, P);
+    return first ? launch_pair<true, false>(s, device, P) : launch_pair<false, false>(s, device, P);
+}
diff --git a/deepdish_amd/csrc/mars_tail.h b/deepdish_amd/csrc/mars_tail.h
--- a/deepdish_amd/csrc/mars_tail.h
+++ b/deepdish_amd/csrc/mars_tail.h
@@ -1,8 +1,18 @@
 #pragma once
 #include "common.h"
 
+__device__ __forceinline__ float dd_mars_elu(float v) {
+    float e = __builtin_amdgcn_exp2f(v * 1.44269504088896340736f);
+    e = __builtin_amdgcn_fmed3f(e, 0.f, 1.f);
+    return __builtin_amdgcn_fmed3f(v, e - 1.f, 3.0e38f);
+}
+__device__ __forceinline__ _Float16 dd_mars_pre(_Float16 raw, float scale, float shift) {
+    return (_Float16)dd_mars_elu(__builtin_fmaf(scale, (float)raw, shift));
+}
+
 struct MarsWsP {
     const _Float16 *in;  int cs_in, coff_in;
+    const float *derive; int derive_pad;
     const _Float16 *in2; int cs_in2, coff_in2;
     const _Float16 *w;   int kpad;
     const _Float16 *w2;  int kpad2;
@@ -21,6 +31,7 @@
 
 struct MarsPairP {
     const _Float16 *in;  int cs_in, coff_in;
+    const float *derive; int derive_pad;
     const _Float16 *in2; int cs_in2, coff_in2;
     const _Float16 *wa;  int kpad_a; const float *bias_a;
     const _Float16 *wp;  int kpad_p; const float *bias_p;
diff --git a/deepdish_amd/csrc/mars_tail.hip b/deepdish_amd/csrc/mars_tail.hip
--- a/deepdish_amd/csrc/mars_tail.hip
+++ b/deepdish_amd/csrc/mars_tail.hip
@@ -9,11 +9,7 @@
 
 enum { ACT_NONE = 0, ACT_ELU = 2 };
 
-__device__ __forceinline__ float elu(float v) {
-    float e = __builtin_amdgcn_exp2f(v * 1.44269504088896340736f);
-    e = __builtin_amdgcn_fmed3f(e, 0.f, 1.f);
-    return __builtin_amdgcn_fmed3f(v, e - 1.f, 3.0e38f);
-}
+__device__ __forceinline__ float elu(float v) { return dd_mars_elu(v); }
 
 __device__ __forceinline__ void lds_fill16(const _Float16 *g, char *lds_wave_base) {
 #if defined(__HIP_DEVICE_COMPILE__)
@@ -41,9 +37,9 @@
     return ws_off_aux(mode) + (mode == MARS_WS_S1_RES ? WS_NBR * WS_RES_BYTES : mode == MARS_WS_S2_PROJ ? WS_NB * WS_PRJ_BYTES : 0);
 }
 constexpr int ws_off_const(int mode) { return ws_off_xchg(mode) + 2 * 8 * ws_xw_bytes(mode); }
-constexpr int ws_lds_bytes(int mode) { return ws_off_const(mode) + 3 * 128 * 4; }
-
-template <int MODE, int ACT, bool OUT2>
+constexpr int ws_lds_bytes(int mode) { return ws_off_const(mode) + 5 * 128 * 4; }
+
+template <int MODE, int ACT, bool OUT2, bool DERIVE>
 __global__ __launch_bounds__(512, 2) void mars_ws128_k(const MarsWsP P) {
     constexpr bool S2 = MODE == MARS_WS_S2_PROJ, RES = MODE == MARS_WS_S1_RES;
     constexpr int LEAD = WS_LEAD, NB = WS_NB, NBR = WS_NBR;
@@ -64,6 +60,10 @@
         cst[tid] = P.bias[tid];
         if constexpr (S2) cst[128 + tid] = P.bias2 ? P.bias2[tid] : 0.f;
         if constexpr (RES && OUT2) { cst[128 + tid] = P.aff2[tid]; cst[256 + tid] = P.aff2[P.cout_pad + tid]; }
+        if constexpr (DERIVE) {
+            cst[384 + tid] = tid < (S2 ? 64 : 128) ? P.derive[tid] : 0.f;
+            cst[512 + tid] = tid < (S2 ? 64 : 128) ? P.derive[P.derive_pad + tid] : 0.f;
+        }
     }
     __syncthreads();
 
@@ -129,6 +129,25 @@
         dq_rslot = dq_rslot + 1 == NBR ? 0 : dq_rslot + 1;
     };
 
+    [[maybe_unused]] auto derive_own = [&](int sl) {
+        char *T = smem + OFF_T + sl * TILE_B;
+        const int pl = S2 ? (lane >> 2) & 7 : lane >> 2;
+        const f4 s0 = *reinterpret_cast<const f4 *>(cst + 384 + pl * 8), s1 = *reinterpret_cast<const f4 *>(cst + 384 + pl * 8 + 4);
+        const f4 t0 = *reinterpret_cast<const f4 *>(cst + 512 + pl * 8), t1 = *reinterpret_cast<const f4 *>(cst + 512 + pl * 8 + 4);
+#pragma unroll
+        for (int h = 0; h < (S2 ? 2 : 1); ++h) {
+            h8 *pc = reinterpret_cast<h8 *>(T + (S2 ? (wave + 8 * h) * 68 : (wave + 1) * 72) * 16 + lane * 16);
+            const h8 r = *pc;
+            h8 o;
+#pragma unroll
+            for (int i = 0; i < 4; ++i) { o[i] = dd_mars_pre(r[i], s0[i], t0[i]); o[4 + i] = dd_mars_pre(r[4 + i], s1[i], t1[i]); }
+            *pc = o;
+        }
+#if defined(__HIP_DEVICE_COMPILE__)
+        asm volatile("s_waitcnt lgkmcnt(0)" ::: "memory");
+#endif
+    };
+
     const unsigned lo = S2 ? (unsigned)((2 * yy * 68 + (kh * 4 + fq) * 4 + x) * 16) : (unsigned)((yy * 72 + (kh * 8 + fq) * 4 + x) * 16);
     const unsigned lo_prj = (unsigned)(((kh * 4 + fq) * 32 + yy * 4 + x) * 16);
     const unsigned lo_res = (unsigned)(((4 * kh + yy) * 72 + (cg * 4 + fq) * 4 + x) * 16);
@@ -166,7 +185,7 @@
             const f4 t0 = *reinterpret_cast<const f4 *>(cst + 256 + co), t1 = *reinterpret_cast<const f4 *>(cst + 256 + co + 4);
             h8 o2;
 #pragma unroll
-            for (int i = 0; i < 4; ++i) { o2[i] = (_Float16)elu(s0[i] * v[i] + t0[i]); o2[4 + i] = (_Float16)elu(s1[i] * v[4 + i] + t1[i]); }
+            for (int i = 0; i < 4; ++i) { o2[i] = dd_mars_pre(o[i], s0[i], t0[i]); o2[4 + i] = dd_mars_pre(o[4 + i], s1[i], t1[i]); }
             *reinterpret_cast<h8 *>(P.out2 + m * P.cs_out2 + P.coff_out2 + co) = o2;
         }
         if constexpr (S2) {
@@ -192,6 +211,7 @@
             if (c <= 1) asm volatile("s_waitcnt vmcnt(%0) lgkmcnt(0)" ::"i"(N_DMA) : "memory");
             else if (c == 2) asm volatile("s_waitcnt vmcnt(%0) lgkmcnt(0)" ::"i"(N_DMA + N_ST) : "memory");
             else asm volatile("s_waitcnt vmcnt(%0) lgkmcnt(0)" ::"i"(N_DMA + 2 * N_ST) : "memory");
+            if constexpr (DERIVE) { if (c < Kc) derive_own(slot); }
         } else asm volatile("s_waitcnt lgkmcnt(0)" ::: "memory");
         DD_STAMP(2);
         __builtin_amdgcn_s_barrier();
@@ -275,6 +295,7 @@
             if (c == 0) asm volatile("s_waitcnt vmcnt(%0) lgkmcnt(0)" ::"i"(N_DMA) : "memory");
             else if (c == 1) asm volatile("s_waitcnt vmcnt(%0) lgkmcnt(0)" ::"i"(N_DMA + N_ST) : "memory");
             else asm volatile("s_waitcnt vmcnt(%0) lgkmcnt(0)" ::"i"(N_DMA + 2 * N_ST) : "memory");
+            if constexpr (DERIVE) { if (c + 1 < Kc) derive_own(slot + 1 == NB ? 0 : slot + 1); }
             __builtin_amdgcn_s_barrier();
             asm volatile("" ::: "memory");
 #endif
@@ -299,19 +320,19 @@
 #endif
 }
 
-template <int MODE, int ACT, bool OUT2>
+template <int MODE, int ACT, bool OUT2, bool DERIVE = false>
 int launch_one(hipStream_t s, int device, const MarsWsP &P) {
     constexpr int lds = ws_lds_bytes(MODE);
     static_assert(lds <= 160 * 1024, "LDS budget");
     static DevOnce once;
     const int rc = once.run(device, [&]() -> int {
-        DD_HIP(hipFuncSetAttribute(reinterpret_cast<const void *>(&mars_ws128_k<MODE, ACT, OUT2>), hipFuncAttributeMaxDynamicSharedMemorySize, lds));
+        DD_HIP(hipFuncSetAttribute(reinterpret_cast<const void *>(&mars_ws128_k<MODE, ACT, OUT2, DERIVE>), hipFuncAttributeMaxDynamicSharedMemorySize, lds));
         return DD_OK;
     });
     if (rc != DD_OK) return rc;
     const int n_cu = dd_cu_count(device);
     const int grid = P.n_img < n_cu ? P.n_img : n_cu;
-    hipLaunchKernelGGL((mars_ws128_k<MODE, ACT, OUT2>), dim3(grid), dim3(512), lds, s, P);
+    hipLaunchKernelGGL((mars_ws128_k<MODE, ACT, OUT2, DERIVE>), dim3(grid), dim3(512), lds, s, P);
     DD_LAUNCH_CHECK();
 #ifdef DD_MARS_STAMPS
     {
@@ -338,15 +359,18 @@
 
 int mars_ws128_launch(hipStream_t s, int device, const MarsWsP &P, int mode, int act, bool out2) {
     DD_REQUIRE(P.n_img > 0 && P.in && P.w && P.bias && P.out && P.zero, DD_E_ARG, "mars_ws128: bad argument");
+    DD_REQUIRE(!P.derive || P.derive_pad >= (mode == MARS_WS_S2_PROJ ? 64 : 128), DD_E_ARG, "mars_ws128: derive_pad %d", P.derive_pad);
     DD_REQUIRE((long long)P.n_img * 128 * (P.cs_in > P.cs_out ? P.cs_in : P.cs_out) < (1ll << 40), DD_E_CAPACITY, "mars_ws128: batch of %d", P.n_img);
     if (mode == MARS_WS_S2_PROJ) {
         DD_REQUIRE(P.in2 && P.w2 && P.out2 && act == ACT_ELU, DD_E_ARG, "mars_ws128: stride-2 form needs the projection operands and ELU");
-        return launch_one<MARS_WS_S2_PROJ, ACT_ELU, false>(s, device, P);
+        return P.derive ? launch_one<MARS_WS_S2_PROJ, ACT_ELU, false, true>(s, device, P) : launch_one<MARS_WS_S2_PROJ, ACT_ELU, false>(s, device, P);
     }
     if (mode == MARS_WS_S1) {
         DD_REQUIRE(!P.res && !P.out2, DD_E_ARG, "mars_ws128: plain form with a residual or a second output");
+        DD_REQUIRE(!P.derive || act == ACT_ELU, DD_E_ARG, "mars_ws128: a derived pre-activation feeds a block's first (ELU) layer");
+        if (P.derive) return launch_one<MARS_WS_S1, ACT_ELU, false, true>(s, device, P);
         return act == ACT_ELU ? launch_one<MARS_WS_S1, ACT_ELU, false>(s, device, P) : launch_one<MARS_WS_S1, ACT_NONE, false>(s, device, P);
     }
-    DD_REQUIRE(mode == MARS_WS_S1_RES && P.res && act == ACT_NONE && (!out2 || (P.out2 && P.aff2)), DD_E_ARG, "mars_ws128: residual form");
+    DD_REQUIRE(mode == MARS_WS_S1_RES && P.res && act == ACT_NONE && !P.derive && (!out2 || (P.out2 && P.aff2)), DD_E_ARG, "mars_ws128: residual form");
     return out2 ? launch_one<MARS_WS_S1_RES, ACT_NONE, true>(s, device, P) : launch_one<MARS_WS_S1_RES, ACT_NONE, false>(s, device, P);
 }
diff --git a/deepdish_amd/csrc/net_priv.h b/deepdish_amd/csrc/net_priv.h
--- a/deepdish_amd/csrc/net_priv.h
+++ b/deepdish_amd/csrc/net_priv.h
@@ -33,6 +33,7 @@
     int tile_mode = 0;
     std::vector<hipEvent_t> events;
     std::vector<int32_t> op_launch;
+    std::vector<char> op_elided;
     struct GraphEntry { int calls = 0; hipGraph_t graph = nullptr; hipGraphExec_t exec = nullptr; };
     bool use_graph = false;
     std::map<std::pair<const void *, int>, GraphEntry> graphs;
diff --git a/deepdish_amd/csrc/nets.hip b/deepdish_amd/csrc/nets.hip
--- a/deepdish_amd/csrc/nets.hip
+++ b/deepdish_amd/csrc/nets.hip
@@ -146,10 +146,7 @@
         const f4 sh = *reinterpret_cast<const f4 *>(P.aff2 + P.cout_pad + co);
         h4 o;
 #pragma unroll
-        for (int r = 0; r < 4; ++r) {
-            const float t = co + r < P.cout ? apply_act(sc[r] * v[r] + sh[r], ACT_ELU) : 0.f;
-            o[r] = (_Float16)t;
-        }
+        for (int r = 0; r < 4; ++r) o[r] = co + r < P.cout ? dd_mars_pre((_Float16)v[r], sc[r], sh[r]) : (_Float16)0.f;
         *reinterpret_cast<h4 *>(P.out2 + (size_t)m * P.cs_out2 + P.coff_out2 + co) = o;
     }
 }
@@ -220,7 +217,7 @@
 #pragma unroll
         for (int r = 0; r < 8; ++r) {
             const float sc = r < 4 ? E.s0[r] : E.s1[r - 4], sh = r < 4 ? E.t0[r] : E.t1[r - 4];
-            o2[r] = (_Float16)apply_act(sc * v[r] + sh, ACT_ELU);
+            o2[r] = dd_mars_pre((_Float16)v[r], sc, sh);
         }
         if (tail) {
 #pragma unroll
@@ -1563,7 +1560,7 @@
 constexpr int RP_X_SLOTS = 8;
 constexpr int rp_pair_halves() { return 6 * 8 + (RU_PRE_SLOTS + 2 * RU_H1_SLOTS + 2 * RP_X_SLOTS) * RU_SLOT; }
 
-template <int ACT_A>
+template <int ACT_A, bool OUT2>
 __global__ __launch_bounds__(512, 2) void res_pair_rows_k(const ConvP P1A, const ConvP P1B, const ConvP P2A, const ConvP P2B, const int n_img) {
     extern __shared__ __attribute__((aligned(16))) _Float16 lds[];
     const int tid = threadIdx.x, lane = tid & 63;
@@ -1668,7 +1665,7 @@
 #pragma unroll
             for (int q = 0; q < 4; ++q) { o[q] = accC[cr][0][q]; o[4 + q] = accC[cr][1][q]; }
             const h8 rv = *reinterpret_cast<const h8 *>(resr + ((s + 1) & (RU_PRE_SLOTS - 1)) * RU_SLOT + offC);
-            conv_epilogue_f16x8<ACT_NONE, false, 1, true, false>(P2B, EB, ((n0 + kk * nstep) * H + y) * W + fr, fq * 8, o, &rv);
+            conv_epilogue_f16x8<ACT_NONE, false, OUT2 ? 1 : 2, true, false>(P2B, EB, ((n0 + kk * nstep) * H + y) * W + fr, fq * 8, o, &rv);
         }
     };
     for (int g = 0; g < Gall; ++g) {
@@ -1717,7 +1714,7 @@
 #pragma unroll
                         for (int q = 0; q < 8; ++q) {
                             const float sc = q < 4 ? EB.s0[q] : EB.s1[q - 4], sh = q < 4 ? EB.t0[q] : EB.t1[q - 4];
-                            o2[q] = (_Float16)apply_act(sc * v[q] + sh, ACT_ELU);
+                            o2[q] = dd_mars_pre(o[q], sc, sh);
                         }
                         u4v_t ou = __builtin_bit_cast(u4v_t, o), ou2 = __builtin_bit_cast(u4v_t, o2);
                         ou &= live ? 0xFFFFFFFFu : 0u;
@@ -3560,16 +3557,18 @@
            A2.H == A1.H && A2.W == A1.W && A1.act == ACT_ELU && A2.act == ACT_ELU;
 }
 
-int launch_res_pair(hipStream_t s, const ConvP &A1, const ConvP &B1, const ConvP &A2, const ConvP &B2, int nimg, int device) {
+int launch_res_pair(hipStream_t s, const ConvP &A1, const ConvP &B1, const ConvP &A2, const ConvP &B2, int nimg, int device, bool write_out2) {
     constexpr size_t lds_bytes = (size_t)4 * rp_pair_halves() * sizeof(_Float16);
     static DevOnce once;
     const int rc = once.run(device, [&]() -> int {
-        DD_HIP(hipFuncSetAttribute(reinterpret_cast<const void *>(&res_pair_rows_k<ACT_ELU>), hipFuncAttributeMaxDynamicSharedMemorySize, (int)lds_bytes));
+        DD_HIP(hipFuncSetAttribute(reinterpret_cast<const void *>(&res_pair_rows_k<ACT_ELU, true>), hipFuncAttributeMaxDynamicSharedMemorySize, (int)lds_bytes));
+        DD_HIP(hipFuncSetAttribute(reinterpret_cast<const void *>(&res_pair_rows_k<ACT_ELU, false>), hipFuncAttributeMaxDynamicSharedMemorySize, (int)lds_bytes));
         return DD_OK;
     });
     if (rc != DD_OK) return rc;
     const int grid = std::min(dd_ceil_div(nimg, 4), 256);
-    hipLaunchKernelGGL((res_pair_rows_k<ACT_ELU>), dim3((unsigned)grid), dim3(512), lds_bytes, s, A1, B1, A2, B2, nimg);
+    if (write_out2) hipLaunchKernelGGL((res_pair_rows_k<ACT_ELU, true>), dim3((unsigned)grid), dim3(512), lds_bytes, s, A1, B1, A2, B2, nimg);
+    else hipLaunchKernelGGL((res_pair_rows_k<ACT_ELU, false>), dim3((unsigned)grid), dim3(512), lds_bytes, s, A1, B1, A2, B2, nimg);
     DD_LAUNCH_CHECK();
     return DD_OK;
 }
@@ -3909,6 +3908,20 @@
     const TensorDesc &qs = net->tensors[q[1]], &qd = net->tensors[q[2]];
     return qs.h == 16 && qs.w == 8 && qd.h == 8 && qd.w == 4 && qs.cs % 8 == 0 && qs.coff % 8 == 0 && qd.cs % 8 == 0 && qd.coff % 8 == 0 && qd.dtype == DT_F16;
 }
+bool mars_one_tensor() {
+    static const bool on = getenv("DD_MARS_ONE_TENSOR") && atoi(getenv("DD_MARS_ONE_TENSOR")) != 0;
+    return on;
+}
+const float *mars_derive_aff(const dd_net *net, int j, int pre, int raw, int *pad) {
+    if (!mars_one_tensor() || j < 1 || pre < 0 || raw < 0) return nullptr;
+    const int32_t *b = net->prog.data() + net->ops_off + (size_t)(j - 1) * OP_WORDS;
+    if (b[0] != OP_CONV || b[4] != pre || b[2] != raw || !b[19] || b[15] != EPI_F16) return nullptr;
+    const TensorDesc &tp = net->tensors[pre], &tr = net->tensors[raw];
+    if (tp.h != tr.h || tp.w != tr.w || tp.c != tr.c || tr.c != b[11] || tr.dtype != DT_F16 || tr.cs % 8 || tr.coff % 8) return nullptr;
+    *pad = b[12];
+    return reinterpret_cast<const float *>(net->d_weights + (size_t)(uint32_t)b[18]);
+}
+
 int mars_pair_match(const dd_net *net, int i, int nimg, MarsPairP &Q, bool &first) {
     void *const *bufs = net->bufs.data();
     static const bool off = getenv("DD_MARS_PAIR") && atoi(getenv("DD_MARS_PAIR")) == 0;
@@ -3936,6 +3949,7 @@
         Q.wp = reinterpret_cast<const _Float16 *>(W(p, 16)); Q.kpad_p = p[13]; Q.bias_p = reinterpret_cast<const float *>(W(p, 17));
         const int32_t *b = op(nb);
         if (b[3] != p[2]) return 0;
+        Q.derive = mars_derive_aff(net, i, a[1], p[1], &Q.derive_pad);
     } else if (i + 1 < net->n_ops && a[30] == 4 && conv3(a, 1, 64, ACT_ELU) && a[3] < 0 && a[4] < 0 && t16x8(a[1], 64) && t16x8(a[2], 64)) {
         first = false; nb = i + 1;
         const TensorDesc &ti = net->tensors[a[1]];
@@ -3944,6 +3958,7 @@
         if (b[3] < 0 || !t16x8(b[3], 64)) return 0;
         const TensorDesc &tr = net->tensors[b[3]];
         Q.res = reinterpret_cast<const _Float16 *>(bufs[tr.buf]); Q.cs_res = tr.cs; Q.coff_res = tr.coff;
+        Q.derive = mars_derive_aff(net, i, a[1], b[3], &Q.derive_pad);
     } else return 0;
     const int32_t *b = op(nb);
     if (!(conv3(b, 1, 64, ACT_NONE) && b[1] == a[2] && b[3] >= 0 && b[4] >= 0 && b[19] && t16x8(b[2], 64) && t16x8(b[4], 64))) return 0;
@@ -3967,6 +3982,18 @@
     Q.out2 = P.out2; Q.cs_out2 = P.cs_out2; Q.coff_out2 = P.coff_out2; Q.aff2 = P.aff2; Q.cout_pad = P.cout_pad;
     Q.zero = P.zero; Q.n_img = nimg;
     return Q;
+}
+
+bool mars_ws_derive(const dd_net *net, int j, int src, int raw, MarsWsP *Q) {
+    int pad = 0;
+    const float *aff = mars_derive_aff(net, j, src, raw, &pad);
+    if (!aff) return false;
+    if (Q) {
+        const TensorDesc &tr = net->tensors[raw];
+        Q->in = reinterpret_cast<const _Float16 *>(net->bufs[tr.buf]); Q->cs_in = tr.cs; Q->coff_in = tr.coff;
+        Q->derive = aff; Q->derive_pad = pad;
+    }
+    return true;
 }
 
 }
@@ -4175,7 +4202,8 @@
 int dd_net_op_launches(dd_net *n, int32_t *codes_host, int cap, int *n_ops_host) {
     DD_REQUIRE(n && codes_host && n_ops_host, DD_E_ARG, "dd_net_op_launches: NULL argument");
     DD_REQUIRE(cap >= n->n_ops, DD_E_ARG, "dd_net_op_launches: cap %d < %d ops", cap, n->n_ops);
-    for (int i = 0; i < n->n_ops; ++i) codes_host[i] = i < (int)n->op_launch.size() ? n->op_launch[i] : OPK_DEFAULT;
+    for (int i = 0; i < n->n_ops; ++i)
+        codes_host[i] = (i < (int)n->op_launch.size() ? n->op_launch[i] : OPK_DEFAULT) | (i < (int)n->op_elided.size() && n->op_elided[i] ? DD_OPK_ONE_TENSOR : 0);
     *n_ops_host = n->n_ops;
     return DD_OK;
 }
@@ -4197,6 +4225,9 @@
         DD_REQUIRE(!(o[2] == t && n->op_launch[i] == OPK_YOLO_HEAD_DEC), DD_E_STATE,
                    "dd_net_read: tensor %d (the Detect matrix) was not written: the head layers reduced their rows in their epilogue "
                    "(dd_net_yolo_decode); read dd_net_yolo_decoded instead", t);
+        DD_REQUIRE(!(o[4] == t && i < (int)n->op_elided.size() && n->op_elided[i]), DD_E_STATE,
+                   "dd_net_read: tensor %d was not written by the last forward (the launch that reads this pre-activation derived it on chip "
+                   "from op %d's first output; DD_MARS_ONE_TENSOR=0 or a smaller batch writes it)", t, i);
         DD_REQUIRE(!((o[2] == t || o[4] == t) && n->op_launch[i] == OPK_FOLDED), DD_E_STATE,
                    "dd_net_read: tensor %d was not written by the last forward (op %d ran inside the next op's launch at this batch "
                    "size and its output stayed on chip); run a smaller batch or a program compiled without the fusion flags", t, i);
@@ -4389,6 +4420,7 @@
         return static_cast<char *>(net->bufs[d.buf]);
     };
     net->op_launch.assign((size_t)net->n_ops, OPK_DEFAULT);
+    net->op_elided.assign((size_t)net->n_ops, 0);
     ConvP stem_p;
     bool stem_pending = false;
     bool wide_pending = false, wide_ready = false;
@@ -4411,6 +4443,52 @@
         net->op_launch[pair_op] = OPK_RES_UNIT;
         return launch_res_unit(s, pair_a, pair_b, nimg, net->ctx->device);
     };
+    auto make_convp = [&](int k) -> ConvP {
+        const int32_t *o = net->prog.data() + net->ops_off + (size_t)k * OP_WORDS;
+        const float *of = reinterpret_cast<const float *>(o);
+        const int src = o[1], dst = o[2], res = o[3], dst2 = o[4];
+        const TensorDesc *ts = &net->tensors[src], *td = &net->tensors[dst];
+        ConvP P;
+        memset(&P, 0, sizeof(P));
+        P.in = reinterpret_cast<const _Float16 *>(base(src)); P.H = ts->h; P.W = ts->w; P.cs_in = ts->cs;
+        P.coff_in = ts->coff; P.cin = o[10];
+        P.kh = o[5]; P.kw = o[6]; P.stride = o[7]; P.pad_t = o[8]; P.pad_l = o[9];
+        P.cout = o[11]; P.cout_pad = o[12]; P.kpad = o[13]; P.act = o[14]; P.epi = o[15];
+        P.w = reinterpret_cast<const _Float16 *>(net->d_weights + (size_t)(uint32_t)o[16]);
+        P.bias = reinterpret_cast<const float *>(net->d_weights + (size_t)(uint32_t)o[17]);
+        P.ho = o[26]; P.wo = o[27]; P.m = nimg * P.ho * P.wo;
+        P.out = base(dst); P.cs_out = td->cs; P.coff_out = td->coff;
+        if (res >= 0) {
+            const TensorDesc &tr = net->tensors[res];
+            P.res = reinterpret_cast<const _Float16 *>(base(res)); P.cs_res = tr.cs; P.coff_res = tr.coff;
+        }
+        if (dst2 >= 0) {
+            const TensorDesc &t2 = net->tensors[dst2];
+            P.out2 = reinterpret_cast<_Float16 *>(base(dst2)); P.cs_out2 = t2.cs; P.coff_out2 = t2.coff;
+            P.aff2 = reinterpret_cast<const float *>(net->d_weights + (size_t)(uint32_t)o[18]);
+        }
+        if (dst2 < 0 && o[19]) {
+            P.aff2 = reinterpret_cast<const float *>(net->d_weights + (size_t)(uint32_t)o[18]);
+            P.post_aff = 1;
+        }
+        for (int q = 0; q < 6; ++q) P.p[q] = o[20 + q];
+        for (int q = 0; q < 8; ++q) P.f[q] = of[32 + q];
+        return P;
+    };
+    auto mars_next_derives = [&](int k) -> bool {
+        if (!mars_one_tensor() || k + 1 >= net->n_ops) return false;
+        const int32_t *o = net->prog.data() + net->ops_off + (size_t)k * OP_WORDS, *q = o + OP_WORDS;
+        if (o[0] != OP_CONV || o[4] < 0 || q[0] != OP_CONV || q[1] != o[4] || q[2] < 0) return false;
+        if (q[30] == 3 || q[30] == 4) {
+            MarsPairP Q; bool first;
+            if (mars_pair_match(net, k + 1, nimg, Q, first)) return Q.derive != nullptr;
+        }
+        const ConvP N = make_convp(k + 1);
+        if (mars_ws_s1_eligible(N)) return !N.res && N.act == ACT_ELU && mars_ws_derive(net, k + 1, q[1], o[2], nullptr);
+        if (q[30] == 3 && k + 2 < net->n_ops && mars_ws_s2_eligible(N) && mars_proj_follows(net, k + 1, N))
+            return q[OP_WORDS + 1] == o[2] && mars_ws_derive(net, k + 1, q[1], o[2], nullptr);
+        return false;
+    };
     auto run_ws = [&](ConvP &P) { return P.cin == 256 ? launch_conv_ws<4>(s, P, net->ctx->device) : launch_conv_ws<8>(s, P, net->ctx->device); };
     int first_op = 0;
     bool mid_on = false;
@@ -4453,7 +4531,7 @@
         if (net->profile) DD_HIP(hipEventRecord(net->events[i], s));
         const int32_t *o = net->prog.data() + net->ops_off + (size_t)i * OP_WORDS;
         const float *of = reinterpret_cast<const float *>(o);
-        const int kind = o[0], src = o[1], dst = o[2], res = o[3], dst2 = o[4];
+        const int kind = o[0], src = o[1], dst = o[2];
         const TensorDesc *ts = src >= 0 ? &net->tensors[src] : nullptr;
         const TensorDesc *td = dst >= 0 ? &net->tensors[dst] : nullptr;
         DD_REQUIRE(!input_pending || (kind == OP_CONV && i == input_op + 1), DD_E_STATE, "dd_net_forward: input op %d was folded into an op that did not take it", input_op);
@@ -4514,6 +4592,7 @@
                 if (pair_left > 0) {
                     DD_NO_PENDING();
                     if (--pair_left > 0) { net->op_launch[i] = OPK_FOLDED; break; }
+                    if (mars_next_derives(i)) { pair64.out2 = nullptr; net->op_elided[i] = 1; }
                     const int rc = mars_pair64_launch(s, net->ctx->device, pair64, pair64_first);
                     if (rc != DD_OK) return rc;
                     net->op_launch[i] = OPK_MARS_PAIR;
@@ -4524,31 +4603,7 @@
                     if (n_ops) { DD_NO_PENDING(); pair_left = n_ops - 1; net->op_launch[i] = OPK_FOLDED; break; }
                 }
 #undef DD_NO_PENDING
-                ConvP P;
-                memset(&P, 0, sizeof(P));
-                P.in = reinterpret_cast<const _Float16 *>(base(src)); P.H = ts->h; P.W = ts->w; P.cs_in = ts->cs;
-                P.coff_in = ts->coff; P.cin = o[10];
-                P.kh = o[5]; P.kw = o[6]; P.stride = o[7]; P.pad_t = o[8]; P.pad_l = o[9];
-                P.cout = o[11]; P.cout_pad = o[12]; P.kpad = o[13]; P.act = o[14]; P.epi = o[15];
-                P.w = reinterpret_cast<const _Float16 *>(net->d_weights + (size_t)(uint32_t)o[16]);
-                P.bias = reinterpret_cast<const float *>(net->d_weights + (size_t)(uint32_t)o[17]);
-                P.ho = o[26]; P.wo = o[27]; P.m = nimg * P.ho * P.wo;
-                P.out = base(dst); P.cs_out = td->cs; P.coff_out = td->coff;
-                if (res >= 0) {
-                    const TensorDesc &tr = net->tensors[res];
-                    P.res = reinterpret_cast<const _Float16 *>(base(res)); P.cs_res = tr.cs; P.coff_res = tr.coff;
-                }
-                if (dst2 >= 0) {
-                    const TensorDesc &t2 = net->tensors[dst2];
-                    P.out2 = reinterpret_cast<_Float16 *>(base(dst2)); P.cs_out2 = t2.cs; P.coff_out2 = t2.coff;
-                    P.aff2 = reinterpret_cast<const float *>(net->d_weights + (size_t)(uint32_t)o[18]);
-                }
-                if (dst2 < 0 && o[19]) {
-                    P.aff2 = reinterpret_cast<const float *>(net->d_weights + (size_t)(uint32_t)o[18]);
-                    P.post_aff = 1;
-                }
-                for (int q = 0; q < 6; ++q) P.p[q] = o[20 + q];
-                for (int q = 0; q < 8; ++q) P.f[q] = of[32 + q];
+                ConvP P = make_convp(i);
                 int rc;
                 DD_REQUIRE(!o[29] || (net->use_rw && P.kh == 3 && P.stride == 1 && P.cin == 32 && P.cout_pad == 32), DD_E_ARG,
                            "dd_net_forward: fused pooling is only built for the 3x3 32->32 kernel");
@@ -4559,8 +4614,10 @@
                         if (pair_pending) {
                             if (res_pair_fusable(pair_a, pair_b, unit_a, P, nimg)) {
                                 pair_pending = false;
-                                rc = launch_res_pair(s, pair_a, pair_b, unit_a, P, nimg, net->ctx->device);
+                                const bool elide = mars_next_derives(i);
+                                rc = launch_res_pair(s, pair_a, pair_b, unit_a, P, nimg, net->ctx->device, !elide);
                                 if (rc != DD_OK) return rc;
+                                net->op_elided[i] = elide;
                                 net->op_launch[i] = OPK_RES_PAIR;
                                 break;
                             }
@@ -4647,9 +4704,12 @@
                     if (o[29] && pool_rows_fusable(P, nimg)) net->op_launch[i] = P.src8 ? OPK_POOL_ROWS_STEM : OPK_POOL_ROWS;
                     rc = launch_conv3x3_rw(s, P, nimg, o[29] != 0, net->ctx->device);
                 } else if (mars_ws_s1_eligible(P)) {
-                    const MarsWsP Q = mars_ws_params(P, nimg);
+                    MarsWsP Q = mars_ws_params(P, nimg);
                     net->op_launch[i] = OPK_MARS_WS;
-                    rc = mars_ws128_launch(s, net->ctx->device, Q, P.res ? MARS_WS_S1_RES : MARS_WS_S1, P.act, P.out2 != nullptr);
+                    if (!P.res && P.act == ACT_ELU && i > 0) mars_ws_derive(net, i, src, (o - OP_WORDS)[2], &Q);
+                    const bool elide = P.res && P.out2 && mars_next_derives(i);
+                    if (elide) { Q.out2 = nullptr; net->op_elided[i] = 1; }
+                    rc = mars_ws128_launch(s, net->ctx->device, Q, P.res ? MARS_WS_S1_RES : MARS_WS_S1, P.act, P.out2 != nullptr && !elide);
                 } else if (o[30] == 3 && i + 1 < net->n_ops && mars_ws_s2_eligible(P) && mars_proj_follows(net, i, P)) {
                     const int32_t *q = net->prog.data() + net->ops_off + (size_t)(i + 1) * OP_WORDS;
                     const TensorDesc &qs = net->tensors[q[1]], &qd = net->tensors[q[2]];
@@ -4658,6 +4718,7 @@
                     Q.w2 = reinterpret_cast<const _Float16 *>(net->d_weights + (size_t)(uint32_t)q[16]); Q.kpad2 = q[13];
                     Q.bias2 = reinterpret_cast<const float *>(net->d_weights + (size_t)(uint32_t)q[17]);
                     Q.out2 = reinterpret_cast<_Float16 *>(base(q[2])); Q.cs_out2 = qd.cs; Q.coff_out2 = qd.coff;
+                    mars_ws_derive(net, i, src, q[1], &Q);
                     net->op_launch[i] = OPK_MARS_WS;
                     rc = mars_ws128_launch(s, net->ctx->device, Q, MARS_WS_S2_PROJ, P.act, false);
                     proj_done = true;
diff --git a/deepdish_amd/profile.py b/deepdish_amd/profile.py
--- a/deepdish_amd/profile.py
+++ b/deepdish_amd/profile.py
@@ -28,12 +28,23 @@
 OPK_FOLDED_PREV = 15
 
 
-def net_op_launches(net):
+OPK_ONE_TENSOR = 0x100
+
+
+def _op_launch_words(net):
     n = len(net.program.ops)
     codes = np.zeros(n, dtype=np.int32)
     cnt = ctypes.c_int(0)
     check(lib().dd_net_op_launches(net._h, ptr(codes), n, ctypes.byref(cnt)), 'dd_net_op_launches')
     return codes
+
+
+def net_op_launches(net):
+    return _op_launch_words(net) & (OPK_ONE_TENSOR - 1)
+
+
+def net_op_one_tensor(net):
+    return (_op_launch_words(net) & OPK_ONE_TENSOR) != 0
 
 
 def launches_of(net, ms, batch):
diff --git a/include/deepdish_hip.h b/include/deepdish_hip.h
--- a/include/deepdish_hip.h
+++ b/include/deepdish_hip.h
@@ -133,6 +133,7 @@
 
 int dd_net_profile(dd_net *net, int enable);
 int dd_net_profile_read(dd_net *net, float *ms_host, int cap, int *n_ops_host);
+#define DD_OPK_ONE_TENSOR 0x100
 int dd_net_op_launches(dd_net *net, int32_t *codes_host, int cap, int *n_ops_host);
 
 int dd_ssd_postprocess(dd_ctx *ctx, const float *raw, const float *anchors, int n_anchors,
```

Result: slower. 143,000 frames/s (-2.2%).
